# timoklein/alphazero-gym

Hardware: AMD Instinct MI355X
Metric: MCTS sims/sec (whole node), Pendulum-v1 4096 trees n_sims=200, 1/2/4/8 GPU (higher is better)
Workload: dtype f32; 1 GPU; config C: Pendulum-v1 A0C, 4096 trees/GPU x 200 sims, 2x256 ELU policy/value MLP, c_uct=0.05 c_pw=1 kappa=0.5; trees_per_gpu=4096, n_sims=200, parallelism=1 GPU

## Files before the change

alphazero_gym_amd/csrc/aux_kernels.cuh:

```cuda
#pragma once
#include "records.h"
#include "env.cuh"
#include "tree.cuh"
#include "results.cuh"


#define RS_TREES 16
__global__ __launch_bounds__(16 * RS_TREES) void results_kernel(KParams P) {
    const int sub = threadIdx.x & 15;
    const int tree = blockIdx.x * RS_TREES + (threadIdx.x >> 4);
    if (tree >= P.B) return;
    const size_t tb = (size_t)tree * P.R;
    TreeStore<TS_GLOBAL> ts;
    ts.hot = P.hot + tb;
    ts.child = P.child + tb * P.Kp;
    ts.prior = P.prior + tb;
    if (P.mode == AZG_MODE_CONTINUOUS) results_for_tree<true, TS_GLOBAL>(P, ts, P.cold + tb, P.action + tb, tb, tree, sub);
    else results_for_tree<false, TS_GLOBAL>(P, ts, P.cold + tb, P.action + tb, tb, tree, sub);
}


struct SelfPlay {
    int max_len, deterministic;
    int S_obs;
    int final_selection;
    double agent_eps;
    const double* ctab;
    unsigned step_idx;
    int* t; int* episode; int* fcnt;
    double* ret; double* fsum;
    float* rows;
    double* roots; int* carry;
};

__device__ __forceinline__ void selfplay_finish(const KParams& P, const SelfPlay& sp, int tree, float* row, float action, double v_target,
                                                int carry) {
    const int S = P.S;
    double root[4] = {0.0, 0.0, 0.0, 0.0};
    for (int k = 0; k < S; ++k) root[k] = sp.roots[(size_t)tree * S + k];
    float obs[8];
    double sn;
    game_obs(P.env_id, root, obs, &sn);
    for (int k = 0; k < 8; ++k) if (k < sp.S_obs) row[k] = obs[k];
    row[sp.S_obs + 3 * P.res_Kmax] = (float)v_target;
    double ns[4] = {0.0, 0.0, 0.0, 0.0}, r;
    int done;
    game_step(P.env_id, root, sn, action, ns, &r, &done);
    double ret = sp.ret[tree] + r;
    int t = sp.t[tree] + 1;
    if (done || t >= sp.max_len) {
        sp.fsum[tree] = sp.fsum[tree] + ret;
        sp.fcnt[tree] += 1;
        ret = 0.0;
        t = 0;
        const int ep = sp.episode[tree] + 1;
        sp.episode[tree] = ep;
        azg_reset_state(P.seed, (unsigned)(P.tree_base + tree), (unsigned)ep, azg_reset_kind(P.env_id), ns);
        carry = 0;
    }
    sp.carry[tree] = carry;
    sp.ret[tree] = ret;
    sp.t[tree] = t;
    for (int k = 0; k < S; ++k) sp.roots[(size_t)tree * S + k] = ns[k];
}

#define SP_TREES 16
__global__ __launch_bounds__(16 * SP_TREES) void selfplay_kernel16(KParams P, SelfPlay sp) {
    const int sub = threadIdx.x & 15;
    const int tree = blockIdx.x * SP_TREES + (threadIdx.x >> 4);
    if (tree >= P.B) return;
    const bool cont = P.mode == AZG_MODE_CONTINUOUS;
    const unsigned gtree = (unsigned)(P.tree_base + tree);
    const int K = P.res_Kmax, S_obs = sp.S_obs;
    float* row = sp.rows + (size_t)tree * (S_obs + 3 * K + 1);
    const int nc = P.res_nch[tree];
    const bool has = sub < nc;
    struct { int edge_n, node_n; double Q; } h;
    {
        const size_t o = (size_t)tree * K + (sub < K ? sub : 0);
        const int cn = P.res_child_n[o];
        h.edge_n = has ? P.res_counts[o] : 0;
        h.Q = has ? P.res_Q[o] : 0.0;
        h.node_n = (has && cn >= 0) ? cn : 0;
    }
    const float act = has ? (cont ? P.res_actions[(size_t)tree * K + sub] : (float)sub) : 0.0f;
    if (sub < K) {
        row[S_obs + sub] = act;
        row[S_obs + K + sub] = has ? (float)h.edge_n : 0.0f;
        row[S_obs + 2 * K + sub] = has ? (float)h.Q : 0.0f;
    }
    int tot = has ? h.edge_n : 0;
    double qmax = has ? h.Q : -__builtin_huge_val();
    int ckey = has ? ((h.edge_n << 4) | (15 - sub)) : -1;
    for (int m = 1; m < 16; m <<= 1) {
        tot += __shfl_xor(tot, m, 16);
        const double o = __shfl_xor(qmax, m, 16);
        qmax = o > qmax ? o : qmax;
        const int ok = __shfl_xor(ckey, m, 16);
        ckey = ok > ckey ? ok : ckey;
    }
    if (nc == 0) qmax = 0.0;
    const int cmax = ckey >> 4, amax = 15 - (ckey & 15);
    double x = 0.0;
    if (!cont && has) {
        if (sp.final_selection == AZG_FS_MAX_VALUE) x = h.Q / qmax;
        else x = sp.ctab ? sp.ctab[(size_t)cmax * (cmax + 1) / 2 + h.edge_n] : (double)h.edge_n / (double)cmax;
    }
    double onp = 0.0;
    if (P.res_v_target == AZG_VT_ON_POLICY) {
        if (!cont) {
            for (int a = 0; a < nc; ++a) onp += ((double)__shfl(h.edge_n, a, 16) / (double)tot) * __shfl(h.Q, a, 16);
        } else {
            for (int a = 0; a < nc; ++a) {
                const double qa = __shfl(h.Q, a, 16);
                for (int b2 = 0; b2 < nc; ++b2) onp += ((double)__shfl(h.edge_n, b2, 16) / (double)tot) * qa;
            }
        }
    }
    int pick = 0;
    if (cont) {
        pick = amax;
        if (sp.final_selection == AZG_FS_MAX_VALUE) {
            double qb = 0.0;
            for (int a = 0; a < nc; ++a) { const double q = __shfl(h.Q, a, 16); if (a == 0 || q > qb) { qb = q; pick = a; } }
        }
        if (sp.agent_eps != 0.0) {
            azg_u32x4 b = azg_draw(P.seed, gtree, sp.step_idx, 0u, AZG_STREAM_ACT);
            if ((double)azg_u01(b.v[0]) < sp.agent_eps) pick = (int)(b.v[1] % (unsigned)nc);
        }
    } else {
        double sum = 0.0;
        for (int a = 0; a < nc; ++a) sum = sum + __shfl(x, a, 16);
        const double pi = has ? __builtin_fabs(x / sum) : 0.0;
        double best = 0.0, cum = 0.0;
        for (int a = 0; a < nc; ++a) {
            const double pa = __shfl(pi, a, 16);
            if (a == 0 || pa > best) { best = pa; pick = a; }
            cum = cum + pa;
        }
        if (!sp.deterministic) {
            azg_u32x4 b = azg_draw(P.seed, gtree, sp.step_idx, 0u, AZG_STREAM_ACT);
            const double u = ((double)b.v[0] + 0.5) * (1.0 / 4294967296.0);
            const double last = cum;
            double c = 0.0;
            pick = nc - 1;
            bool found = false;
            for (int a = 0; a < nc; ++a) {
                const double pa = __shfl(pi, a, 16);
                if (!found) {
                    c = c + pa;
                    if (u < c / last) { pick = a; found = true; }
                }
            }
        }
    }
    const float pact = __shfl(act, pick, 16);
    const int pnode_n = __shfl(h.node_n, pick, 16);
    if (sub != 0) return;
    selfplay_finish(P, sp, tree, row, pact, P.res_v_target == AZG_VT_ON_POLICY ? onp : qmax, cont ? 0 : pnode_n);
}

#define SPW_THREADS 64
__global__ __launch_bounds__(SPW_THREADS) void selfplay_kernel(KParams P, SelfPlay sp) {
    const int tree = blockIdx.x * blockDim.x + threadIdx.x;
    if (tree >= P.B) return;
    const size_t tb = (size_t)tree * P.R;
    const unsigned gtree = (unsigned)(P.tree_base + tree);
    const int K = P.res_Kmax, S_obs = sp.S_obs;
    float* row = sp.rows + (size_t)tree * (S_obs + 3 * K + 1);
    const int nc = P.hot[tb].n_child;
    auto id = [&](int a) { return a < nc ? (int)P.child[tb * P.Kp + a] : 0; };
    auto rec = [&](int a) { return P.hot[tb + id(a)]; };
    auto act = [&](int a) { return P.action[tb + id(a)]; };
    double qmax = 0.0, onp = 0.0;
    long tot = 0;
    int cmax = 0, amax = 0;
    for (int a = 0; a < nc; ++a) tot += rec(a).edge_n;
    for (int a = 0; a < K; ++a) {
        const bool has = a < nc;
        const RecL h = rec(a);
        row[S_obs + a] = has ? act(a) : 0.0f;
        row[S_obs + K + a] = has ? (float)h.edge_n : 0.0f;
        row[S_obs + 2 * K + a] = has ? (float)h.Q : 0.0f;
        if (has) {
            if (a == 0 || h.Q > qmax) qmax = h.Q;
            if (a == 0 || h.edge_n > cmax) { cmax = h.edge_n; amax = a; }
        }
    }
    if (P.res_v_target == AZG_VT_ON_POLICY)
        for (int a = 0; a < nc; ++a)
            for (int b = 0; b < nc; ++b) onp += ((double)rec(b).edge_n / (double)tot) * rec(a).Q;
    int pick = amax;
    if (sp.final_selection == AZG_FS_MAX_VALUE) {
        double qb = 0.0;
        for (int a = 0; a < nc; ++a) { const double q = rec(a).Q; if (a == 0 || q > qb) { qb = q; pick = a; } }
    }
    if (sp.agent_eps != 0.0) {
        azg_u32x4 b = azg_draw(P.seed, gtree, sp.step_idx, 0u, AZG_STREAM_ACT);
        if ((double)azg_u01(b.v[0]) < sp.agent_eps) pick = (int)(b.v[1] % (unsigned)nc);
    }
    selfplay_finish(P, sp, tree, row, act(pick), P.res_v_target == AZG_VT_ON_POLICY ? onp : qmax, 0);
}
```

alphazero_gym_amd/csrc/azg_engine.hip:

```cpp
#include <cmath>
#include <cstdio>
#include <cstdlib>
#include <cstring>

#include "engine_host.h"
#include "../../include/azg_math.h"

static std::string g_create_err;

int fail(azg_engine* e, int code, const std::string& msg) {
    if (e) e->err = msg; else g_create_err = msg;
    return code;
}

static int ls_prepare(azg_engine* e) {
    if (e->ls_hp == e->HP) return AZG_OK;
    e->ls_mem.clear();
    const size_t B = e->cfg.n_trees, G = ((B + TREES_PER_WG - 1) / TREES_PER_WG + 3) / 4 * 4, HP = e->HP;
    float* obsT; float *a0, *a1, *parts; LsTree* tr; LsLane* ln;
    e->team_cnt_bytes = (((B + 31) / 32) * 8 * 32 + 32) * sizeof(unsigned);
    if (dalloc(e, e->ls_mem, &e->d_team_cnt, e->team_cnt_bytes / 4) ||
        dalloc(e, e->ls_mem, &obsT, G * 64) || dalloc(e, e->ls_mem, &a0, G * HP * 16) || dalloc(e, e->ls_mem, &a1, G * HP * 16) ||
        dalloc(e, e->ls_mem, &parts, G * (HP / 64) * 64 * 4) || dalloc(e, e->ls_mem, &tr, B) ||
        dalloc(e, e->ls_mem, &ln, B * 16))
        return AZG_E_DEVICE;
    e->ls.obsT = obsT; e->ls.act[0] = (f32x4*)a0; e->ls.act[1] = (f32x4*)a1; e->ls.parts = (f32x4*)parts;
    e->ls.tree = tr; e->ls.lane = ln;
    if (hipMemset(obsT, 0, G * 64 * sizeof(float)) != hipSuccess || hipMemset(a0, 0, G * HP * 16 * sizeof(float)) != hipSuccess || hipMemset(a1, 0, G * HP * 16 * sizeof(float)) != hipSuccess) return AZG_E_DEVICE;
    e->ls_hp = e->HP;
    return AZG_OK;
}

static bool use_lockstep(const azg_engine* e) {
    if (e->opt.force_persistent) return false;
    if (e->P.in8) return false;
    return e->HP >= 512 && e->n_hidden >= 2 && !e->P.layernorm;
}

template <int ENV>
static hipError_t search_path(azg_engine* e, bool lockstep) {
    if (lockstep) {
        if constexpr (ENV == AZG_ENV_ACROBOT) return hipErrorInvalidValue;
        else return azg_lockstep_search<ENV>(e);
    }
    return e->HP <= 128 ? azg_persistent_search<ENV, false>(e) : azg_persistent_search<ENV, true>(e);
}
static hipError_t search_launch(azg_engine* e, bool lockstep) {
    switch (azg_kernel_env(e->cfg)) {
        case AZG_ENV_CARTPOLE: return search_path<AZG_ENV_CARTPOLE>(e, lockstep);
        case AZG_ENV_MOUNTAINCAR_CONT: return search_path<AZG_ENV_MOUNTAINCAR_CONT>(e, lockstep);
        case AZG_ENV_ACROBOT: return search_path<AZG_ENV_ACROBOT>(e, lockstep);
        default: return search_path<AZG_ENV_PENDULUM_V1>(e, lockstep);
    }
}

static int team_check(azg_engine* e) {
    unsigned flag = 0;
    e->team_pending = 0;
    if (hipMemcpy(&flag, e->d_team_cnt + (e->team_cnt_bytes / 4 - 1), 4, hipMemcpyDeviceToHost) != hipSuccess)
        return fail(e, AZG_E_DEVICE, "reading the team kernel's status failed");
    if (flag) e->opt.ls_team = 0;
    if (flag == 0) return AZG_OK;
    e->team_fallbacks += 1;
    e->search_idx = e->team_search_idx;
    int rc = azg_search_resident(e);
    if (rc) return rc;
    if (hipStreamSynchronize(e->stream) != hipSuccess) return fail(e, AZG_E_DEVICE, "hipStreamSynchronize failed");
    return AZG_OK;
}
int settle_team(azg_engine* e) {
    if (!e->team_pending) return AZG_OK;
    HIPCHK(e, hipStreamSynchronize(e->stream));
    return team_check(e);
}

struct EnvFacts { int state_words, obs_width, discrete, n_actions; };
static constexpr EnvFacts kEnv[AZG_ENV_ACROBOT + 1] = {
    {4, 4, 1, 2},
    {2, 3, 0, 0},
    {2, 3, 0, 0},
    {2, 2, 1, 3},
    {2, 2, 0, 0},
    {4, 6, 1, 3},
};

static bool root_is_terminal(int env_id, const double* s) {
    switch (env_id) {
        case AZG_ENV_CARTPOLE: {
            const double theta_thr = 12.0 * 2.0 * 3.141592653589793 / 360.0, x_thr = 2.4;
            return (s[0] < -x_thr) || (s[0] > x_thr) || (s[2] < -theta_thr) || (s[2] > theta_thr);
        }
        case AZG_ENV_ACROBOT: return azg_acrobot_terminal(s);
        case AZG_ENV_MOUNTAINCAR: return s[0] >= 0.5 && s[1] >= 0.0;
        case AZG_ENV_MOUNTAINCAR_CONT: return s[0] >= 0.45 && s[1] >= 0.0;
        default: return false;
    }
}

EngineOptions EngineOptions::from_env() {
    const auto digit = [](const char* name, int dflt) {
        const char* v = getenv(name);
        return (v && v[0] >= '0' && v[0] <= '9') ? v[0] - '0' : dflt;
    };
    const auto num = [](const char* name) { const char* v = getenv(name); return v ? atoi(v) : 0; };
    EngineOptions o;
    o.force_persistent = digit("AZG_FORCE_PERSISTENT", 0) == 1;
    o.force_stream_weights = digit("AZG_FORCE_STREAM_WEIGHTS", 0) == 1;
    o.force_global_tree = digit("AZG_FORCE_GLOBAL_TREE", 0) == 1;
    o.no_spec = digit("AZG_NO_SPEC", 0) == 1;
    o.waves = digit("AZG_WAVES", o.waves);
    o.groups = digit("AZG_GROUPS", o.groups);
    { const int t = num("AZG_TRACE_CAP"); o.trace_cap = t > 0 ? t : 0; }
    { const int t = num("AZG_TILE_TREES"); o.tile_trees = (t == 16 || t == 8) ? t : 0; }
    o.ls_team = digit("AZG_LS_TEAM", o.ls_team);
    o.team_wide = digit("AZG_TEAM_WIDE", o.team_wide);
    o.team_tt = num("AZG_TEAM_TT");
    if (const char* v = getenv("AZG_TEAM_SPIN_LIMIT")) o.team_spin_limit = atol(v);
    o.no_lds_state = getenv("AZG_NO_LDS_STATE") != nullptr;
    o.publish_always = digit("AZG_PUBLISH_TREES", 0) == 1;
    return o;
}

extern "C" {

int azg_abi_version(void) { return AZG_ABI_VERSION; }

const char* azg_last_error(const azg_engine* e) { return e ? e->err.c_str() : g_create_err.c_str(); }

void azg_engine_destroy(azg_engine* e) {
    if (!e) return;
    DeviceScope scope(e->cfg.device_id);
    if (e->stream) (void)hipStreamSynchronize(e->stream);
    delete e;
}

static int mapped_hip_runtimes(std::string& paths) {
    static int cached_n = -1;
    static std::string cached_paths;
    if (cached_n >= 0) { paths = cached_paths; return cached_n; }
    std::vector<std::string> seen;
    FILE* f = fopen("/proc/self/maps", "r");
    if (!f) return 0;
    char line[1024];
    while (fgets(line, sizeof line, f)) {
        if (!strstr(line, "libamdhip64")) continue;
        const char* p = strchr(line, '/');
        if (!p) continue;
        std::string path(p);
        while (!path.empty() && (path.back() == '\n' || path.back() == ' ')) path.pop_back();
        bool dup = false;
        for (const auto& q : seen) dup = dup || q == path;
        if (!dup) seen.push_back(path);
    }
    fclose(f);
    paths.clear();
    for (const auto& q : seen) paths += (paths.empty() ? "" : ", ") + q;
    cached_paths = paths;
    cached_n = (int)seen.size();
    return cached_n;
}

static int engine_build(azg_engine* e) {
    const azg_config* cfg = &e->cfg;
    e->opt = EngineOptions::from_env();
    e->S_env = kEnv[cfg->env_id].state_words;
    e->S_obs = kEnv[cfg->env_id].obs_width;
    const int ns = cfg->n_sims;
    std::vector<int> pw(ns + 2, 0);
    if (cfg->mode == AZG_MODE_CONTINUOUS) {
        int kmax = 1;
        for (int n = 0; n < ns + 2; ++n) {
            double v = std::ceil(cfg->c_pw * std::pow((double)(n + 1), cfg->kappa));
            if (v > 1e6) v = 1e6;
            pw[n] = (int)v;
            if (n < ns && pw[n] > kmax) kmax = pw[n];
        }
        e->Kmax = kmax;
        e->R = ns + 2;
        e->nd = 2;
    } else {
        e->Kmax = cfg->num_actions;
        e->R = 1 + cfg->num_actions * (ns + 1);
        e->nd = cfg->num_actions;
    }
    if (e->R > 32767) return fail(e, AZG_E_UNSUPPORTED, "tree too large: records per tree must be < 32768");
    if (cfg->tie_break == AZG_TIE_RANDOM && e->Kmax > 16) return fail(e, AZG_E_UNSUPPORTED, "tie_break random supports at most 16 children per node");
    e->Kp = (e->Kmax + 15) / 16 * 16;
    e->tab_n = cfg->mode == AZG_MODE_CONTINUOUS ? ns + 2 : 4 * ns + 4;
    ON_DEVICE(e);
    (void)hipDeviceGetAttribute(&e->n_cus, hipDeviceAttributeMultiprocessorCount, cfg->device_id);
    HIPCHK(e, hipStreamCreateWithFlags(&e->stream, hipStreamNonBlocking));
    HIPCHK(e, hipEventCreate(&e->ev0));
    HIPCHK(e, hipEventCreate(&e->ev1));
    KParams& P = e->P;
    const size_t B = (size_t)cfg->n_trees, R = (size_t)e->R, K = (size_t)e->Kmax;
    RecL* hot; Cold* cold; double* edge_W; float* action; float* prior; unsigned short* child; int* n_rec;
    int* d_pw; double* d_sq; unsigned long long* stamps;
    e->res = ResultsLayout(B, K);
    e->stamp_n = stamp_rows(B);
    DeviceAllocs& mem = e->mem;
    if (dalloc(e, mem, &hot, B * R) || dalloc(e, mem, &cold, B * R) || dalloc(e, mem, &edge_W, B * R) || dalloc(e, mem, &action, B * R) ||
        dalloc(e, mem, &prior, B * R) || dalloc(e, mem, &child, B * R * e->Kp) || dalloc(e, mem, &n_rec, B) ||
        dalloc(e, mem, &d_pw, (size_t)ns + 2) || dalloc(e, mem, &d_sq, (size_t)e->tab_n) || dalloc(e, mem, &e->d_roots, B * e->S_env) ||
        dalloc(e, mem, &e->d_carry, B) || dalloc(e, mem, &e->d_res_block, e->res.bytes) || dalloc(e, mem, &e->d_child_n, B * K) ||
        dalloc(e, mem, &e->d_child_state, B * K * e->S_env) || dalloc(e, mem, &e->d_rootV, B) || dalloc(e, mem, &e->d_rootdist, B * e->nd) ||
        dalloc(e, e->stamp_mem, &stamps, e->stamp_n * 16))
        return AZG_E_DEVICE;
    HIPCHK(e, hipHostMalloc(&e->h_res.p, e->res.bytes, hipHostMallocDefault));
    char* const blk = e->d_res_block;
    e->d_Q = (double*)(blk + e->res.Q); e->d_vt = (double*)(blk + e->res.vt); e->d_actions = (float*)(blk + e->res.actions);
    e->d_counts = (int*)(blk + e->res.counts); e->d_nch = (int*)(blk + e->res.nch);
    std::vector<double> sq(e->tab_n);
    for (int n = 0; n < e->tab_n; ++n) sq[n] = std::sqrt((double)(n + 1));
    HIPCHK(e, hipMemcpy(d_pw, pw.data(), sizeof(int) * (ns + 2), hipMemcpyHostToDevice));
    HIPCHK(e, hipMemcpy(d_sq, sq.data(), sizeof(double) * e->tab_n, hipMemcpyHostToDevice));
    HIPCHK(e, hipMemset(hot, 0, B * R * sizeof(RecL)));
    HIPCHK(e, hipMemset(e->d_carry, 0, B * sizeof(int)));
    P.B = cfg->n_trees; P.n_sims = ns; P.R = e->R; P.Kp = e->Kp; P.A = cfg->num_actions; P.nd = e->nd;
    P.trace_cap = e->opt.trace_cap > 0 ? e->opt.trace_cap : 5;
    P.tie_random = cfg->tie_break == AZG_TIE_RANDOM; P.env_id = cfg->env_id; P.v1 = cfg->env_id == AZG_ENV_PENDULUM_V1; P.tree_base = cfg->tree_id_base; P.mode = cfg->mode;
    P.c_uct = cfg->c_uct; P.gamma = cfg->gamma; P.epsilon = cfg->epsilon; P.reward_scale = cfg->reward_scale;
    P.c_uct_f = (float)cfg->c_uct; P.gamma_f = (float)cfg->gamma; P.bound_f = (float)cfg->action_bound;
    P.seed = cfg->seed; P.S = e->S_env; P.tab_n = e->tab_n; P.pw0 = cfg->mode == AZG_MODE_CONTINUOUS ? pw[0] : 0;
    P.roots = e->d_roots; P.carry = e->d_carry;
    P.hot = hot; P.cold = cold; P.edge_W = edge_W; P.action = action; P.prior = prior; P.child = child;
    P.n_rec = n_rec; P.pw_need = d_pw; P.sqrt_tab = d_sq; P.stamps = stamps;
    P.res_actions = e->d_actions; P.res_counts = e->d_counts; P.res_Q = e->d_Q; P.res_vt = e->d_vt; P.res_nch = e->d_nch;
    P.res_child_n = e->d_child_n; P.res_child_state = e->d_child_state; P.res_root_V = e->d_rootV; P.res_root_dist = e->d_rootdist;
    P.res_Kmax = e->Kmax; P.res_v_target = cfg->v_target;
    P.net_T = cfg->n_trees; P.net_wgs = 1; P.net_wstride = 0;
    return AZG_OK;
}

int azg_engine_create(const azg_config* cfg, azg_engine** out) {
    if (!cfg || !out) return fail(nullptr, AZG_E_INVALID, "null argument");
    {
        std::string rts;
        const char* allow = getenv("AZG_ALLOW_MULTI_HIP");
        if (mapped_hip_runtimes(rts) > 1 && !(allow && allow[0] == '1'))
            return fail(nullptr, AZG_E_DEVICE, ("two HIP runtimes are mapped in this process (" + rts + "): load PyTorch (import torch) BEFORE "
                                               "libazgym_hip.so so that both use PyTorch's copy; if they are meant to coexist (differing "
                                               "SONAMEs, a deliberate second copy), set AZG_ALLOW_MULTI_HIP=1").c_str());
    }
    if (cfg->struct_size != (int32_t)sizeof(azg_config)) return fail(nullptr, AZG_E_INVALID, "azg_config size mismatch");
    if (cfg->n_trees < 1 || cfg->n_sims < 1) return fail(nullptr, AZG_E_INVALID, "n_trees and n_sims must be >= 1");
    if (cfg->env_id < 0 || cfg->env_id > AZG_ENV_ACROBOT) return fail(nullptr, AZG_E_INVALID, "unknown env_id");
    const bool discrete_env = kEnv[cfg->env_id].discrete;
    if (cfg->mode == AZG_MODE_DISCRETE && !discrete_env)
        return fail(nullptr, AZG_E_UNSUPPORTED, "discrete mode requires a discrete-action env (CartPole, MountainCar, Acrobot)");
    if (cfg->mode == AZG_MODE_CONTINUOUS && discrete_env)
        return fail(nullptr, AZG_E_UNSUPPORTED, "continuous mode requires a continuous-action env (Pendulum, MountainCarContinuous)");
    if (cfg->mode == AZG_MODE_DISCRETE && cfg->num_actions != kEnv[cfg->env_id].n_actions)
        return fail(nullptr, AZG_E_INVALID, "num_actions does not match the env (CartPole 2, MountainCar 3, Acrobot 3)");
    if (cfg->tie_break != AZG_TIE_FIRST && cfg->tie_break != AZG_TIE_RANDOM) return fail(nullptr, AZG_E_INVALID, "unknown tie_break");
    if (cfg->mode == AZG_MODE_CONTINUOUS && !(cfg->c_pw > 0.0 && cfg->c_pw < 1e6 && cfg->kappa >= 0.0 && cfg->kappa <= 8.0))
        return fail(nullptr, AZG_E_INVALID, "c_pw must be > 0 and kappa >= 0 (progressive widening: ceil(c_pw (n + 1)^kappa) children)");
    int ndev = 0;
    if (hipGetDeviceCount(&ndev) != hipSuccess || ndev < 1) return fail(nullptr, AZG_E_DEVICE, "no HIP device available");
    if (cfg->device_id < 0 || cfg->device_id >= ndev) return fail(nullptr, AZG_E_DEVICE, "device_id out of range");
    azg_engine* e = new azg_engine();
    e->cfg = *cfg;
    const int rc = engine_build(e);
    if (rc != AZG_OK) {
        const std::string msg = e->err;
        azg_engine_destroy(e);
        return fail(nullptr, rc, msg);
    }
    *out = e;
    return AZG_OK;
}

int azg_set_search_index(azg_engine* e, uint32_t idx) { if (!e) return AZG_E_INVALID; e->search_idx = idx; return AZG_OK; }

int azg_upload_roots(azg_engine* e, const double* roots, const int32_t* carry) {
    if (!e || !roots) return AZG_E_INVALID;
    const int B = e->cfg.n_trees, S = e->S_env;
    for (int i = 0; i < B; ++i)
        if (root_is_terminal(e->cfg.env_id, roots + (size_t)i * S)) return fail(e, AZG_E_TERMINAL_ROOT, "Can't do tree search from a terminal node");
    int cmax = 0;
    if (carry)
        for (int i = 0; i < B; ++i) {
            if (carry[i] < 0 || carry[i] > (1 << 30)) return fail(e, AZG_E_INVALID, "root_n_carry out of range");
            if (carry[i] != 0 && e->cfg.mode == AZG_MODE_CONTINUOUS)
                return fail(e, AZG_E_INVALID, "root_n_carry: continuous searches start from a fresh root (no carried count)");
            if (carry[i] > cmax) cmax = carry[i];
        }
    ON_DEVICE(e);
    { int trc = settle_team(e); if (trc) return trc; }
    e->carry_max = cmax;
    e->redo_ok = 0;
    HIPCHK(e, hipMemcpyAsync(e->d_roots, roots, sizeof(double) * (size_t)B * S, hipMemcpyHostToDevice, e->stream));
    if (carry) HIPCHK(e, hipMemcpyAsync(e->d_carry, carry, sizeof(int) * (size_t)B, hipMemcpyHostToDevice, e->stream));
    else HIPCHK(e, hipMemsetAsync(e->d_carry, 0, sizeof(int) * (size_t)B, e->stream));
    HIPCHK(e, hipStreamSynchronize(e->stream));
    return AZG_OK;
}

int azg_search_resident(azg_engine* e) {
    if (!e) return AZG_E_INVALID;
    if (!e->mlp_ready)
        return fail(e, AZG_E_STATE, e->n_nets > 1 ? "azg_set_net_weights has not been called for every net of the population"
                                                 : "azg_set_weights has not been called");
    if (e->n_nets > 1 && use_lockstep(e))
        return fail(e, AZG_E_UNSUPPORTED, "populations run on the one-launch search kernel only");
    ON_DEVICE(e);
    e->P.search_idx = e->search_idx;
    e->last_search_idx = e->search_idx;
    e->ms_kept_valid = 0;
    e->P.publish = (e->opt.publish_always || e->publish_once) ? 1 : 0;
    e->team_search_idx = e->search_idx;
    e->last = LaunchRecord();
    const bool lockstep = use_lockstep(e);
    if (lockstep) { int prc = ls_prepare(e); if (prc) return prc; }
    if (lockstep) HIPCHK(e, hipEventRecord(e->ev0, e->stream));
    const hipError_t rc = search_launch(e, lockstep);
    if (rc != hipSuccess) return fail(e, AZG_E_DEVICE, std::string("search kernel launch: ") + hipGetErrorString(rc));
    if (!e->last.timed) HIPCHK(e, hipEventRecord(e->ev1, e->stream));
    e->search_idx += 1;
    e->searched = 1;
    const bool persistent = e->last.form == AZG_FORM_PERSISTENT;
    e->results_valid = persistent ? 1 : 0;
    e->published = (!persistent || e->last.tree_lds == TS_GLOBAL || e->P.publish) ? 1 : 0;
    e->redo_ok = 1;
    if (persistent && e->last.tree_lds == TS_GLOBAL && e->last.lds_exit != AZG_LDS_EXIT_FORCED && !e->lds_warned) {
        e->lds_warned = 1;
        static const char* why[] = {"", "more than 511 records per tree (n_sims + 2)", "more than 16 children per node (c_pw / kappa)",
                                    "the workgroup's LDS plan exceeds the CU's 160 KB", "", "",
                                    "the root's visit count (carried + n_sims) overflows the LDS records' counters"};
        const int x = e->last.lds_exit;
        const char* reason = x == AZG_LDS_EXIT_RECORDS && e->R <= 511 ? "more than 255 records per tree (n_sims + 2) for this network's kernels"
                                                                      : (x >= 0 && x < (int)(sizeof(why) / sizeof(why[0])) ? why[x] : "");
        if (!getenv("AZG_QUIET"))
            fprintf(stderr, "azgym: the trees of this search do not fit LDS residency (%s): they are kept in global memory -- same results, "
                            "slower tree walk (azg_search_info; once per engine)\n", reason);
    }
    return AZG_OK;
}

int azg_sync(azg_engine* e) {
    if (!e) return AZG_E_INVALID;
    ON_DEVICE(e);
    HIPCHK(e, hipStreamSynchronize(e->stream));
    return settle_team(e);
}

int azg_search(azg_engine* e, const double* roots, const int32_t* carry) {
    int rc = azg_upload_roots(e, roots, carry);
    if (rc) return rc;
    rc = azg_search_resident(e);
    if (rc) return rc;
    return azg_sync(e);
}

int azg_last_search_ms(azg_engine* e, float* ms) {
    if (!e || !ms) return AZG_E_INVALID;
    if (!e->searched) return fail(e, AZG_E_STATE, "no search has run");
    ON_DEVICE(e);
    HIPCHK(e, hipEventSynchronize(e->ev1));
    { int trc = settle_team(e); if (trc) return trc; }
    if (e->ms_kept_valid) { *ms = e->ms_kept; return AZG_OK; }
    HIPCHK(e, hipEventElapsedTime(ms, e->ev0, e->ev1));
    return AZG_OK;
}

static int gather_results(azg_engine* e) {
    ON_DEVICE(e);
    int rc = launch_results(e);
    if (rc) return rc;
    HIPCHK(e, hipStreamSynchronize(e->stream));
    return AZG_OK;
}

int azg_results(azg_engine* e, float* actions, int32_t* counts, double* Q, double* v_target, int32_t* n_children) {
    if (!e) return AZG_E_INVALID;
    ON_DEVICE(e);
    int rc = launch_results(e);
    if (rc) return rc;
    const ResultsLayout& L = e->res;
    HIPCHK(e, hipMemcpyAsync(e->h_res.p, e->d_res_block, L.bytes, hipMemcpyDeviceToHost, e->stream));
    HIPCHK(e, hipStreamSynchronize(e->stream));
    const char* h = (const char*)e->h_res.p;
    if (Q) memcpy(Q, h + L.Q, L.vt - L.Q);
    if (v_target) memcpy(v_target, h + L.vt, L.actions - L.vt);
    if (actions) memcpy(actions, h + L.actions, L.counts - L.actions);
    if (counts) memcpy(counts, h + L.counts, L.nch - L.counts);
    if (n_children) memcpy(n_children, h + L.nch, L.bytes - L.nch);
    return AZG_OK;
}

int azg_results_resident(azg_engine* e, const float** actions, const int32_t** counts, const double** Q, const double** v_target,
                         const int32_t** n_children) {
    if (!e) return AZG_E_INVALID;
    ON_DEVICE(e);
    int rc = launch_results(e);
    if (rc) return rc;
    if (actions) *actions = e->d_actions;
    if (counts) *counts = e->d_counts;
    if (Q) *Q = e->d_Q;
    if (v_target) *v_target = e->d_vt;
    if (n_children) *n_children = e->d_nch;
    return AZG_OK;
}

int azg_root_children(azg_engine* e, int32_t* child_n, double* child_state) {
    if (!e) return AZG_E_INVALID;
    int rc = gather_results(e);
    if (rc) return rc;
    size_t B = e->cfg.n_trees, K = e->Kmax;
    D2H(child_n, e->d_child_n, B * K * 4);
    D2H(child_state, e->d_child_state, B * K * e->S_env * 8);
    return AZG_OK;
}

int azg_root_eval(azg_engine* e, float* value, float* dist) {
    if (!e) return AZG_E_INVALID;
    if (e->n_nets > 1) return fail(e, AZG_E_UNSUPPORTED, "azg_root_eval: not available for populations (azg_set_population > 1)");
    int rc = gather_results(e);
    if (rc) return rc;
    size_t B = e->cfg.n_trees;
    D2H(value, e->d_rootV, B * 4);
    D2H(dist, e->d_rootdist, B * e->nd * 4);
    return AZG_OK;
}

int azg_mlp_eval(azg_engine* e, const float* obs, size_t n, float* value, float* dist, float* raw) {
    if (!e || !obs) return AZG_E_INVALID;
    if (e->n_nets > 1) return fail(e, AZG_E_UNSUPPORTED, "azg_mlp_eval: not available for populations (azg_set_population > 1): evaluate each net's policy");
    if (!e->mlp_ready) return fail(e, AZG_E_STATE, "azg_set_weights has not been called");
    if (n == 0) return AZG_OK;
    if (n > (size_t)1 << 24) return fail(e, AZG_E_INVALID, "too many observations in one call");
    ON_DEVICE(e);
    const size_t So = e->S_obs, nd = e->nd;
    const size_t need = n * (So + 1 + nd + 1 + nd);
    if (need > e->eval_floats) {
        e->eval_mem.clear();
        e->eval_floats = 0;
        if (dalloc(e, e->eval_mem, &e->d_eval, need)) return AZG_E_DEVICE;
        e->eval_floats = need;
    }
    float* d_obs = e->d_eval;
    float* d_v = d_obs + n * So;
    float* d_d = d_v + n;
    float* d_r = d_d + n * nd;
    HIPCHK(e, hipMemcpyAsync(d_obs, obs, n * So * 4, hipMemcpyHostToDevice, e->stream));
    hipError_t rc = azg_dispatch_mlp_eval(e, d_obs, (int)n, d_v, d_d, d_r);
    if (rc != hipSuccess) return fail(e, AZG_E_DEVICE, std::string("mlp_eval kernel launch: ") + hipGetErrorString(rc));
    HIPCHK(e, hipStreamSynchronize(e->stream));
    D2H(value, d_v, n * 4);
    D2H(dist, d_d, n * nd * 4);
    D2H(raw, d_r, n * (nd + 1) * 4);
    return AZG_OK;
}

int azg_dump_tree(azg_engine* e, int32_t* n_records, int32_t* parent, int32_t* edge_n, double* edge_W, double* edge_Q,
                  float* edge_action, int32_t* node_n, double* node_r, float* node_V, uint8_t* node_flags) {
    if (!e) return AZG_E_INVALID;
    if (!e->searched) return fail(e, AZG_E_STATE, "no search has run");
    ON_DEVICE(e);
    HIPCHK(e, hipStreamSynchronize(e->stream));
    { int trc = settle_team(e); if (trc) return trc; }
    if (!e->published) {
        if (!e->redo_ok)
            return fail(e, AZG_E_STATE, "the last search's trees were not written out and its inputs have changed since (self-play step, new "
                                        "roots or weights): dump right after the search, or set AZG_PUBLISH_TREES=1");
        float ms_before = 0.0f;
        HIPCHK(e, hipEventElapsedTime(&ms_before, e->ev0, e->ev1));
        const uint32_t idx_now = e->search_idx;
        e->publish_once = 1;
        e->search_idx = e->last_search_idx;
        int rc = azg_search_resident(e);
        e->publish_once = 0;
        e->search_idx = idx_now;
        if (rc) return rc;
        HIPCHK(e, hipStreamSynchronize(e->stream));
        { int trc = settle_team(e); if (trc) return trc; }
        e->ms_kept = ms_before; e->ms_kept_valid = 1;
    }
    size_t B = e->cfg.n_trees, R = e->R;
    std::vector<RecL> hot(B * R);
    std::vector<Cold> cold(B * R);
    std::vector<int> nrec(B);
    std::vector<double> ew(B * R);
    std::vector<float> ac(B * R);
    HIPCHK(e, hipMemcpy(hot.data(), e->P.hot, B * R * sizeof(RecL), hipMemcpyDeviceToHost));
    HIPCHK(e, hipMemcpy(cold.data(), e->P.cold, B * R * sizeof(Cold), hipMemcpyDeviceToHost));
    HIPCHK(e, hipMemcpy(nrec.data(), e->P.n_rec, B * 4, hipMemcpyDeviceToHost));
    HIPCHK(e, hipMemcpy(ew.data(), e->P.edge_W, B * R * 8, hipMemcpyDeviceToHost));
    HIPCHK(e, hipMemcpy(ac.data(), e->P.action, B * R * 4, hipMemcpyDeviceToHost));
    const bool cont = e->cfg.mode == AZG_MODE_CONTINUOUS;
    const int A = e->cfg.num_actions;
    for (size_t i = 0; i < B; ++i) {
        if (n_records) n_records[i] = nrec[i];
        for (size_t j = 0; j < R; ++j) {
            size_t o = i * R + j;
            bool in = (int)j < nrec[i];
            const RecL& h = hot[o];
            bool ex = in && (h.flags & FLAG_EXPANDED);
            if (parent) parent[o] = in ? (j == 0 ? -1 : h.parent) : 0;
            if (edge_n) edge_n[o] = in ? h.edge_n : 0;
            if (edge_W) edge_W[o] = in ? ew[o] : 0.0;
            if (edge_Q) edge_Q[o] = in ? h.Q : 0.0;
            if (edge_action) edge_action[o] = in ? (cont ? ac[o] : (j == 0 ? 0.0f : (float)((j - 1) % A))) : 0.0f;
            if (node_n) node_n[o] = in ? h.node_n : 0;
            if (node_r) node_r[o] = ex ? cold[o].r : 0.0;
            if (node_V) node_V[o] = ex ? cold[o].V : 0.0f;
            if (node_flags) node_flags[o] = in ? h.flags : 0;
        }
    }
    return AZG_OK;
}

static int kernel_name(const azg_engine* e, char* buf, size_t n) {
    const int env = azg_kernel_env(e->cfg);
    const char* gmm = (env != AZG_ENV_CARTPOLE && e->P.ncomp >= 2) ? "true" : "false";
    const LaunchRecord& r = e->last;
    switch (r.form) {
        case AZG_FORM_PERSISTENT: return snprintf(buf, n, "search_kernel<%d, %d, %d, %d, %s, %d, %d, %d, %d>", env, e->HP, e->nreg, r.tree_lds, gmm, r.waves, r.groups, r.tile_trees, r.spec);
        case AZG_FORM_PER_LAYER: return snprintf(buf, n, "ls_tree_kernel<%d, ...> + ls_layer0_kernel + ls_hidden_tiled_kernel<%d, ...> per simulation step", env, e->HP);
        case AZG_FORM_TEAM: return snprintf(buf, n, "ls_team_kernel<%d, %d, %s, %d, %d, %d, %d, %d>", env, e->HP, gmm, r.tree_lds, r.team_kc, r.team_minb, r.spec, r.team_tt);
        default: return snprintf(buf, n, "(no search yet)");
    }
}

int azg_search_info(azg_engine* e, azg_search_report* info) {
    if (!e || !info) return AZG_E_INVALID;
    if (info->struct_size != (int32_t)sizeof(azg_search_report)) return fail(e, AZG_E_INVALID, "azg_search_info: struct_size mismatch");
    if (e->searched && e->team_pending) {
        ON_DEVICE(e);
        int trc = settle_team(e);
        if (trc) return trc;
    }
    memset(info, 0, sizeof(*info));
    info->struct_size = (int32_t)sizeof(azg_search_report);
    const LaunchRecord& r = e->last;
    info->kernel_form = e->searched ? r.form : AZG_FORM_NONE;
    info->max_records = e->R; info->max_children = e->Kmax;
    info->team_fallbacks = e->team_fallbacks;
    if (!e->searched) { kernel_name(e, info->kernel_name, sizeof(info->kernel_name)); info->lds_exit = AZG_LDS_RESIDENT; return AZG_OK; }
    info->tree_storage = r.form == AZG_FORM_PERSISTENT ? r.tree_lds : AZG_TREES_GLOBAL;
    info->lds_exit = r.lds_exit;
    info->spec = r.spec;
    info->waves = r.waves; info->groups = r.groups; info->tile_trees = r.tile_trees;
    if (r.form == AZG_FORM_TEAM) { info->team_trees = r.team_tt; info->team_per_cu = r.team_minb; info->team_parts = r.team_parts; }
    float ms = 0.0f;
    int rc = azg_last_search_ms(e, &ms);
    if (rc) return rc;
    info->last_ms = ms;
    kernel_name(e, info->kernel_name, sizeof(info->kernel_name));
    return AZG_OK;
}

int azg_max_children(const azg_engine* e) { return e ? e->Kmax : AZG_E_INVALID; }
int azg_max_records(const azg_engine* e) { return e ? e->R : AZG_E_INVALID; }
int azg_env_state_dim(const azg_engine* e) { return e ? e->S_env : AZG_E_INVALID; }
int azg_obs_dim(const azg_engine* e) { return e ? e->S_obs : AZG_E_INVALID; }

int azg_synthetic_roots(azg_engine* e, double* roots) {
    if (!e || !roots) return AZG_E_INVALID;
    for (int i = 0; i < e->cfg.n_trees; ++i)
        azg_reset_state(e->cfg.seed, (uint32_t)(e->cfg.tree_id_base + i), 0u, azg_reset_kind(e->cfg.env_id), roots + (size_t)i * e->S_env);
    return AZG_OK;
}

}
```

alphazero_gym_amd/csrc/engine_host.h:

```cpp
#pragma once
#include <hip/hip_runtime.h>

#include <atomic>
#include <string>
#include <vector>

#include "hip_host.h"
#include "records.h"
#include "../../include/azgym_population.h"

struct EngineOptions {
    int force_persistent = 0;
    int force_stream_weights = 0;
    int force_global_tree = 0;
    int waves = 0;
    int groups = 0;
    int trace_cap = 0;
    int no_spec = 0;
    int tile_trees = 0;
    int ls_team = 1;
    int team_wide = 1;
    int team_tt = 0;
    long team_spin_limit = 1L << 23;
    int no_lds_state = 0;
    int publish_always = 0;
    static EngineOptions from_env();
};
#define AZG_MAX_DEVICES 64

struct LaunchRecord {
    int form = AZG_FORM_NONE;
    int tree_lds = TS_GLOBAL, spec = 0;
    int lds_exit = AZG_LDS_NOT_APPLICABLE;
    int waves = 0, groups = 0, tile_trees = 0;
    int team_kc = 0, team_minb = 0, team_tt = 0, team_parts = 0;
    int timed = 0;
};

struct WeightMap {
    bool valid = false;
    azg_mlp_desc desc;
    int HP = 0;
    std::vector<unsigned> src;
    size_t oW0, oW0b, ob0, oW0u, ob0u, oWl[MAX_STREAM_LAYERS], obl[MAX_STREAM_LAYERS], oWh, obh, olg[MAX_STREAM_LAYERS], olb[MAX_STREAM_LAYERS];
};

struct ResultsLayout {
    size_t Q = 0, vt = 0, actions = 0, counts = 0, nch = 0, bytes = 0;
    ResultsLayout() = default;
    ResultsLayout(size_t B, size_t K) : vt(B * K * 8), actions(vt + B * 8), counts(actions + B * K * 4), nch(counts + B * K * 4), bytes(nch + B * 4) {}
};

struct EngineQueue {
    hipStream_t stream = nullptr;
    hipEvent_t ev0 = nullptr, ev1 = nullptr;
    ~EngineQueue() {
        if (ev0) (void)hipEventDestroy(ev0);
        if (ev1) (void)hipEventDestroy(ev1);
        if (stream) (void)hipStreamDestroy(stream);
    }
};

struct azg_engine : EngineQueue {
    azg_config cfg{};
    EngineOptions opt;
    int carry_max = 0;
    int S_env = 0, S_obs = 0, Kmax = 0, Kp = 0, R = 0, nd = 0, tab_n = 0;
    int mlp_ready = 0, HP = 0, n_hidden = 0, nreg = 0;
    int n_cus = 256;
    LaunchRecord last;
    KParams P{};
    DeviceAllocs mem;
    DeviceAllocs wblob_mem; float* d_wblob = nullptr;
    size_t w_floats = 0;
    std::vector<float> w_stage;
    WeightMap wmap;
    DeviceAllocs wmap_mem; unsigned* d_wmap = nullptr;
    DeviceAllocs dist_mem;
    int dist_nd = -1, dist_ncomp = -1;
    float* d_actions = nullptr; int* d_counts = nullptr; double* d_Q = nullptr; double* d_vt = nullptr; int* d_nch = nullptr;
    int* d_child_n = nullptr; double* d_child_state = nullptr; float* d_rootV = nullptr; float* d_rootdist = nullptr;
    ResultsLayout res;
    char* d_res_block = nullptr; PinnedBlock h_res;
    double* d_roots = nullptr; int* d_carry = nullptr;
    uint32_t search_idx = 0;
    int sp_on = 0, sp_max_len = 0, sp_det = 0, sp_cap = 0, sp_steps = 0, sp_row = 0;
    int sp_insert = 0, sp_fs = 0, sp_ring = 0;
    long long sp_total = 0;
    double sp_agent_eps = 0.0;
    double* d_sp_ctab = nullptr;
    uint32_t sp_step_idx = 0;
    int* d_sp_t = nullptr; int* d_sp_episode = nullptr; int* d_sp_fcnt = nullptr; double* d_sp_ret = nullptr; double* d_sp_fsum = nullptr;
    float* d_sp_rows = nullptr;
    DeviceAllocs sp_mem;
    unsigned* d_team_cnt = nullptr; size_t team_cnt_bytes = 0;
    int team_pending = 0;
    int team_fallbacks = 0;
    uint32_t team_search_idx = 0;
    int lds_warned = 0;
    LockStep ls{};
    DeviceAllocs ls_mem;
    int ls_hp = 0;
    DeviceAllocs eval_mem; float* d_eval = nullptr; size_t eval_floats = 0;
    DeviceAllocs rollout_mem; char* d_rollout = nullptr; size_t rollout_bytes = 0;
    std::vector<char> rollout_stage;
    int searched = 0, results_valid = 0;
    int publish_once = 0;
    int published = 0;
    int redo_ok = 0;
    int n_nets = 1;
    std::vector<char> net_have = std::vector<char>(1, 0);
    DeviceAllocs stamp_mem; size_t stamp_n = 0;
    uint32_t last_search_idx = 0;
    float ms_kept = 0.0f; int ms_kept_valid = 0;
    std::string err;
};


int fail(azg_engine* e, int code, const std::string& msg);

#define HIPCHK(e, call)                                                                                  \
    do {                                                                                                 \
        hipError_t _rc = (call);                                                                         \
        if (_rc != hipSuccess) return fail(e, AZG_E_DEVICE, std::string(#call) + ": " + hipGetErrorString(_rc)); \
    } while (0)
#define ON_DEVICE(e)                                     \
    DeviceScope _scope((e)->cfg.device_id);              \
    if (!_scope.ok) return fail(e, AZG_E_DEVICE, "hipSetDevice failed")
#define D2H(dst, src, bytes) do { if (dst) HIPCHK(e, hipMemcpy(dst, src, bytes, hipMemcpyDeviceToHost)); } while (0)

template <typename T>
static int dalloc(azg_engine* e, DeviceAllocs& mem, T** p, size_t n) {
    if ((*p = mem.alloc<T>(n))) return AZG_OK;
    return fail(e, AZG_E_DEVICE, std::string("hipMalloc: ") + hipGetErrorString(mem.last));
}

int settle_team(azg_engine* e);
int launch_results(azg_engine* e);

static inline size_t stamp_rows(size_t B) {
    size_t r = ((B + 3) / 4) * 4;
    const size_t r8 = ((B + 15) / 16) * 8, team = ((B + 31) / 32) * 16 * 3 / 2;
    if (r8 > r) r = r8;
    if (team > r) r = team;
    return r < 16 ? 16 : r;
}

static inline long azg_padded_trees(const azg_engine* e, int tpw) {
    const long T = e->cfg.n_trees / e->n_nets;
    return (long)e->n_nets * ((T + tpw - 1) / tpw * tpw);
}

static inline int azg_kernel_env(const azg_config& c) {
    if (c.mode == AZG_MODE_DISCRETE) return c.env_id == AZG_ENV_ACROBOT ? AZG_ENV_ACROBOT : AZG_ENV_CARTPOLE;
    return c.env_id == AZG_ENV_MOUNTAINCAR_CONT ? AZG_ENV_MOUNTAINCAR_CONT : AZG_ENV_PENDULUM_V1;
}

struct TreeStorage { int ts, lds_exit; };
static inline TreeStorage azg_tree_storage(const azg_engine* e, bool lds9) {
    const long nmax = (long)e->carry_max + e->cfg.n_sims + 2;
    if (e->opt.force_global_tree) return {TS_GLOBAL, AZG_LDS_EXIT_FORCED};
    if (e->Kp != 16) return {TS_GLOBAL, AZG_LDS_EXIT_CHILDREN};
    if (e->R <= 255) return nmax < 65536 ? TreeStorage{TS_LDS8, AZG_LDS_RESIDENT} : TreeStorage{TS_GLOBAL, AZG_LDS_EXIT_COUNTS};
    if (e->R > 511 || !lds9) return {TS_GLOBAL, AZG_LDS_EXIT_RECORDS};
    return nmax < 2048 ? TreeStorage{TS_LDS9, AZG_LDS_RESIDENT} : TreeStorage{TS_GLOBAL, AZG_LDS_EXIT_COUNTS};
}

struct KernelAttrs {
    std::atomic<int> static_lds{-1};
    std::atomic<size_t> dyn_lds[AZG_MAX_DEVICES] = {};
    std::atomic<int> per_cu[AZG_MAX_DEVICES] = {};

    hipError_t static_bytes(const void* kern, int* bytes) {
        if ((*bytes = static_lds.load(std::memory_order_relaxed)) >= 0) return hipSuccess;
        hipFuncAttributes fa;
        hipError_t rc = hipFuncGetAttributes(&fa, kern);
        if (rc == hipSuccess) static_lds.store(*bytes = (int)fa.sharedSizeBytes, std::memory_order_relaxed);
        return rc;
    }
    hipError_t set_dyn_lds(const azg_engine* e, const void* kern, size_t bytes) {
        std::atomic<size_t>& last = dyn_lds[e->cfg.device_id % AZG_MAX_DEVICES];
        if (last.load(std::memory_order_relaxed) == bytes) return hipSuccess;
        hipError_t rc = hipFuncSetAttribute(kern, hipFuncAttributeMaxDynamicSharedMemorySize, (int)bytes);
        if (rc == hipSuccess) last.store(bytes, std::memory_order_relaxed);
        return rc;
    }
    hipError_t occupancy(const azg_engine* e, const void* kern, int threads, size_t bytes, int* blocks) {
        std::atomic<int>& cached = per_cu[e->cfg.device_id % AZG_MAX_DEVICES];
        *blocks = cached.load(std::memory_order_relaxed);
        if (*blocks > 0 && dyn_lds[e->cfg.device_id % AZG_MAX_DEVICES].load(std::memory_order_relaxed) == bytes) return hipSuccess;
        hipError_t rc = set_dyn_lds(e, kern, bytes);
        if (rc == hipSuccess) rc = hipOccupancyMaxActiveBlocksPerMultiprocessor(blocks, kern, threads, bytes);
        if (rc == hipSuccess) cached.store(*blocks, std::memory_order_relaxed);
        return rc;
    }
};

template <int ENV, bool WIDE> hipError_t azg_persistent_search(azg_engine* e);
template <int ENV> hipError_t azg_lockstep_search(azg_engine* e);
template <int ENV> hipError_t azg_team_search(azg_engine* e);
hipError_t azg_team_wide_forms(azg_engine* e, int g_base, int G, bool dry, bool common, bool t32, bool t64);
hipError_t azg_dispatch_mlp_eval(azg_engine* e, const float* obs, int n, float* value, float* dist, float* raw);
```

alphazero_gym_amd/csrc/engine_selftest.hip:

```cpp
#include "engine_host.h"
#include "probe_kernels.cuh"

extern "C" {

int azg_debug_stamps(azg_engine* e, unsigned long long* out, size_t max_rows) {
    if (!e || !out) return AZG_E_INVALID;
    size_t rows = e->stamp_n;
    if (rows > max_rows) rows = max_rows;
    ON_DEVICE(e);
    HIPCHK(e, hipStreamSynchronize(e->stream));
    HIPCHK(e, hipMemcpy(out, e->P.stamps, rows * 16 * sizeof(unsigned long long), hipMemcpyDeviceToHost));
    return (int)rows;
}

int azg_math_selftest(int device_id, int fn_id, const double* in, double* out, size_t n) {
    if (!in || !out || n == 0) return AZG_E_INVALID;
    DeviceScope scope(device_id);
    if (!scope.ok) return AZG_E_DEVICE;
    DeviceAllocs mem;
    double* const di = mem.alloc<double>(n);
    double* const dout = mem.alloc<double>(n);
    if (!di || !dout) return AZG_E_DEVICE;
    int rc = AZG_OK;
    if (hipMemcpy(di, in, n * 8, hipMemcpyHostToDevice) != hipSuccess) rc = AZG_E_DEVICE;
    if (rc == AZG_OK) {
        if (fn_id == 100) {
            int K = (int)((n - 1) / 2);
            hipLaunchKernelGGL(mfma_probe_kernel, dim3(1), dim3(64), 0, 0, di, dout, K);
        } else if (fn_id == 102 && n >= 16) {
            std::vector<int> hc(1 << 16);
            for (size_t i = 0; i < hc.size(); ++i) hc[i] = (int)((i * 4099 + 77) & (hc.size() - 1));
            if (int* chase = mem.alloc<int>(hc.size())) {
                (void)hipMemcpy(chase, hc.data(), hc.size() * 4, hipMemcpyHostToDevice);
                hipLaunchKernelGGL(latency_probe_kernel, dim3(1), dim3(64), 0, 0, dout, chase, 4096);
                (void)hipDeviceSynchronize();
            }
        } else if (fn_id == 101 && n >= 8) {
            const int wgs = (int)in[0], iters = (int)in[1], reps = (int)in[2] > 0 ? (int)in[2] : 1;
            hipEvent_t e0, e1;
            (void)hipEventCreate(&e0); (void)hipEventCreate(&e1);
            hipLaunchKernelGGL(mfma_rate_kernel, dim3(wgs), dim3(256), 0, 0, dout, iters);
            (void)hipEventRecord(e0, 0);
            for (int r = 0; r < reps; ++r) hipLaunchKernelGGL(mfma_rate_kernel, dim3(wgs), dim3(256), 0, 0, dout, iters);
            (void)hipEventRecord(e1, 0);
            (void)hipEventSynchronize(e1);
            float ms = 0.0f;
            (void)hipEventElapsedTime(&ms, e0, e1);
            double res[2] = {ms / reps, (double)wgs * 4 * iters * 16 * 2048.0 / (ms / reps * 1e-3) / 1e12};
            (void)hipMemcpy(dout + 3, res, sizeof(res), hipMemcpyHostToDevice);
            (void)hipEventDestroy(e0); (void)hipEventDestroy(e1);
        } else {
            hipLaunchKernelGGL(math_selftest_kernel, dim3((unsigned)((n + 255) / 256)), dim3(256), 0, 0, fn_id, di, dout, n);
        }
        if (hipGetLastError() != hipSuccess || hipDeviceSynchronize() != hipSuccess) rc = AZG_E_DEVICE;
    }
    if (rc == AZG_OK && hipMemcpy(out, dout, n * 8, hipMemcpyDeviceToHost) != hipSuccess) rc = AZG_E_DEVICE;
    return rc;
}

}
```

alphazero_gym_amd/csrc/env.cuh:

```cuda
#pragma once
#include "records.h"


template <int ENV> struct EnvFamily {
    static constexpr bool CONT = ENV == AZG_ENV_PENDULUM_V1 || ENV == AZG_ENV_MOUNTAINCAR_CONT;
    static constexpr bool TERM = ENV != AZG_ENV_PENDULUM_V1;
    static constexpr int S = CONT ? 2 : 4;
    static constexpr bool IN8 = ENV == AZG_ENV_ACROBOT;
};

template <int ENV>
__device__ __forceinline__ void env_obs(const double* s, float* obs, double* sn_out) {
    if (ENV == AZG_ENV_CARTPOLE) {
        obs[0] = (float)s[0]; obs[1] = (float)s[1]; obs[2] = (float)s[2]; obs[3] = (float)s[3];
        *sn_out = 0.0;
    } else if (ENV == AZG_ENV_MOUNTAINCAR_CONT) {
        obs[0] = (float)s[0]; obs[1] = (float)s[1]; obs[2] = 0.0f; obs[3] = 0.0f;
        *sn_out = 0.0;
    } else {
        double sn, cs;
        azg_sincos(s[0], &sn, &cs);
        obs[0] = (float)cs; obs[1] = (float)sn; obs[2] = (float)s[1]; obs[3] = 0.0f;
        *sn_out = sn;
    }
}

__device__ __forceinline__ void cartpole_step(const double* s, int action, double* o, double* reward, int* done) {
    const double gravity = 9.8, masspole = 0.1, total_mass = 0.1 + 1.0, length = 0.5;
    const double polemass_length = 0.1 * 0.5, force_mag = 10.0, tau = 0.02;
    const double theta_thr = 12.0 * 2.0 * 3.141592653589793 / 360.0, x_thr = 2.4;
    double x = s[0], x_dot = s[1], theta = s[2], theta_dot = s[3];
    double force = action == 1 ? force_mag : -force_mag;
    double sintheta, costheta;
    azg_sincos(theta, &sintheta, &costheta);
    double temp = (force + (polemass_length * (theta_dot * theta_dot)) * sintheta) / total_mass;
    double thetaacc = (gravity * sintheta - costheta * temp) /
                      (length * (4.0 / 3.0 - (masspole * (costheta * costheta)) / total_mass));
    double xacc = temp - ((polemass_length * thetaacc) * costheta) / total_mass;
    x = x + tau * x_dot;
    x_dot = x_dot + tau * xacc;
    theta = theta + tau * theta_dot;
    theta_dot = theta_dot + tau * thetaacc;
    o[0] = x; o[1] = x_dot; o[2] = theta; o[3] = theta_dot;
    *done = (x < -x_thr) || (x > x_thr) || (theta < -theta_thr) || (theta > theta_thr);
    *reward = 1.0;
}

__device__ __forceinline__ void mountaincar_step(const double* s, int action, double* o, double* reward, int* done) {
    const double min_position = -1.2, max_position = 0.6, max_speed = 0.07, goal_position = 0.5, goal_velocity = 0.0;
    const double force = 0.001, gravity = 0.0025;
    double position = s[0], velocity = s[1];
    double sn, cs;
    azg_sincos(3.0 * position, &sn, &cs);
    velocity = velocity + ((double)(action - 1) * force + cs * (-gravity));
    velocity = velocity < -max_speed ? -max_speed : (velocity > max_speed ? max_speed : velocity);
    position = position + velocity;
    position = position < min_position ? min_position : (position > max_position ? max_position : position);
    if (position == min_position && velocity < 0.0) velocity = 0.0;
    o[0] = position; o[1] = velocity; o[2] = 0.0; o[3] = 0.0;
    *done = (position >= goal_position) && (velocity >= goal_velocity);
    *reward = -1.0;
}

__device__ __forceinline__ void mountaincar_cont_step(const double* s, float action, double* o, double* reward, int* done) {
    const double min_position = -1.2, max_position = 0.6, max_speed = 0.07, goal_position = 0.45, goal_velocity = 0.0, power = 0.0015;
    double position = s[0], velocity = s[1];
    const double a = (double)action;
    const double force = a < -1.0 ? -1.0 : (a > 1.0 ? 1.0 : a);
    double sn, cs;
    azg_sincos(3.0 * position, &sn, &cs);
    velocity = velocity + (force * power - 0.0025 * cs);
    velocity = velocity > max_speed ? max_speed : velocity;
    velocity = velocity < -max_speed ? -max_speed : velocity;
    position = position + velocity;
    position = position > max_position ? max_position : position;
    position = position < min_position ? min_position : position;
    if (position == min_position && velocity < 0.0) velocity = 0.0;
    const int d = (position >= goal_position) && (velocity >= goal_velocity);
    o[0] = position; o[1] = velocity;
    *done = d;
    *reward = (d ? 100.0 : 0.0) - (a * a) * 0.1;
}

__device__ __forceinline__ void discrete_env_step(int env_id, const double* s, int action, double* o, double* reward, int* done) {
    if (env_id == AZG_ENV_MOUNTAINCAR) mountaincar_step(s, action, o, reward, done);
    else cartpole_step(s, action, o, reward, done);
}
template <int ENV>
__device__ __forceinline__ void family_env_step(int env_id, const double* s, int action, double* o, double* reward, int* done) {
    if constexpr (ENV == AZG_ENV_ACROBOT) azg_acrobot_step(s, action, o, reward, done);
    else discrete_env_step(env_id, s, action, o, reward, done);
}

__device__ __forceinline__ void discrete_env_obs(int env_id, const double* s, float* obs8) {
    if (env_id == AZG_ENV_ACROBOT) { azg_acrobot_obs(s, obs8); obs8[6] = 0.0f; obs8[7] = 0.0f; }
    else { obs8[0] = (float)s[0]; obs8[1] = (float)s[1]; obs8[2] = (float)s[2]; obs8[3] = (float)s[3]; obs8[4] = obs8[5] = obs8[6] = obs8[7] = 0.0f; }
}

__device__ __forceinline__ double discrete_env_reward(int env_id) { return env_id == AZG_ENV_CARTPOLE ? 1.0 : -1.0; }
__device__ __forceinline__ double discrete_env_terminal_reward(int env_id) {
    return env_id == AZG_ENV_CARTPOLE ? 1.0 : (env_id == AZG_ENV_ACROBOT ? 0.0 : -1.0);
}

__device__ __forceinline__ double pendulum_torque(float action) {
    const float max_torque = 2.0f;
    const float uc = action < -max_torque ? -max_torque : (action > max_torque ? max_torque : action);
    return (double)uc;
}
__device__ __forceinline__ double pendulum_reward(const double* s, float action) {
    const double pi = 3.141592653589793;
    const double th = s[0], thdot = s[1], u = pendulum_torque(action);
    const double an = azg_pymod(th + pi, 2.0 * pi, 0.15915494309189535) - pi;
    const double costs = (an * an + 0.1 * (thdot * thdot)) + 0.001 * (u * u);
    return -costs;
}
__device__ __forceinline__ void pendulum_dynamics(int v1, const double* s, double sn_th, float action, double* o) {
    const double max_speed = 8.0, dt = 0.05, pi = 3.141592653589793;
    const double th = s[0], thdot = s[1], u = pendulum_torque(action);
    double newth, newthdot, sn, cs;
    if (v1) {
        newthdot = thdot + (15.0 * sn_th + 3.0 * u) * dt;
        newthdot = newthdot < -max_speed ? -max_speed : (newthdot > max_speed ? max_speed : newthdot);
        newth = th + newthdot * dt;
    } else {
        azg_sincos(th + pi, &sn, &cs);
        newthdot = thdot + (-15.0 * sn + 3.0 * u) * dt;
        newth = th + newthdot * dt;
        newthdot = newthdot < -max_speed ? -max_speed : (newthdot > max_speed ? max_speed : newthdot);
    }
    o[0] = newth; o[1] = newthdot;
}
__device__ __forceinline__ void pendulum_step(int v1, const double* s, double sn_th, float action, double* o, double* reward, int* done) {
    *reward = pendulum_reward(s, action);
    pendulum_dynamics(v1, s, sn_th, action, o);
    *done = 0;
}


__device__ __forceinline__ bool env_is_continuous(int env_id) {
    return env_id == AZG_ENV_PENDULUM_V0 || env_id == AZG_ENV_PENDULUM_V1 || env_id == AZG_ENV_MOUNTAINCAR_CONT;
}
__device__ __forceinline__ void game_obs(int env_id, const double* s, float* obs8, double* sn) {
    if (!env_is_continuous(env_id)) { discrete_env_obs(env_id, s, obs8); *sn = 0.0; return; }
    if (env_id == AZG_ENV_MOUNTAINCAR_CONT) env_obs<AZG_ENV_MOUNTAINCAR_CONT>(s, obs8, sn);
    else env_obs<AZG_ENV_PENDULUM_V1>(s, obs8, sn);
    obs8[4] = obs8[5] = obs8[6] = obs8[7] = 0.0f;
}
__device__ __forceinline__ void game_step(int env_id, const double* s, double sn, float action, double* ns, double* reward, int* done) {
    if (env_id == AZG_ENV_ACROBOT) azg_acrobot_step(s, (int)action, ns, reward, done);
    else if (!env_is_continuous(env_id)) discrete_env_step(env_id, s, (int)action, ns, reward, done);
    else if (env_id == AZG_ENV_MOUNTAINCAR_CONT) mountaincar_cont_step(s, action, ns, reward, done);
    else pendulum_step(env_id == AZG_ENV_PENDULUM_V1, s, sn, action, ns, reward, done);
}
```

alphazero_gym_amd/csrc/lockstep.cuh:

```cuda
#pragma once
#include <type_traits>

#include "records.h"
#include "env.cuh"
#include "mlp.cuh"
#include "tree.cuh"
#include "tree_phases.cuh"

template <int ENV, bool GMM, int NCH, int HP>
__global__ __launch_bounds__(256) void ls_tree_kernel(KParams P, LockStep L, int sim, int g_base) {
    constexpr bool CONT = EnvFamily<ENV>::CONT;
    extern __shared__ double s_dyn[];
    const int tid = threadIdx.x, wave = tid >> 6, lane = tid & 63, sub = lane & 15;
    const int tl = wave * 4 + (lane >> 4);
    const int tg = g_base + blockIdx.x;
    const int tree = tg * TREES_PER_WG + tl;
    const bool live = tree < P.B;
    const unsigned gtree = (unsigned)(P.tree_base + tree);
    double* s_sqrt = s_dyn;
    int* s_pw = (int*)(s_dyn + P.tab_n);
    for (int i = tid; i < P.tab_n; i += 256) s_sqrt[i] = P.sqrt_tab[i];
    if (CONT) for (int i = tid; i < P.n_sims + 2; i += 256) s_pw[i] = P.pw_need[i];
    __syncthreads();
    const size_t tb = (size_t)(live ? tree : 0) * P.R;
    Cold* cold = P.cold + tb;
    double* edge_W = P.edge_W + tb;
    float* action = P.action + tb;
    TreeStore<false> ts;
    ts.hot = P.hot + tb;
    ts.child = P.child + tb * P.Kp;
    ts.prior = P.prior + tb;
    float* obsT = L.obsT + (size_t)tg * 64;
    TreeState st;
    if (sim == -2) {
        tree_init_root<ENV, false>(P, st, ts, cold, edge_W, action, tree, live, sub, tl, gtree, obsT);
    } else {
        const LsTree t = L.tree[live ? tree : 0];
#ifdef AZG_STAMPS
        unsigned long long st_acc[16] = {0, 0, 0, 0, 0, 0, 0, 0, 0, 0, 0, 0, 0, 0, 0, 0};
#endif
        const LsLane ln = L.lane[(size_t)(live ? tree : 0) * 16 + sub];
        st.nrec = t.nrec; st.eps_draws = t.eps_draws; st.leaf = t.leaf; st.need_eval = live && t.need_eval; st.path_D = t.path_D;
        st.kbase = t.kbase; st.my_depth = ln.my_depth; st.pid = ln.pid; st.pr = ln.pr; st.pW = ln.pW; st.eps_c = ln.eps_c;
        if (live) tree_phase_a<ENV, false, GMM, NCH>(P, st, ts, cold, edge_W, action, tb, sim, sub, tl, gtree,
                                                     L.parts + (size_t)tg * NCH * 64, P.bhead, s_sqrt STAMP_ARG, s_pw);
        st.need_eval = false;
        if (sim < P.n_sims - 1) {
            __threadfence_block();
            if (live) tree_phase_b<ENV, false, GMM>(P, st, ts, cold, edge_W, action, tb, sub, tl, gtree, s_sqrt, s_pw, obsT STAMP_ARG);
            else if (sub < 4) obsT[sub * 16 + tl] = 0.0f;
        } else if (live && sub == 0) {
            P.n_rec[tree] = st.nrec;
        }
    }
    if (live) {
        if (sub == 0) {
            LsTree t;
            t.nrec = st.nrec; t.eps_draws = st.eps_draws; t.leaf = st.leaf; t.need_eval = st.need_eval ? 1 : 0; t.path_D = st.path_D;
            t.kbase = st.kbase;
            L.tree[tree] = t;
        }
        LsLane ln;
        ln.my_depth = st.my_depth; ln.pid = st.pid; ln.pr = st.pr; ln.pW = st.pW; ln.eps_c = st.eps_c; ln.pad = 0.0f;
        L.lane[(size_t)tree * 16 + sub] = ln;
    }
}

template <int HP>
__global__ __launch_bounds__(256) void ls_layer0_kernel(KParams P, LockStep L, int g_base) {
    constexpr int NS = HP / 256;
    const int tg = g_base + blockIdx.x / NS, sl = blockIdx.x % NS;
    const int wave = threadIdx.x >> 6, lane = threadIdx.x & 63;
    const float b = L.obsT[(size_t)tg * 64 + lane];
    f32x4* out = L.act[0] + (size_t)tg * (HP / 16) * 64;
#pragma unroll
    for (int i = 0; i < 4; ++i) {
        const int tile = sl * 16 + wave * 4 + i;
        f32x4 acc = __builtin_amdgcn_mfma_f32_16x16x4f32(P.W0[tile * 64 + lane], b, P.b0[tile * 64 + lane], 0, 0, 0);
        out[tile * 64 + lane] = act4<true>(P.act, acc);
    }
}

#ifndef LS_KC
#define LS_KC 4
#endif
#ifndef LS_PIPE
#define LS_PIPE 4
#endif
#ifndef LS_LAYER_WD
#define LS_LAYER_WD 0
#endif
#ifndef LS_LAYER_KC
#define LS_LAYER_KC 2
#endif
#ifndef LS_XCD_2D
#define LS_XCD_2D 1
#endif
template <bool SC1>
struct TileMem {
    __amdgpu_buffer_rsrc_t r;
    const f32x4* p;
    bool wt;
    __device__ __forceinline__ explicit TileMem(const void* base, bool write_through = true) : p((const f32x4*)base), wt(write_through) {
        if constexpr (SC1) r = __builtin_amdgcn_make_buffer_rsrc((void*)base, 0, 0x7fffffff, 0x00020000);
    }
    __device__ __forceinline__ f32x4 load4(size_t i) const {
        if constexpr (SC1) {
            typedef unsigned u32x4 __attribute__((ext_vector_type(4)));
            u32x4 v = __builtin_amdgcn_raw_buffer_load_b128(r, (int)(i * 16), 0, 16);
            return __builtin_bit_cast(f32x4, v);
        } else return p[i];
    }
    __device__ __forceinline__ float load1(size_t i) const {
        if constexpr (SC1) return __builtin_bit_cast(float, __builtin_amdgcn_raw_buffer_load_b32(r, (int)(i * 4), 0, 16));
        else return ((const float*)p)[i];
    }
    __device__ __forceinline__ void store1(size_t i, float v) const {
        if constexpr (SC1) {
            if (wt) __builtin_amdgcn_raw_buffer_store_b32(__builtin_bit_cast(unsigned, v), r, (int)(i * 4), 0, 16);
            else __builtin_amdgcn_raw_buffer_store_b32(__builtin_bit_cast(unsigned, v), r, (int)(i * 4), 0, 0);
        } else ((float*)p)[i] = v;
    }
    __device__ __forceinline__ void store4(size_t i, f32x4 v) const {
        if constexpr (SC1) {
            typedef unsigned u32x4 __attribute__((ext_vector_type(4)));
            if (wt) __builtin_amdgcn_raw_buffer_store_b128(__builtin_bit_cast(u32x4, v), r, (int)(i * 16), 0, 16);
            else __builtin_amdgcn_raw_buffer_store_b128(__builtin_bit_cast(u32x4, v), r, (int)(i * 16), 0, 0);
        } else ((f32x4*)p)[i] = v;
    }
};

template <int HP, bool LAST, int TG, int UT, bool SC1, int KC_ = LS_KC, int DBG = 0>
__device__ __forceinline__ void ls_tile(const KParams& P, const LockStep& L, int layer, int in_buf, int us, int g0, f32x4* s_ab, bool wt = true) {
    static_assert(!LAST || UT == 4, "a head chunk is 4 tiles");
    static_assert(TG == 4 || TG == 2, "4 waves: one or two per tree group");
    constexpr int WPG = 4 / TG;
    constexpr int WT = UT / WPG;
    constexpr int S4 = HP / 16, NU = HP / (16 * UT), KC = KC_, NCHUNK = S4 / KC;
    constexpr int PIPE = LS_PIPE == 4 && KC < 4 ? 3 : LS_PIPE;
    static_assert(S4 % KC == 0, "k-blocks per layer must be a multiple of the chunk");
    constexpr int ASZ = UT * KC * 64, BSZ = TG * KC * 64;
    constexpr int STAGE = ASZ + BSZ;
    constexpr int NLA = ASZ / 256, NLB = BSZ / 256;
    static_assert(ASZ % 256 == 0 && BSZ % 256 == 0, "chunk does not divide over the workgroup");
    const int tid = threadIdx.x, lane = tid & 63, wave = tid >> 6;
    const int t0 = us * UT;
    const int wg = wave % TG, wt0 = (wave / TG) * WT;
    const f32x4* W = P.Wl[layer - 1];
    const TileMem<SC1> in(L.act[in_buf]), out(L.act[in_buf ^ 1], wt), parts(L.parts, wt);
    f32x4 ra[NLA], rb[NLB];
    auto load_one = [&](int c, int j) {
        const int jj = j < NLA ? j : j - NLA;
        const int e = jj * 256 + tid, i = e / (KC * 64), r = e % (KC * 64);
        if (j < NLA) ra[jj] = W[((size_t)(t0 + i) * S4 + c * KC) * 64 + r];
        else rb[jj] = in.load4(((size_t)(g0 + i) * S4 + c * KC) * 64 + r);
    };
    f32x4 dbg_const = {1.0f, 2.0f, 3.0f, 4.0f};
    if (DBG & 8) asm volatile("" : "+v"(dbg_const));
    auto store_one = [&](int st, int j) {
        if (DBG & 8) { s_ab[st * STAGE + j * 256 + tid] = dbg_const; return; }
        if (j < NLA) s_ab[st * STAGE + j * 256 + tid] = ra[j];
        else s_ab[st * STAGE + ASZ + (j - NLA) * 256 + tid] = rb[j - NLA];
    };
    auto load_chunk = [&](int c) {
#pragma unroll
        for (int j = 0; j < NLA + NLB; ++j) load_one(c, j);
    };
    auto store_chunk = [&](int st) {
#pragma unroll
        for (int j = 0; j < NLA + NLB; ++j) store_one(st, j);
    };
    f32x4 acc[WT];
#pragma unroll
    for (int i = 0; i < WT; ++i) acc[i] = P.bl[layer - 1][(t0 + wt0 + i) * 64 + lane];
    load_chunk(0);
    store_chunk(0);
    if (PIPE >= 2 && NCHUNK > 1) load_chunk(1);
    __syncthreads();
#pragma unroll
    for (int i = 0; i < WT; ++i) asm volatile("" : "+v"(acc[i]));
    constexpr int NL = NLA + NLB, NGRP = 4 * KC;
    constexpr int SLOT0 = 1, SLOTD = (NGRP - 2) / NL > 0 ? (NGRP - 2) / NL : 1;
    auto chunk = [&](int c, auto has1_t, auto has2_t) {
        constexpr bool has1 = decltype(has1_t)::value, has2 = decltype(has2_t)::value;
        if (PIPE == 2) {
            if (has1) store_chunk((c + 1) & 1);
            if (has2) load_chunk(c + 2);
        } else if (PIPE == 1 && has1) load_chunk(c + 1);
        const f32x4* sB = s_ab + (c & 1) * STAGE + ASZ + wg * KC * 64;
        const f32x4* sA = s_ab + (c & 1) * STAGE + wt0 * KC * 64;
        f32x4 a[WT], b, an[WT], bn;
        b = sB[lane];
#pragma unroll
        for (int i = 0; i < WT; ++i) a[i] = sA[(i * KC) * 64 + lane];
#pragma unroll
        for (int s = 0; s < KC; ++s) {
            if (s + 1 < KC && !(DBG & 4)) {
                bn = sB[(s + 1) * 64 + lane];
#pragma unroll
                for (int i = 0; i < WT; ++i) an[i] = sA[(i * KC + s + 1) * 64 + lane];
            }
            __builtin_amdgcn_sched_barrier(0);
#pragma unroll
            for (int cmp = 0; cmp < 4; ++cmp) {
#pragma unroll
                for (int i = 0; i < WT; ++i) acc[i] = __builtin_amdgcn_mfma_f32_16x16x4f32(a[i][cmp], b[cmp], acc[i], 0, 0, 0);
                if (PIPE == 3) {
                    const int q = 4 * s + cmp;
                    if (q >= SLOT0 && (q - SLOT0) % SLOTD == 0 && (q - SLOT0) / SLOTD < NL) {
                        const int j = (q - SLOT0) / SLOTD;
                        __builtin_amdgcn_sched_barrier(0);
                        if (has1 && !(DBG & 2)) store_one((c + 1) & 1, j);
                        if (has2 && !(DBG & 1)) load_one(c + 2, j);
                        __builtin_amdgcn_sched_barrier(0);
                    }
                }
            }
            if (s + 1 < KC && !(DBG & 4)) {
                b = bn;
#pragma unroll
                for (int i = 0; i < WT; ++i) a[i] = an[i];
            }
        }
        if (PIPE == 1 && has1) store_chunk((c + 1) & 1);
        if (!(DBG & 2)) __syncthreads();
    };
    constexpr int NS4 = 4 * (KC - 1), SLOTD4 = NS4 / NL > 0 ? NS4 / NL : 1, SLOT04 = NS4 > NL * SLOTD4 ? 1 : 0;
    static_assert(PIPE != 4 || NS4 >= NL, "schedule 4 deals the staging pieces out over the first KC - 1 k-blocks");
    f32x4 ca[WT], cb;
    auto chunk4 = [&](int c, auto has1_t, auto has2_t) {
        constexpr bool has1 = decltype(has1_t)::value, has2 = decltype(has2_t)::value;
        const f32x4* sB = s_ab + (c & 1) * STAGE + ASZ + wg * KC * 64;
        const f32x4* sA = s_ab + (c & 1) * STAGE + wt0 * KC * 64;
        f32x4 an[WT], bn;
#pragma unroll
        for (int s = 0; s < KC; ++s) {
            if (s + 1 < KC) {
                if (!(DBG & 4)) {
                    bn = sB[(s + 1) * 64 + lane];
#pragma unroll
                    for (int i = 0; i < WT; ++i) an[i] = sA[(i * KC + s + 1) * 64 + lane];
                }
            } else {
                if (!(DBG & 2)) asm volatile("s_waitcnt lgkmcnt(0)\n\ts_barrier" ::: "memory");
                if (has1 && !(DBG & 4)) {
                    const f32x4* sBn = s_ab + ((c + 1) & 1) * STAGE + ASZ + wg * KC * 64;
                    const f32x4* sAn = s_ab + ((c + 1) & 1) * STAGE + wt0 * KC * 64;
                    bn = sBn[lane];
#pragma unroll
                    for (int i = 0; i < WT; ++i) an[i] = sAn[(i * KC) * 64 + lane];
                }
            }
            __builtin_amdgcn_sched_barrier(0);
#pragma unroll
            for (int cmp = 0; cmp < 4; ++cmp) {
#pragma unroll
                for (int i = 0; i < WT; ++i) acc[i] = __builtin_amdgcn_mfma_f32_16x16x4f32(ca[i][cmp], cb[cmp], acc[i], 0, 0, 0);
                const int q = 4 * s + cmp;
                if (s + 1 < KC && q >= SLOT04 && (q - SLOT04) % SLOTD4 == 0 && (q - SLOT04) / SLOTD4 < NL) {
                    const int j = (q - SLOT04) / SLOTD4;
                    __builtin_amdgcn_sched_barrier(0);
                    if (has1 && !(DBG & 2)) store_one((c + 1) & 1, j);
                    if (has2 && !(DBG & 1)) load_one(c + 2, j);
                    __builtin_amdgcn_sched_barrier(0);
                }
            }
            if ((s + 1 < KC || has1) && !(DBG & 4)) {
                cb = bn;
#pragma unroll
                for (int i = 0; i < WT; ++i) ca[i] = an[i];
            }
        }
    };
    static_assert(NCHUNK >= 2, "the staging pipeline is written for at least two chunks");
    (void)chunk; (void)chunk4;
    if constexpr (PIPE == 4) {
        cb = s_ab[ASZ + wg * KC * 64 + lane];
#pragma unroll
        for (int i = 0; i < WT; ++i) ca[i] = s_ab[(wt0 + i) * KC * 64 + lane];
#pragma unroll 1
        for (int c = 0; c < NCHUNK - 2; ++c) chunk4(c, std::true_type{}, std::true_type{});
        chunk4(NCHUNK - 2, std::true_type{}, std::false_type{});
        chunk4(NCHUNK - 1, std::false_type{}, std::false_type{});
    } else {
#pragma unroll 1
        for (int c = 0; c < NCHUNK - 2; ++c) chunk(c, std::true_type{}, std::true_type{});
        chunk(NCHUNK - 2, std::true_type{}, std::false_type{});
        chunk(NCHUNK - 1, std::false_type{}, std::false_type{});
    }
    if (DBG & 8) {
#pragma unroll
        for (int j = 0; j < NLA; ++j) asm volatile("" ::"v"(ra[j]));
#pragma unroll
        for (int j = 0; j < NLB; ++j) asm volatile("" ::"v"(rb[j]));
    }
    f32x4 h[WT];
#pragma unroll
    for (int i = 0; i < WT; ++i) h[i] = act4<true>(P.act, acc[i]);
    const int tg = g0 + wg;
    if constexpr (!LAST) {
#pragma unroll
        for (int i = 0; i < WT; ++i) out.store4(((size_t)tg * S4 + t0 + wt0 + i) * 64 + lane, h[i]);
    } else {
        f32x4 hs = {0.0f, 0.0f, 0.0f, 0.0f};
        if constexpr (WPG == 2) {
            if (wt0 == 0) {
#pragma unroll
                for (int i = 0; i < WT; ++i) hs = mfma4(P.Whead[(t0 + i) * 64 + lane], h[i], hs);
                s_ab[wg * 64 + lane] = hs;
            }
            __syncthreads();
            if (wt0 != 0) {
                hs = s_ab[wg * 64 + lane];
#pragma unroll
                for (int i = 0; i < WT; ++i) hs = mfma4(P.Whead[(t0 + wt0 + i) * 64 + lane], h[i], hs);
                parts.store4(((size_t)tg * NU + us) * 64 + lane, hs);
            }
        } else {
#pragma unroll
            for (int i = 0; i < 4; ++i) hs = mfma4(P.Whead[(t0 + i) * 64 + lane], h[i], hs);
            parts.store4(((size_t)tg * NU + us) * 64 + lane, hs);
        }
    }
}

template <int HP, bool LAST, int TG, bool SC1, int KC>
__device__ __forceinline__ void ls_tile_wd(const KParams& P, const LockStep& L, int layer, int in_buf, int us, int g0, f32x4* s_b, bool wt = true) {
    constexpr int S4 = HP / 16, NU = HP / 64, NCHUNK = S4 / KC;
    constexpr int BSZ = TG * KC * 64;
    constexpr int NLB = BSZ / 256;
    static_assert(S4 % KC == 0 && BSZ % 256 == 0 && NCHUNK >= 4 && NCHUNK % 2 == 0, "chunking");
    static_assert(KC >= 2 && 4 * (KC - 1) >= NLB, "the staging pieces are dealt out over the first KC - 1 k-blocks");
    const int tid = threadIdx.x, lane = tid & 63, wave = tid >> 6;
    const int tile = us * 4 + wave;
    const f32x4* W = P.Wl[layer - 1] + (size_t)tile * S4 * 64 + lane;
    const TileMem<SC1> in(L.act[in_buf]), out(L.act[in_buf ^ 1], wt), parts(L.parts, wt);
    f32x4 aw[2][KC];
    f32x4 rb[NLB];
    auto load_b = [&](int c, int j) {
        const int e = j * 256 + tid, i = e / (KC * 64), r = e % (KC * 64);
        rb[j] = in.load4(((size_t)(g0 + i) * S4 + c * KC) * 64 + r);
    };
    auto store_b = [&](int st, int j) { s_b[st * BSZ + j * 256 + tid] = rb[j]; };
    f32x4 acc[TG];
#pragma unroll
    for (int g = 0; g < TG; ++g) acc[g] = P.bl[layer - 1][tile * 64 + lane];
    f32x4 whead = {0.0f, 0.0f, 0.0f, 0.0f};
    if constexpr (LAST) whead = P.Whead[tile * 64 + lane];
#pragma unroll
    for (int s = 0; s < KC; ++s) aw[0][s] = W[s * 64];
#pragma unroll
    for (int j = 0; j < NLB; ++j) load_b(0, j);
// ... 109 lines not shown
```

alphazero_gym_amd/csrc/records.h:

```cpp
#pragma once
#include <hip/hip_runtime.h>
#include "../../include/azg_math.h"
#include "../../include/azgym.h"

#define FLAG_EXPANDED 1
#define FLAG_TERMINAL 2
#define TREES_PER_WG 16
#define MAX_STREAM_LAYERS 8

typedef float f32x4 __attribute__((ext_vector_type(4)));

struct __attribute__((aligned(16))) RecS {
    double Q;
    unsigned short edge_n;
    unsigned short node_n;
    unsigned char parent;
    unsigned char n_child : 5;
    unsigned char wnext : 1;
    unsigned char flags : 2;
    unsigned char first;
    unsigned char cbase;
};
#define POOL_UNITS(R) ((7 * ((R) - 1) + 8) / 9 + 1)
struct __attribute__((aligned(16))) RecM {
    double Q;
    unsigned long long edge_n : 11;
    unsigned long long node_n : 11;
    unsigned long long parent : 9;
    unsigned long long first : 9;
    unsigned long long cbase : 9;
    unsigned long long n_child : 5;
    unsigned long long flags : 2;
    unsigned long long wnext : 1;
};
static_assert(sizeof(RecM) == 16, "RecM must be 16 bytes");
#define TS_GLOBAL 0
#define TS_LDS8 1
#define TS_LDS9 2
struct __attribute__((aligned(8))) RecL {
    double Q;
    int edge_n;
    int node_n;
    short parent;
    unsigned short n_child;
    unsigned short first;
    unsigned char flags;
    unsigned char pad;
};
static_assert(sizeof(RecS) == 16, "RecS must be 16 bytes");
static_assert(sizeof(RecL) == 24, "RecL must be 24 bytes");

struct __attribute__((aligned(16))) Cold {
    double s[4];
    double r;
    float V;
    float mu;
    float sg;
    float pad;
};
static_assert(sizeof(Cold) == 64, "Cold must be 64 bytes");

struct KParams {
    int B, n_sims, R, Kp, A, nd, n_out, n_hidden, act, v1, tree_base, mode;
    double c_uct, gamma, epsilon, reward_scale;
    float c_uct_f, gamma_f, bound_f, ls_min, ls_max;
    unsigned long long seed;
    unsigned search_idx;
    int S;
    int tab_n;
    const double* roots;
    const int* carry;
    RecL* hot;
    Cold* cold;
    double* edge_W;
    float* action;
    float* prior;
    float* gmm;
    int ncomp;
    unsigned short* child;
    int* n_rec;
    const int* pw_need;
    const double* sqrt_tab;
    const f32x4* W0u;
    const f32x4* b0u;
    const float* W0;
    const float* W0b;
    int in8;
    const f32x4* b0;
    const f32x4* Wl[MAX_STREAM_LAYERS];
    const f32x4* bl[MAX_STREAM_LAYERS];
    const f32x4* Whead;
    const float* bhead;
    int layernorm;
    int Htrue[MAX_STREAM_LAYERS];
    const f32x4* lng[MAX_STREAM_LAYERS];
    const f32x4* lnb[MAX_STREAM_LAYERS];
    float* res_actions; int* res_counts; double* res_Q; double* res_vt; int* res_nch; int* res_child_n; double* res_child_state;
    float* res_root_V; float* res_root_dist;
    int res_Kmax, res_v_target;
    int tie_random;
    int env_id;
    int trace_cap;
    int lds_state;
    int pw0;
    int publish;
    unsigned long long* stamps;
    int net_T, net_wgs;
    size_t net_wstride;
};

struct LsLane { int my_depth, pid; double pr, pW; float eps_c; float pad; };
struct LsTree { int nrec; unsigned eps_draws; int leaf, need_eval, path_D, kbase; };

struct LockStep {
    float* obsT;
    f32x4* act[2];
    f32x4* parts;
    LsTree* tree;
    LsLane* lane;
};


#ifdef AZG_STAMPS
#ifdef AZG_STAMP_ONLY
#define STAMP_ON(s1, s2) ((s1) == (AZG_STAMP_ONLY) || (s2) == (AZG_STAMP_ONLY))
#else
#define STAMP_ON(s1, s2) 1
#endif
#define STAMP3(var, s1, s2, s3) [[maybe_unused]] unsigned long long var = 0; if constexpr (STAMP_ON(s1, s2) || STAMP_ON(s3, s3)) { var = __builtin_amdgcn_s_memtime(); __builtin_amdgcn_sched_barrier(0); }
#define STAMP2(var, s1, s2) STAMP3(var, s1, s2, -1)
#define STAMP(var) STAMP2(var, -2, -2)
#define STAMP_ADD(slot, t0, t1) do { if constexpr (STAMP_ON(slot, slot)) st_acc[slot] += (t1) - (t0); } while (0)
#define STAMP_PARAM , unsigned long long* st_acc
#define STAMP_ARG , st_acc
#ifdef AZG_STAMPS_A
#define STAMP_A(var, s1, s2) STAMP2(var, s1, s2)
#define STAMP_A_ADD(slot, t0, t1) do { if constexpr (STAMP_ON(slot, slot)) { if (st_acc) st_acc[slot] += (t1) - (t0); } } while (0)
#define STAMP_M(var, s1, s2) [[maybe_unused]] unsigned long long var = 0
#define STAMP_M_ADD(slot, t0, t1)
#else
#define STAMP_A(var, s1, s2)
#define STAMP_A_ADD(slot, t0, t1)
#define STAMP_M(var, s1, s2) STAMP2(var, s1, s2)
#define STAMP_M_ADD(slot, t0, t1) STAMP_ADD(slot, t0, t1)
#endif
#define STAMP_PARAM_OPT , unsigned long long* st_acc = nullptr
#else
#define STAMP_PARAM
#define STAMP_ARG
#define STAMP(var)
#define STAMP2(var, s1, s2)
#define STAMP3(var, s1, s2, s3)
#define STAMP_ADD(slot, t0, t1)
#define STAMP_A(var, s1, s2)
#define STAMP_A_ADD(slot, t0, t1)
#define STAMP_M(var, s1, s2)
#define STAMP_M_ADD(slot, t0, t1)
#define STAMP_PARAM_OPT
#endif
```

alphazero_gym_amd/csrc/results.cuh:

```cuda
#pragma once
#include "records.h"
#include "tree.cuh"

template <bool CONT, int TLDS>
__device__ __forceinline__ void results_for_tree(const KParams& P, const TreeStore<TLDS>& ts, const Cold* cold, const float* action, size_t tb,
                                                 int tree, int sub) {
    typedef typename TreeStore<TLDS>::Rec Rec;
    const int Kmax = P.res_Kmax;
    const Rec root = ts.hot[0];
    const int nc = root.n_child;
    int tot_l = 0;
    double qmax_l = -__builtin_huge_val();
    for (int a = sub; a < Kmax; a += 16) {
        const int k = a < nc ? (CONT ? ts.child_at(0, root, a, P.Kp) : (int)root.first + a) : -1;
        const Rec h = ts.hot[k >= 0 ? k : 0];
        const size_t o = (size_t)tree * Kmax + a;
        P.res_actions[o] = k >= 0 ? (CONT ? action[k] : (float)a) : 0.0f;
        P.res_counts[o] = k >= 0 ? (int)h.edge_n : 0;
        P.res_Q[o] = k >= 0 ? h.Q : 0.0;
        const bool ex = k >= 0 && (h.flags & FLAG_EXPANDED);
        P.res_child_n[o] = ex ? (int)h.node_n : -1;
        for (int s2 = 0; s2 < P.S; ++s2) P.res_child_state[o * P.S + s2] = ex ? cold[k].s[s2] : 0.0;
        if (k >= 0) { tot_l += (int)h.edge_n; qmax_l = h.Q > qmax_l ? h.Q : qmax_l; }
    }
    for (int m = 1; m < 16; m <<= 1) {
        tot_l += __shfl_xor(tot_l, m, 16);
        const double o = __shfl_xor(qmax_l, m, 16);
        qmax_l = o > qmax_l ? o : qmax_l;
    }
    if (sub == 0) {
        const double qmax = nc > 0 ? qmax_l : 0.0;
        double onp = 0.0;
        if (P.res_v_target == AZG_VT_ON_POLICY) {
            auto kid = [&](int a) { return ts.hot[CONT ? ts.child_at(0, root, a, P.Kp) : (int)root.first + a]; };
            const long tot = tot_l;
            if (!CONT) {
                for (int a = 0; a < nc; ++a) { const Rec h = kid(a); onp += ((double)(int)h.edge_n / (double)tot) * h.Q; }
            } else {
                for (int a = 0; a < nc; ++a) {
                    const double qa = kid(a).Q;
                    for (int b2 = 0; b2 < nc; ++b2) onp += ((double)(int)kid(b2).edge_n / (double)tot) * qa;
                }
            }
        }
        P.res_vt[tree] = P.res_v_target == AZG_VT_ON_POLICY ? onp : qmax;
        P.res_nch[tree] = nc;
        P.res_root_V[tree] = cold[0].V;
    }
    if (CONT && P.ncomp >= 2) {
        for (int i = sub; i < 3 * P.ncomp; i += 16) {
            const int part = i / P.ncomp, c = i % P.ncomp;
            P.res_root_dist[(size_t)tree * 3 * P.ncomp + i] = P.gmm[tb * 3 * GMM_MAXC + part * GMM_MAXC + c];
        }
    } else if (CONT) {
        if (sub == 0) { P.res_root_dist[(size_t)tree * 2] = cold[0].mu; P.res_root_dist[(size_t)tree * 2 + 1] = cold[0].sg; }
    } else {
        for (int d = sub; d < P.nd; d += 16) P.res_root_dist[(size_t)tree * P.nd + d] = ts.prior[(int)root.first + d];
    }
}
```

alphazero_gym_amd/csrc/search_kernel.cuh:

```cuda
#pragma once
#include "records.h"
#include "env.cuh"
#include "mlp.cuh"
#include "tree.cuh"
#include "tree_phases.cuh"
#include "results.cuh"
#ifndef AZG_DEFER
#define AZG_DEFER 1
#endif

struct LdsLayout {
    size_t act_off;
    size_t tree_off;
    size_t per_tree;
    size_t state_off;
    size_t total;
};
__host__ __device__ inline LdsLayout lds_layout(int tab_n, int n_sims, int HP, int NG, int nbuf, int R, bool cont, int tlds, int lds_state = 0, int NT = 16) {
    LdsLayout L;
    L.act_off = ((size_t)tab_n * 8 + (size_t)(n_sims + 2) * 2 + 15) / 16 * 16;
    L.tree_off = L.act_off + (size_t)nbuf * NG * HP * 64;
    L.per_tree = (size_t)R * 16 + (cont ? (size_t)POOL_UNITS(R) * (tlds == TS_LDS9 ? 8 : 4) : (size_t)R * 4);
    L.per_tree = (L.per_tree + 15) / 16 * 16;
    L.state_off = 0;
    if (lds_state && !cont && tlds != TS_GLOBAL) { L.state_off = L.per_tree; L.per_tree += (size_t)(n_sims + 1) * 32; }
    L.total = L.tree_off + (tlds != TS_GLOBAL ? L.per_tree * NT * NG : 0);
    return L;
}
__host__ __device__ constexpr int act_buffers(int NREG) { return NREG == 1 ? 1 : 2; }

template <int ENV, int HP, int NREG, int TLDS, bool GMM, int NW, int NG, int NT = 16, int SPEC = 0>
__global__ __launch_bounds__(64 * NW, NT < 16 ? 2 : 1) void search_kernel(KParams P) {
    constexpr bool CONT = EnvFamily<ENV>::CONT;
    static_assert(NT == 16 || (NG == 1 && NW == 4 && (NT == 8 || NT == 4)), "half-filled tiles: one group, four waves");
    constexpr int TPW = NT * NG;
    constexpr int NWALK = (NW == 8 && NG == 1) ? 4 : NW;
    constexpr int TPV = TPW / NWALK;
    typedef typename TreeStore<TLDS>::Rec Rec;
    constexpr int NCH = head_chunks<HP>();
    constexpr int PSTR = GMM ? 64 : 16;
    __shared__ f32x4 s_parts[NG * NCH * PSTR];
    constexpr bool IN8 = EnvFamily<ENV>::IN8;
    __shared__ float s_obsT[(IN8 ? 8 : 4) * TPW];
    __shared__ float s_bhead[16];
    __shared__ float s_ln[NREG == 0 ? 2 * 64 : 1];
    __shared__ int s_done;
    constexpr bool DEFER = AZG_DEFER && NW == 8 && NG == 1 && ENV == AZG_ENV_PENDULUM_V1 && TLDS != TS_GLOBAL && NREG > 0 && !GMM && HP <= 256;
    __shared__ int s_l0;
    extern __shared__ double s_dyn[];

    const int tid = threadIdx.x;
    const int wave = tid >> 6, lane = tid & 63;
    const int wnet = (int)blockIdx.x / P.net_wgs;
    const int wj0 = ((int)blockIdx.x - wnet * P.net_wgs) * TPW;
    const int tree0 = wnet * P.net_T + wj0;
    const int n_live = (P.net_T - wj0) < TPW ? (P.net_T - wj0) : TPW;
    const size_t wofs = (size_t)wnet * P.net_wstride;
    constexpr bool LEAN = (NW == 8);
    const LdsLayout L = lds_layout(P.tab_n, P.n_sims, HP, NG, act_buffers(NREG), P.R, CONT, TLDS, P.lds_state, NT);
    double* s_sqrt = s_dyn;
    unsigned short* s_pw = (unsigned short*)(s_dyn + P.tab_n);
    f32x4* s_actA = (f32x4*)((char*)s_dyn + L.act_off);
    f32x4* s_actB = act_buffers(NREG) == 2 ? s_actA + NG * (HP / 16 * 64) : s_actA;
    for (int i = tid; i < P.tab_n; i += 64 * NW) s_sqrt[i] = P.sqrt_tab[i];
    if (CONT) for (int i = tid; i < P.n_sims + 2; i += 64 * NW) s_pw[i] = (unsigned short)(P.pw_need[i] < 65535 ? P.pw_need[i] : 65535);
    if (tid < 16) s_bhead[tid] = P.bhead[wofs + tid];
    if (tid == 0) { s_done = 0; s_l0 = 0; }

    typedef WRegs<HP, NREG, NW, DEFER> WR;
    WR wr;
    constexpr int NTW = HP / (16 * NW);
    if constexpr (DEFER) {
        if (wave >= NW / 2) {
#pragma unroll
            for (int i = 0; i < 2 * NTW; ++i) {
                wr.w0[i] = P.W0[wofs + ((wave - NW / 2) * 2 * NTW + i) * 64 + lane];
                wr.b0[i] = net_ptr(P.b0, wofs)[((wave - NW / 2) * 2 * NTW + i) * 64 + lane];
            }
        }
    } else if constexpr (HP <= 256) {
#pragma unroll
        for (int i = 0; i < NTW; ++i) {
            wr.w0[i] = P.W0[wofs + (wave * NTW + i) * 64 + lane];
            if constexpr (IN8) { if (P.in8) wr.w0b[i] = P.W0b[wofs + (wave * NTW + i) * 64 + lane]; }
            wr.b0[i] = net_ptr(P.b0, wofs)[(wave * NTW + i) * 64 + lane];
        }
    }
    if (NREG > 0) {
        constexpr int S4 = HP / 16;
#pragma unroll
        for (int l = 0; l < NREG; ++l) {
#pragma unroll
            for (int i = 0; i < NTW; ++i) {
                wr.b[l][i] = net_ptr(P.bl[l], wofs)[(wave * NTW + i) * 64 + lane];
#pragma unroll
                for (int s4 = 0; s4 < S4; ++s4) wr.w[l][i][s4] = net_ptr(P.Wl[l], wofs)[((wave * NTW + i) * S4 + s4) * 64 + lane];
            }
        }
#pragma unroll
        for (int i = 0; i < NTW; ++i) wr.wh[i] = net_ptr(P.Whead, wofs)[(wave * NTW + i) * 64 + lane];
    }

    struct Ctx {
        int sub, tl, tree; bool has_tree, live; unsigned gtree; size_t tb;
        Cold* cold; double* edge_W; float* action; TreeStore<TLDS> ts; const f32x4* my_parts;
    };
    auto make_ctx = [&](int t) {
        Ctx c;
        const int w = t >> 6, ln = t & 63;
        c.sub = ln & 15;
        c.has_tree = w < NWALK && (ln >> 4) < TPV;
        c.tl = c.has_tree ? w * TPV + (ln >> 4) : 0;
        c.tree = tree0 + c.tl;
        c.live = c.has_tree && c.tl < n_live;
        c.gtree = (unsigned)(P.tree_base + c.tree);
        c.tb = (size_t)(c.live ? c.tree : 0) * P.R;
        c.cold = P.cold + c.tb;
        c.edge_W = P.edge_W + c.tb;
        c.action = P.action + c.tb;
        if constexpr (TLDS != TS_GLOBAL) {
            char* base = (char*)s_dyn + L.tree_off + L.per_tree * c.tl;
            c.ts.hot = (Rec*)base;
            c.ts.pool = (typename TreeStore<TLDS>::PoolId*)(base + (size_t)P.R * 16);
            c.ts.prior = (float*)(base + (size_t)P.R * 16);
            c.ts.state = L.state_off ? (double*)(base + L.state_off) : nullptr;
        } else {
            c.ts.hot = (Rec*)(P.hot + c.tb);
            c.ts.child = P.child + c.tb * P.Kp;
            c.ts.prior = P.prior + c.tb;
        }
        c.my_parts = s_parts + (c.tl / NT) * NCH * PSTR;
        return c;
    };
    Ctx cx = make_ctx(tid);

#ifdef AZG_STAMPS
    unsigned long long st_acc[16] = {0, 0, 0, 0, 0, 0, 0, 0, 0, 0, 0, 0, 0, 0, 0, 0};
#endif
    TreeState st = {};
    st.need_eval = false;
    BDeferred bdef = {};
    if (cx.has_tree) tree_init_root<ENV, TLDS, TPW, IN8>(P, st, cx.ts, cx.cold, cx.edge_W, cx.action, cx.tree, cx.live, cx.sub, cx.tl, cx.gtree, s_obsT);
    __syncthreads();

    constexpr bool MULTI = !CONT;
    static_assert(!(LEAN && MULTI), "discrete 8-wave shapes: extend the LEAN packing first");
    int my_sim = -1;
    for (int sim = -1; sim < P.n_sims; ++sim) {
        STAMP2(t_a, 0, -1);
        __syncthreads();
        if constexpr (MULTI) { if (*(volatile int*)&s_done >= n_live) break; }
        STAMP2(t_b, 0, 1);
        if constexpr (DEFER) {
            STAMP2(t_b2a, 12, -1);
            if (cx.live) tree_phase_b2<ENV, TLDS, SPEC>(P, st, cx.ts, cx.cold, cx.edge_W, cx.action, bdef, cx.sub, cx.gtree, s_pw);
            bdef.pending = false;
            STAMP2(t_b2b, 12, -1);
#ifdef AZG_STAMP_ONLY
            STAMP_ADD(12, t_b2a, t_b2b);
#endif
        }
        unsigned pk0 = 0, pk1 = 0, pk2 = 0, pk3 = 0;
        int tid_o = tid;
        if constexpr (LEAN) {
            pk0 = (unsigned)st.nrec | ((unsigned)st.leaf << 16);
            pk1 = (unsigned)st.path_D | ((unsigned)st.kbase << 16);
            pk2 = (unsigned)(st.my_depth + 1) | ((unsigned)st.pid << 16);
            pk3 = (unsigned)st.ptop | ((unsigned)st.need_eval << 16) | ((unsigned)st.resume << 20);
            asm volatile("" : "+v"(pk0), "+v"(pk1), "+v"(pk2), "+v"(pk3));
        }
#ifdef AZG_STAMPS
        mlp_forward<HP, NREG, NW, NG, PSTR, WR, NT, IN8, DEFER>(P, wr, s_obsT, s_actA, s_actB, s_parts, s_ln, wave, lane, st_acc, &s_l0, sim + 2, wofs);
#else
        mlp_forward<HP, NREG, NW, NG, PSTR, WR, NT, IN8, DEFER>(P, wr, s_obsT, s_actA, s_actB, s_parts, s_ln, wave, lane, &s_l0, sim + 2, wofs);
#endif
        STAMP2(t_c, 1, 2);
        if constexpr (LEAN) {
            asm volatile("" : "+v"(pk0), "+v"(pk1), "+v"(pk2), "+v"(pk3), "+v"(tid_o));
            st.nrec = (int)(pk0 & 0xffffu); st.leaf = (int)(pk0 >> 16);
            st.path_D = (int)(pk1 & 0xffffu); st.kbase = (int)(pk1 >> 16);
            st.my_depth = (int)(pk2 & 0xffffu) - 1; st.pid = (int)(pk2 >> 16);
            st.ptop = (int)(pk3 & 0xffffu); st.need_eval = ((pk3 >> 16) & 1u) != 0; st.resume = (int)(pk3 >> 20);
            cx = make_ctx(tid_o);
            st.pr = 0.0; st.pW = 0.0;
            if (cx.live && (MULTI ? my_sim : sim) >= 0 && st.my_depth >= 1) {
                st.pr = CONT ? cx.cold[st.pid].r : discrete_env_reward(Spec<SPEC, ENV>::env(P));
                st.pW = cx.edge_W[st.pid];
            }
        }
        if constexpr (!MULTI) {
            if (cx.live) tree_phase_a<ENV, TLDS, GMM, NCH, PSTR, !CONT, SPEC>(P, st, cx.ts, cx.cold, cx.edge_W, cx.action, cx.tb, sim, cx.sub, cx.tl % NT, cx.gtree, cx.my_parts, s_bhead, s_sqrt STAMP_ARG, s_pw);
            if (sim == P.n_sims - 1) break;
            if constexpr (DEFER) { if (sim < 0 && cx.live) eps_prepare(P, st, cx.gtree, cx.sub); }
            tree_fence();
            STAMP2(t_d, 2, 3);
            st.need_eval = false;
            if (cx.live) tree_phase_b<ENV, TLDS, GMM, TPW, unsigned short, !LEAN, !CONT, SPEC, IN8, DEFER>(P, st, cx.ts, cx.cold, cx.edge_W, cx.action, cx.tb, cx.sub, cx.tl, cx.gtree, s_sqrt, s_pw, s_obsT STAMP_ARG, &bdef);
            tree_fence();
            STAMP2(t_e, 3, -1);
            STAMP_ADD(2, t_c, t_d);
            STAMP_ADD(3, t_d, t_e);
        } else {
            bool run = cx.live && my_sim < P.n_sims;
            int k = 0;
            while (run) {
                STAMP2(t_c2, 2, -1);
                tree_phase_a<ENV, TLDS, GMM, NCH, PSTR, !CONT, SPEC>(P, st, cx.ts, cx.cold, cx.edge_W, cx.action, cx.tb, my_sim, cx.sub, cx.tl % NT, cx.gtree, cx.my_parts, s_bhead, s_sqrt STAMP_ARG, s_pw);
                tree_fence();
                STAMP2(t_d, 2, 3);
                st.need_eval = false;
                if (my_sim == P.n_sims - 1) {
                    my_sim = P.n_sims;
                    if (cx.sub == 0) atomicAdd(&s_done, 1);
                    run = false;
                } else {
                    my_sim += 1;
                    tree_phase_b<ENV, TLDS, GMM, TPW, unsigned short, !LEAN, !CONT, SPEC, IN8>(P, st, cx.ts, cx.cold, cx.edge_W, cx.action, cx.tb, cx.sub, cx.tl, cx.gtree, s_sqrt, s_pw, s_obsT STAMP_ARG);
                    tree_fence();
                    k += 1;
                    if (st.need_eval || k >= P.trace_cap) run = false;
                }
                STAMP2(t_e, 3, -1);
                STAMP_ADD(2, t_c2, t_d);
                STAMP_ADD(3, t_d, t_e);
            }
        }
        STAMP_ADD(0, t_a, t_b);
        STAMP_ADD(1, t_b, t_c);
    }
    const int nrec = st.nrec;
    const int sub = cx.sub, tree = cx.tree;
    const bool live = cx.live;
    const size_t tb = cx.tb;
    const TreeStore<TLDS>& ts = cx.ts;
#ifdef AZG_STAMPS
    if (lane == 0) for (int i = 0; i < 16; ++i) P.stamps[((size_t)blockIdx.x * NW + wave) * 16 + i] = st_acc[i];
#endif
    if (live) results_for_tree<CONT, TLDS>(P, ts, cx.cold, cx.action, tb, tree, sub);
    if (live) {
        if (sub == 0) P.n_rec[tree] = nrec;
        if constexpr (TLDS != TS_GLOBAL) {
            if (P.publish) {
                RecL* gh = P.hot + tb;
                for (int j = sub; j < nrec; j += 16) {
                    Rec h = ts.hot[j];
                    RecL o;
                    o.Q = h.Q; o.edge_n = h.edge_n; o.node_n = h.node_n; o.parent = (short)h.parent; o.n_child = h.n_child;
                    o.first = CONT ? 0 : h.first; o.flags = h.flags; o.pad = 0;
                    gh[j] = o;
                    if (CONT) {
                        for (int i = 0; i < (int)h.n_child; ++i) P.child[(tb + j) * P.Kp + i] = (unsigned short)ts.child_at(j, h, i, P.Kp);
                    } else {
                        P.prior[tb + j] = ts.prior[j];
                    }
                }
            }
        }
    }
}
```

alphazero_gym_amd/csrc/team.cuh:

```cuda
#pragma once
#include "lockstep.cuh"

#define TEAM_CNT_STRIDE 32
#define TEAM_MAX_CNT 8
#define TEAM_CNT_XA (TEAM_MAX_CNT - 1)
#define TEAM_CNT_XB (TEAM_MAX_CNT - 2)
#ifndef TEAM_SPREAD
#define TEAM_SPREAD 1
#endif
#ifndef TEAM_SAME_XCD
#define TEAM_SAME_XCD 1
#endif
#ifndef TEAM_DEFER
#define TEAM_DEFER 1
#endif
#ifndef TEAM_LDS_COLD
#define TEAM_LDS_COLD 1
#endif
__host__ __device__ inline size_t team_cold_bytes(int R) { return ((size_t)R * (64 + 8 + 4) + 15) / 16 * 16; }
#ifndef TEAM_TILE_DBG
#define TEAM_TILE_DBG 0
#endif
#ifndef TEAM_WD
#define TEAM_WD 1
#endif
#if TEAM_WD
#define LS_TILE_STAGE_F4(KC, TG) (2 * (TG) * (KC) * 64)
#else
#define LS_TILE_STAGE_F4(KC, TG) (2 * (4 + (TG)) * (KC) * 64)
#endif

struct TeamCtl {
    unsigned* cnt;
    unsigned* abort;
    unsigned spin_limit;
};

__host__ __device__ inline size_t team_tree_bytes(int R, bool cont, int tlds) {
    if (tlds == TS_GLOBAL) return 0;
    size_t per = (size_t)R * 16 + (cont ? (size_t)POOL_UNITS(R) * (tlds == TS_LDS9 ? 8 : 4) : (size_t)R * 4);
    return (per + 15) / 16 * 16;
}
__host__ __device__ inline size_t team_table_off(int kc, int tg = 2) { size_t f4 = LS_TILE_STAGE_F4(kc, tg); return (f4 < 1024 ? 1024 : f4) * 16; }
__host__ __device__ inline size_t team_tree_off(int tab_n, int n_sims, int kc, int tg = 2) {
    return (team_table_off(kc, tg) + (size_t)tab_n * 8 + (size_t)(n_sims + 2) * 4 + 15) / 16 * 16;
}

__device__ __forceinline__ void team_arrive(unsigned* c) {
    asm volatile("s_waitcnt vmcnt(0)" ::: "memory");
    __syncthreads();
    if (threadIdx.x == 0) __hip_atomic_fetch_add(c, 1u, __ATOMIC_RELAXED, __HIP_MEMORY_SCOPE_AGENT);
}

__device__ __forceinline__ bool team_wait(const unsigned* c, unsigned target, const TeamCtl& T, volatile int* s_ok) {
    unsigned* abort = T.abort;
    if (threadIdx.x == 0) {
        int ok = 1;
        unsigned spins = 0;
        if (T.spin_limit == 0u) {
            __hip_atomic_store(abort, 1u, __ATOMIC_RELAXED, __HIP_MEMORY_SCOPE_AGENT);
            ok = 0;
        } else {
            while (__hip_atomic_load(c, __ATOMIC_RELAXED, __HIP_MEMORY_SCOPE_AGENT) < target) {
                __builtin_amdgcn_s_sleep(2);
                if ((++spins & 15u) == 0u) {
                    if (spins > T.spin_limit) __hip_atomic_store(abort, 1u, __ATOMIC_RELAXED, __HIP_MEMORY_SCOPE_AGENT);
                    if (__hip_atomic_load(abort, __ATOMIC_RELAXED, __HIP_MEMORY_SCOPE_AGENT) != 0u) { ok = 0; break; }
                }
            }
        }
        *s_ok = ok;
    }
    __syncthreads();
    const bool ok = *s_ok != 0;
    __syncthreads();
    return ok;
}

#ifdef AZG_STAMPS
#define TSTAMP(v) const unsigned long long v = __builtin_amdgcn_s_memtime()
#define TADD(slot, a, b) tacc[slot] += (b) - (a)
#else
#define TSTAMP(v)
#define TADD(slot, a, b)
#endif

template <int ENV, int HP, bool GMM, int TLDS, int KC = LS_KC, int MINB = 2, int SPEC = 0, int TT = 32>
__global__ __launch_bounds__(256, MINB) void ls_team_kernel(KParams P, LockStep L, TeamCtl T, int TQ, int g_base) {
    constexpr bool CONT = EnvFamily<ENV>::CONT;
    constexpr int NU = HP / 64, NCH = HP / 64, TGN = TT / 16;
    constexpr int TPW = TT / NU;
    static_assert(TT == 32 || TT == 64, "a team is two or four 16-tree groups");
    static_assert(TPW >= 1 && TPW <= 4, "a team is TT trees over HP/64 workgroups");
    typedef typename TreeStore<TLDS>::Rec Rec;
    extern __shared__ f32x4 s_ab[];
    __shared__ float s_obs[32];
    __shared__ int s_ok;
    double* s_sqrt = (double*)((char*)s_ab + team_table_off(KC, TGN));
    int* s_pw = (int*)(s_sqrt + P.tab_n);
    const int tid = threadIdx.x, wave = tid >> 6, lane = tid & 63, sub = lane & 15;
    int tq, us;
#if TEAM_SPREAD
    if (NU % 8 == 0) { const int x = blockIdx.x % 8, j = blockIdx.x / 8, sp = NU / 8; tq = j / sp; us = x * sp + j % sp; }
    else
#endif
    if (TQ % 8 == 0) { const int x = blockIdx.x % 8, j = blockIdx.x / 8; tq = x * (TQ / 8) + j / NU; us = j % NU; }
    else { tq = blockIdx.x / NU; us = blockIdx.x % NU; }
    const int g0 = g_base + TGN * tq;
    unsigned* cnt = T.cnt + (size_t)(g0 / 2) * TEAM_MAX_CNT * TEAM_CNT_STRIDE;
    const int n_layers = P.n_hidden - 1;

    const int tj = lane >> 4;
    const bool has_tree = wave == 0 && tj < TPW;
    const int tt = us * TPW + (has_tree ? tj : 0);
    const int tree = g0 * 16 + tt;
    const bool live = has_tree && tree < P.B;
    const unsigned gtree = (unsigned)(P.tree_base + tree);
    const size_t tb = (size_t)(live ? tree : 0) * P.R;
    Cold* cold = P.cold + tb;
    double* edge_W = P.edge_W + tb;
    float* action = P.action + tb;
    TreeStore<TLDS> ts;
    if constexpr (TLDS != TS_GLOBAL) {
        char* base = (char*)s_ab + team_tree_off(P.tab_n, P.n_sims, KC, TGN) + team_tree_bytes(P.R, CONT, TLDS) * (has_tree ? tj : 0);
        ts.hot = (Rec*)base;
        ts.pool = (typename TreeStore<TLDS>::PoolId*)(base + (size_t)P.R * 16);
        ts.prior = (float*)(base + (size_t)P.R * 16);
        ts.state = nullptr;
    } else {
        ts.hot = (Rec*)(P.hot + tb);
        ts.child = P.child + tb * P.Kp;
        ts.prior = P.prior + tb;
    }
    constexpr bool LDS_COLD = TEAM_LDS_COLD && HP == 1024 && TT == 32 && MINB == 2 && TLDS == TS_LDS8;
    if constexpr (LDS_COLD) {
        char* cb = (char*)s_ab + team_tree_off(P.tab_n, P.n_sims, KC, TGN) + team_tree_bytes(P.R, CONT, TLDS) * TPW + team_cold_bytes(P.R) * (has_tree ? tj : 0);
        cold = (Cold*)cb;
        edge_W = (double*)(cb + (size_t)P.R * 64);
        action = (float*)(cb + (size_t)P.R * 72);
    }
    TreeState st = {};
    constexpr bool BDEF = TEAM_DEFER && ENV == AZG_ENV_PENDULUM_V1 && !GMM && TT == 32;
    BDeferred bdef = {};
    bool wt = true;
    if (tid == 0) {
        const unsigned xcc = __builtin_amdgcn_s_getreg((4 - 1) << 11 | 0 << 6 | 20) & 7u;
        __hip_atomic_fetch_max(cnt + TEAM_CNT_XA * TEAM_CNT_STRIDE, xcc, __ATOMIC_RELAXED, __HIP_MEMORY_SCOPE_AGENT);
        __hip_atomic_fetch_max(cnt + TEAM_CNT_XB * TEAM_CNT_STRIDE, 7u - xcc, __ATOMIC_RELAXED, __HIP_MEMORY_SCOPE_AGENT);
    }
    const TileMem<true> parts_mem(L.parts);
    for (int i = tid; i < P.tab_n; i += 256) s_sqrt[i] = P.sqrt_tab[i];
    if (CONT) for (int i = tid; i < P.n_sims + 2; i += 256) s_pw[i] = P.pw_need[i];
    if (tid < 32) s_obs[tid] = 0.0f;
    __syncthreads();
    const TileMem<true> act0(L.act[0], true);
    auto first_layer = [&](bool wt_now) {
        constexpr int TPT = 256 / TPW;
        constexpr int UPT = HP / TPT;
        const int j = tid / TPT, u0 = (tid % TPT) * UPT;
        static_assert(UPT % 4 == 0, "whole float4s of units per thread");
        const int c = us * TPW + j;
        const float x0 = s_obs[0 * TPW + j], x1 = s_obs[1 * TPW + j], x2 = s_obs[2 * TPW + j], x3 = s_obs[3 * TPW + j];
        TileMem<true> out = act0;
        out.wt = wt_now;
#pragma unroll
        for (int h = 0; h < UPT / 4; ++h) {
            const int u = u0 + 4 * h;
            f32x4 acc = P.b0u[u / 4];
            const f32x4 wa = P.W0u[u], wb = P.W0u[u + 1], wc = P.W0u[u + 2], wd = P.W0u[u + 3];
            acc.x = __builtin_fmaf(wa.x, x0, acc.x); acc.x = __builtin_fmaf(wa.y, x1, acc.x); acc.x = __builtin_fmaf(wa.z, x2, acc.x); acc.x = __builtin_fmaf(wa.w, x3, acc.x);
            acc.y = __builtin_fmaf(wb.x, x0, acc.y); acc.y = __builtin_fmaf(wb.y, x1, acc.y); acc.y = __builtin_fmaf(wb.z, x2, acc.y); acc.y = __builtin_fmaf(wb.w, x3, acc.y);
            acc.z = __builtin_fmaf(wc.x, x0, acc.z); acc.z = __builtin_fmaf(wc.y, x1, acc.z); acc.z = __builtin_fmaf(wc.z, x2, acc.z); acc.z = __builtin_fmaf(wc.w, x3, acc.z);
            acc.w = __builtin_fmaf(wd.x, x0, acc.w); acc.w = __builtin_fmaf(wd.y, x1, acc.w); acc.w = __builtin_fmaf(wd.z, x2, acc.w); acc.w = __builtin_fmaf(wd.w, x3, acc.w);
            out.store4(((size_t)(g0 + c / 16) * (HP / 16) + u / 16) * 64 + ((u % 16) / 4) * 16 + c % 16, act4<true>(P.act, acc));
        }
    };
#ifdef TEAM_STAGGER
    if ((blockIdx.x >= gridDim.x / 2) && tid == 0) {
        const unsigned long long t0 = __builtin_amdgcn_s_memtime();
        while (__builtin_amdgcn_s_memtime() - t0 < (unsigned long long)(TEAM_STAGGER)) __builtin_amdgcn_s_sleep(8);
    }
    __syncthreads();
#endif
    if (has_tree) tree_init_root<ENV, TLDS, TPW>(P, st, ts, cold, edge_W, action, tree, live, sub, tj, gtree, s_obs);
    __syncthreads();
    first_layer(true);
    team_arrive(cnt);
#ifdef AZG_STAMPS
    unsigned long long tacc[8] = {0, 0, 0, 0, 0, 0, 0, 0};
    unsigned long long st_acc[16] = {0, 0, 0, 0, 0, 0, 0, 0, 0, 0, 0, 0, 0, 0, 0, 0};
#endif
    TSTAMP(t_begin);
    for (int k = 0; k <= P.n_sims; ++k) {
        const int sim = k - 1;
        TSTAMP(t0);
        if (!team_wait(cnt, (unsigned)(NU * (k + 1)), T, &s_ok)) return;
        TSTAMP(t1);
        TADD(0, t0, t1);
        if (TEAM_SAME_XCD && k == 0) {
            if (tid == 0)
                s_ok = __hip_atomic_load(cnt + TEAM_CNT_XA * TEAM_CNT_STRIDE, __ATOMIC_RELAXED, __HIP_MEMORY_SCOPE_AGENT) +
                       __hip_atomic_load(cnt + TEAM_CNT_XB * TEAM_CNT_STRIDE, __ATOMIC_RELAXED, __HIP_MEMORY_SCOPE_AGENT) == 7u;
            __syncthreads();
            wt = s_ok == 0;
            __syncthreads();
        }
        for (int l = 1; l <= n_layers; ++l) {
            const int in_buf = (l - 1) & 1;
            TSTAMP(ta);
#if TEAM_WD
            if (l == n_layers) ls_tile_wd<HP, true, TGN, true, KC>(P, L, l, in_buf, us, g0, s_ab, wt);
            else ls_tile_wd<HP, false, TGN, true, KC>(P, L, l, in_buf, us, g0, s_ab, wt);
#else
            if (l == n_layers) ls_tile<HP, true, TGN, 4, true, KC, TEAM_TILE_DBG>(P, L, l, in_buf, us, g0, s_ab, wt);
            else ls_tile<HP, false, TGN, 4, true, KC, TEAM_TILE_DBG>(P, L, l, in_buf, us, g0, s_ab, wt);
#endif
            TSTAMP(tb_);
            team_arrive(cnt + l * TEAM_CNT_STRIDE);
            if (!team_wait(cnt + l * TEAM_CNT_STRIDE, (unsigned)(NU * (k + 1)), T, &s_ok)) return;
            TSTAMP(tc);
            TADD(l < 3 ? l : 3, ta, tb_);
            TADD(l < n_layers ? 4 : 5, tb_, tc);
        }
        TSTAMP(te);
        for (int i = tid; i < NCH * 4 * TPW; i += 256) {
            const int w = i / (4 * TPW), q = (i / TPW) % 4, j = i % TPW, c = us * TPW + j;
            s_ab[w * 64 + q * 16 + j] = parts_mem.load4(((size_t)(g0 + c / 16) * NCH + w) * 64 + q * 16 + c % 16);
        }
        __syncthreads();
        TSTAMP(tp0);
        __builtin_amdgcn_s_setprio(3);
        if (live) tree_phase_a<ENV, TLDS, GMM, NCH, 64, false, SPEC>(P, st, ts, cold, edge_W, action, tb, sim, sub, tj, gtree, s_ab, P.bhead, s_sqrt STAMP_ARG, s_pw);
        st.need_eval = false;
        TSTAMP(tp1);
        if constexpr (BDEF) { if (k == 0 && live) eps_prepare(P, st, gtree, sub); }
        if (k < P.n_sims) {
            tree_fence();
            if (live) tree_phase_b<ENV, TLDS, GMM, TPW, int, true, false, SPEC, false, BDEF>(P, st, ts, cold, edge_W, action, tb, sub, tj, gtree, s_sqrt, s_pw, s_obs STAMP_ARG, &bdef);
        }
        __builtin_amdgcn_s_setprio(0);
        TSTAMP(tp2);
#ifdef AZG_STAMPS
        st_acc[0] += tp0 - te; st_acc[1] += tp1 - tp0; st_acc[2] += tp2 - tp1;
#endif
        if (k < P.n_sims) {
            __syncthreads();
            first_layer(wt);
            team_arrive(cnt);
            if constexpr (BDEF) {
                if (live) tree_phase_b2<ENV, TLDS, SPEC, true>(P, st, ts, cold, edge_W, action, bdef, sub, gtree, s_pw);
                bdef.pending = false;
            }
        }
        TSTAMP(tf);
        TADD(6, te, tf);
#ifdef AZG_STAMPS
        st_acc[3] += tf - tp2;
#endif
    }
    if (live) {
        if (sub == 0) P.n_rec[tree] = st.nrec;
        if constexpr (TLDS != TS_GLOBAL) {
            RecL* gh = P.hot + tb;
            for (int j = sub; j < st.nrec; j += 16) {
                Rec h = ts.hot[j];
                RecL o;
                o.Q = h.Q; o.edge_n = h.edge_n; o.node_n = h.node_n; o.parent = (short)h.parent; o.n_child = h.n_child;
                o.first = CONT ? 0 : h.first; o.flags = h.flags; o.pad = 0;
                gh[j] = o;
                if (CONT) {
                    for (int i = 0; i < (int)h.n_child; ++i) P.child[(tb + j) * P.Kp + i] = (unsigned short)ts.child_at(j, h, i, P.Kp);
                } else {
                    P.prior[tb + j] = ts.prior[j];
                }
            }
        }
        if constexpr (LDS_COLD) {
            for (int j = sub; j < st.nrec; j += 16) { P.cold[tb + j] = cold[j]; P.edge_W[tb + j] = edge_W[j]; P.action[tb + j] = action[j]; }
        }
    }
#ifdef AZG_STAMPS
    TSTAMP(t_end);
    TADD(7, t_begin, t_end);
#ifdef TEAM_CENSUS
    tacc[0] = (unsigned long long)__builtin_amdgcn_s_getreg((32 - 1) << 11 | 0 << 6 | 4) | ((unsigned long long)__builtin_amdgcn_s_getreg((4 - 1) << 11 | 0 << 6 | 20) << 32) |
              ((unsigned long long)blockIdx.x << 40);
#endif
    if (tid == 0) {
        for (int i = 0; i < 8; ++i) P.stamps[((size_t)tq * NU + us) * 8 + i] = tacc[i];
        for (int i = 0; i < 16; ++i) P.stamps[(size_t)gridDim.x * 8 + ((size_t)tq * NU + us) * 16 + i] = st_acc[i];
    }
#endif
}
```

alphazero_gym_amd/csrc/tree.cuh:

```cuda
#pragma once
#include "records.h"

__device__ __forceinline__ void tree_fence() { __builtin_amdgcn_fence(__ATOMIC_ACQ_REL, "wavefront"); }

__device__ __forceinline__ double tree_div(double n, double d) {
    double r = __builtin_amdgcn_rcp(d);
    double e = __builtin_fma(-d, r, 1.0);
    r = __builtin_fma(r, e, r);
    e = __builtin_fma(-d, r, 1.0);
    r = __builtin_fma(r, e, r);
    double q = n * r;
    double rem = __builtin_fma(-d, q, n);
    return __builtin_fma(rem, r, q);
}


template <int CTRL>
__device__ __forceinline__ int dpp_i32(int v) { return __builtin_amdgcn_update_dpp(0, v, CTRL, 0xf, 0xf, false); }
template <int CTRL>
__device__ __forceinline__ double dpp_f64(double v) {
    unsigned long long u = azg_d2u(v);
    unsigned lo = (unsigned)dpp_i32<CTRL>((int)(unsigned)u), hi = (unsigned)dpp_i32<CTRL>((int)(unsigned)(u >> 32));
    return azg_u2d(((unsigned long long)hi << 32) | lo);
}
template <int CTRL>
__device__ __forceinline__ float dpp_f32(float v) { return __builtin_bit_cast(float, dpp_i32<CTRL>(__builtin_bit_cast(int, v))); }
#define DPP_QUAD_BCAST1 0x55
#define DPP_QUAD_XOR1 0xB1
#define DPP_QUAD_XOR2 0x4E
#define DPP_ROW_ROR4 0x124
#define DPP_ROW_ROR8 0x128
#define DPP_ROW_ROR15 0x12F

__device__ __forceinline__ double rowmax16(double u, bool valid) {
    double m = valid ? u : -__builtin_huge_val();
    double o;
    o = dpp_f64<DPP_QUAD_XOR1>(m); m = o > m ? o : m;
    o = dpp_f64<DPP_QUAD_XOR2>(m); m = o > m ? o : m;
    o = dpp_f64<DPP_ROW_ROR4>(m); m = o > m ? o : m;
    o = dpp_f64<DPP_ROW_ROR8>(m); m = o > m ? o : m;
    return m;
}
__device__ __forceinline__ int rowmin16(int c) {
    int t;
    t = dpp_i32<DPP_QUAD_XOR1>(c); c = t < c ? t : c;
    t = dpp_i32<DPP_QUAD_XOR2>(c); c = t < c ? t : c;
    t = dpp_i32<DPP_ROW_ROR4>(c); c = t < c ? t : c;
    t = dpp_i32<DPP_ROW_ROR8>(c); c = t < c ? t : c;
    return c;
}
__device__ __forceinline__ int argmax16(double u, bool valid, int sub) {
    double m = rowmax16(u, valid);
    return rowmin16((valid && u == m) ? sub : 99);
}
__device__ __forceinline__ int rowmax16_i32(int v) {
    int o;
    o = dpp_i32<DPP_QUAD_XOR1>(v); v = o > v ? o : v;
    o = dpp_i32<DPP_QUAD_XOR2>(v); v = o > v ? o : v;
    o = dpp_i32<DPP_ROW_ROR4>(v); v = o > v ? o : v;
    o = dpp_i32<DPP_ROW_ROR8>(v); v = o > v ? o : v;
    return v;
}
__device__ __forceinline__ unsigned rowmax16_u32(unsigned v) {
    unsigned o;
    o = (unsigned)dpp_i32<DPP_QUAD_XOR1>((int)v); v = o > v ? o : v;
    o = (unsigned)dpp_i32<DPP_QUAD_XOR2>((int)v); v = o > v ? o : v;
    o = (unsigned)dpp_i32<DPP_ROW_ROR4>((int)v); v = o > v ? o : v;
    o = (unsigned)dpp_i32<DPP_ROW_ROR8>((int)v); v = o > v ? o : v;
    return v;
}
__device__ __forceinline__ int argmax16_payload(double u, bool valid, int sub, int payload) {
    const long long bits = (long long)azg_d2u(u);
    const long long key = bits ^ ((bits >> 63) & 0x7fffffffffffffffLL);
    const int hi = valid ? (int)(key >> 32) : (int)0x80000000;
    const unsigned lo = (unsigned)key;
    const int mh = rowmax16_i32(hi);
    const bool top = valid && hi == mh;
    const unsigned ml = rowmax16_u32(top ? lo : 0u);
    return rowmin16((top && lo == ml) ? ((sub << 16) | payload) : 0x7fffffff) & 0xffff;
}

#define DPP_QUAD_BCAST0 0x00
__device__ __forceinline__ int argmax2_payload(double u, int sub, int payload) {
    const double o = dpp_f64<DPP_QUAD_XOR1>(u);
    const int po = dpp_i32<DPP_QUAD_XOR1>(payload);
    int w = (sub == 0) ? (u >= o ? payload : po) : 0;
    w = dpp_i32<DPP_QUAD_BCAST0>(w);
    int t = dpp_i32<DPP_ROW_ROR4>(w); w = t > w ? t : w;
    t = dpp_i32<DPP_ROW_ROR8>(w); w = t > w ? t : w;
    return w;
}

template <int TLDS> struct TreeStore;
template <typename RecT, typename IdT> struct TreeStoreLds {
    typedef RecT Rec;
    typedef IdT PoolId;
    Rec* hot; IdT* pool; float* prior;
    double* state;
    __device__ __forceinline__ int child_at(int, const Rec& hp, int i, int) const {
        return hp.n_child == 1 ? (int)hp.first : (int)pool[4 * (int)hp.cbase + i];
    }
    __device__ __forceinline__ void child_append(int p, const Rec& hp, int K, int id, int& ptop, bool writer, int, bool wnext = false) const {
        const int cb = hp.cbase;
        if (K == 0) {
            if (writer) hot[p].first = (decltype(hp.first))id;
        } else if (K == 1 || K == 4 || K == 8) {
            const int nb = ptop;
            ptop += K == 1 ? 1 : K / 2;
            if (writer) {
                if (K == 1) pool[4 * nb] = (IdT)hp.first;
                else for (int w = 0; w < K; ++w) pool[4 * nb + w] = pool[4 * cb + w];
                pool[4 * nb + K] = (IdT)id;
                hot[p].cbase = (decltype(hp.cbase))nb;
            }
        } else {
            if (writer) pool[4 * cb + K] = (IdT)id;
        }
        if (writer) { hot[p].n_child = (decltype(hp.n_child))(K + 1); hot[p].wnext = wnext ? 1 : 0; }
    }
};
template <> struct TreeStore<TS_LDS8> : TreeStoreLds<RecS, unsigned char> {};
template <> struct TreeStore<TS_LDS9> : TreeStoreLds<RecM, unsigned short> {};
template <> struct TreeStore<TS_GLOBAL> {
    typedef RecL Rec;
    Rec* hot; unsigned short* child; float* prior;
    static constexpr double* state = nullptr;
    __device__ __forceinline__ int child_at(int p, const Rec&, int i, int Kp) const { return (int)child[p * Kp + i]; }
    __device__ __forceinline__ void child_append(int p, const Rec&, int K, int id, int&, bool writer, int Kp, bool wnext = false) const {
        if (writer) {
            child[p * Kp + K] = (unsigned short)id;
            hot[p].n_child = (unsigned short)(K + 1);
            hot[p].pad = wnext ? 1 : 0;
        }
    }
};

__device__ __forceinline__ bool get_wnext(const RecS& h) { return h.wnext != 0; }
__device__ __forceinline__ bool get_wnext(const RecM& h) { return h.wnext != 0; }
__device__ __forceinline__ bool get_wnext(const RecL& h) { return (h.pad & 1) != 0; }
__device__ __forceinline__ void set_wnext(RecS& h, bool w) { h.wnext = w ? 1 : 0; }
__device__ __forceinline__ void set_wnext(RecM& h, bool w) { h.wnext = w ? 1 : 0; }
__device__ __forceinline__ void set_wnext(RecL& h, bool w) { h.pad = w ? 1 : 0; }
template <typename PW>
__device__ __forceinline__ int pw_at(const PW* s_pw, int n, int cap) { return (int)s_pw[n < cap ? n : cap]; }

template <typename Rec>
__device__ __forceinline__ Rec make_edge(double Q, int parent) {
    Rec h;
    h.Q = Q; h.edge_n = 0; h.node_n = 0; h.parent = (decltype(h.parent))parent; h.n_child = 0; h.flags = 0; h.first = 0;
    set_wnext(h, false);
    return h;
}
__device__ __forceinline__ void clear_pad(RecS& h) { h.cbase = 0; }
__device__ __forceinline__ void clear_pad(RecM& h) { h.cbase = 0; }
__device__ __forceinline__ void clear_pad(RecL& h) { h.pad = 0; }

template <bool CONT, int TLDS, typename F, typename PW = int>
__device__ __forceinline__ void backup_from(const TreeStore<TLDS>& ts, const Cold* cold, double* edge_W, int j, float V, int sub,
                                            float gamma_f, double gamma, bool firstlvl, bool at_leaf, double Rv, F&& on_node,
                                            const PW* s_pw = nullptr, int pw_cap = 0) {
    typedef typename TreeStore<TLDS>::Rec Rec;
    while (true) {
        int mine = 0, cnt = 0, jj = j;
        bool hit_root = false;
#pragma unroll 1
        for (int d = 0; d < 16; ++d) {
            if (sub == d) mine = jj;
            cnt = d + 1;
            if (jj == 0) { hit_root = true; break; }
            jj = ts.hot[jj].parent;
        }
        Rec mrec = ts.hot[mine];
        const bool is_edge = (sub < cnt) && (mine != 0);
        double r = 0.0, W = 0.0;
        if (is_edge) { r = cold[mine].r; W = edge_W[mine]; }
        double myR = 0.0;
        const int nedge = hit_root ? cnt - 1 : cnt;
#pragma unroll 1
        for (int d = 0; d < nedge; ++d) {
            double rd = __shfl(r, d, 16);
            double gR;
            if (firstlvl) {
                gR = CONT ? (double)(gamma_f * V) : gamma * (double)V;
                firstlvl = false;
            } else {
                gR = gamma * Rv;
            }
            Rv = rd + gR;
            if (sub == d) myR = Rv;
        }
        if (sub < cnt) {
            if (is_edge) {
                int en = (int)mrec.edge_n + 1;
                double Wn = W + myR;
                mrec.Q = tree_div(Wn, (double)en);
                mrec.edge_n = (decltype(mrec.edge_n))en;
                edge_W[mine] = Wn;
            }
            if (!(at_leaf && sub == 0)) {
                mrec.node_n = (decltype(mrec.node_n))(mrec.node_n + 1);
                if constexpr (CONT) set_wnext(mrec, pw_at(s_pw, (int)mrec.node_n, pw_cap) - (int)mrec.n_child > 0);
            }
            ts.hot[mine] = mrec;
        }
        if (!TLDS) tree_fence();
        for (int d = 0; d < cnt; ++d) {
            const int pn = __shfl(mine, d, 16);
            if (!(at_leaf && d == 0)) on_node(pn);
        }
        if (hit_root) break;
        j = jj;
        at_leaf = false;
    }
}

template <bool CONT, int TLDS, typename F, typename PW = int>
__device__ __forceinline__ void backup_path(const TreeStore<TLDS>& ts, const Cold* cold, double* edge_W, float V, int sub, float gamma_f,
                                            double gamma, int D, int my_depth, int pid, double pr, double& pW, F&& on_node,
                                            typename TreeStore<TLDS>::Rec& rec, double& chainR, bool same_chain = false,
                                            double r_uniform = 0.0, double r_first = 0.0, const PW* s_pw = nullptr, int pw_cap = 0) {
    typedef typename TreeStore<TLDS>::Rec Rec;
    const int n0 = D < 16 ? D : 16;
    double Rv = 0.0, myR = 0.0;
    if (same_chain) {
        myR = chainR;
    } else if constexpr (!CONT) {
        double R = 0.0;
        if (gamma == 1.0) {
            const float av = __builtin_fabsf(V);
            if (av == 0.0f || (av >= 0x1p-25f && av < 0x1p30f)) {
                const int dl = (D - sub) & 15;
                if (dl < n0) myR = (r_first + (double)dl * r_uniform) + (double)V;
                R = n0 > 0 ? (r_first + (double)(n0 - 1) * r_uniform) + (double)V : (double)V;
            } else {
                R = (double)V;
#pragma unroll 2
                for (int d = 0; d < n0; ++d) {
                    R = (d == 0 ? r_first : r_uniform) + R;
                    if (sub == ((D - d) & 15)) myR = R;
                }
            }
        } else {
#pragma unroll 2
            for (int d = 0; d < n0; ++d) {
                const double gR = d == 0 ? gamma * (double)V : gamma * R;
                R = (d == 0 ? r_first : r_uniform) + gR;
                if (sub == ((D - d) & 15)) myR = R;
            }
        }
        Rv = R;
        chainR = myR;
    } else {
#pragma unroll 1
        for (int d = 0; d < n0; ++d) {
            const int src = (D - d) & 15;
            const double nb = dpp_f64<DPP_ROW_ROR15>(myR);
            const double gR = d == 0 ? (CONT ? (double)(gamma_f * V) : gamma * (double)V) : gamma * nb;
            if (sub == src) myR = pr + gR;
        }
        chainR = myR;
    }
    if (CONT && D >= 16) Rv = __shfl(myR, (D - 15) & 15, 16);
    const bool valid = my_depth >= 0 && my_depth > D - 16;
    int par = 0;
    rec = make_edge<Rec>(0.0, 0);
    clear_pad(rec);
    if (valid) {
        rec = ts.hot[pid];
        int need = 0;
        if constexpr (CONT) { if (my_depth < D) need = pw_at(s_pw, (int)rec.node_n + 1, pw_cap); }
        par = rec.parent;
        if (my_depth >= 1) {
            int en = (int)rec.edge_n + 1;
            double Wn = pW + myR;
            rec.Q = tree_div(Wn, (double)en);
            rec.edge_n = (decltype(rec.edge_n))en;
            edge_W[pid] = Wn;
            pW = Wn;
        }
        if (my_depth < D) {
            rec.node_n = (decltype(rec.node_n))(rec.node_n + 1);
            if constexpr (CONT) set_wnext(rec, need - (int)rec.n_child > 0);
        }
        ts.hot[pid] = rec;
    }
    if (D >= 16) {
        int j = __shfl(par, (D - 15) & 15, 16);
        backup_from<CONT, TLDS>(ts, cold, edge_W, j, V, sub, gamma_f, gamma, false, false, Rv, on_node, s_pw, pw_cap);
    }
}
```

alphazero_gym_amd/csrc/tree_phases.cuh:

```cuda
#pragma once
#ifndef EARLY_COLD
#define EARLY_COLD 1
#endif
#include "records.h"
#include "env.cuh"
#include "mlp.cuh"
#include "tree.cuh"

struct TreeState {
    int nrec;
    unsigned eps_draws;
    int leaf;
    bool need_eval;
    int path_D;
    int my_depth, pid;
    double pr, pW;
    int kbase;
    float eps_c;
    float eps_next;
    int ptop;
    int resume;
    double chainR;
    bool repeat;
};

template <int SPEC, int ENV = AZG_ENV_CARTPOLE> struct Spec {
    static __device__ __forceinline__ bool eps0(const KParams& P) { return SPEC ? true : P.epsilon == 0.0; }
    static __device__ __forceinline__ bool tie_random(const KParams& P) { return SPEC ? false : P.tie_random != 0; }
    static __device__ __forceinline__ bool plain(const KParams& P) { return SPEC ? true : (P.epsilon == 0.0 && !P.tie_random); }
    static __device__ __forceinline__ int A(const KParams& P) { return ENV == AZG_ENV_ACROBOT ? 3 : (SPEC ? 2 : P.A); }
    static __device__ __forceinline__ int env(const KParams& P) {
        return ENV == AZG_ENV_ACROBOT ? (int)AZG_ENV_ACROBOT : (SPEC ? (int)AZG_ENV_CARTPOLE : P.env_id);
    }
    static __device__ __forceinline__ int v1(const KParams& P) { return SPEC ? 1 : P.v1; }
    static __device__ __forceinline__ bool in_table(const KParams& P, int n) { return SPEC ? true : n < P.tab_n; }
};

template <bool CONT> __device__ __forceinline__ int rec_best(const RecS& h) { return CONT ? (int)h.first : (int)h.first + (int)h.cbase; }
template <bool CONT> __device__ __forceinline__ int rec_best(const RecM& h) { return CONT ? (int)h.first : (int)h.first + (int)h.cbase; }
template <bool CONT> __device__ __forceinline__ int rec_best(const RecL& h) { return CONT ? (int)h.first : (int)h.first + (int)h.pad; }
template <bool CONT> __device__ __forceinline__ void set_best(RecS* r, const RecS& h, int c) {
    if (CONT) r->first = (unsigned char)c; else r->cbase = (unsigned char)(c - (int)h.first);
}
template <bool CONT> __device__ __forceinline__ void set_best(RecM* r, const RecM& h, int c) {
    if (CONT) r->first = (unsigned)c; else r->cbase = (unsigned)(c - (int)h.first);
}
template <bool CONT> __device__ __forceinline__ void set_best(RecL* r, const RecL& h, int c) {
    if (CONT) r->first = (unsigned short)c; else r->pad = (unsigned char)(c - (int)h.first);
}

template <int ENV, int TLDS, typename Rec, int SPEC = 0>
__device__ __forceinline__ int select_child(const KParams& P, const TreeStore<TLDS>& ts, int p, const Rec& hp, int sub, const double* s_sqrt,
                                            int pick, unsigned gtree = 0u) {
    constexpr bool CONT = EnvFamily<ENV>::CONT;
    const int K = hp.n_child;
    double sq;
    if (CONT || Spec<SPEC, ENV>::in_table(P, (int)hp.node_n)) sq = s_sqrt[hp.node_n];
    else sq = __builtin_sqrt((double)((int)hp.node_n + 1));
    int win_c = 0;
    if (TLDS || K <= 16) {
        const bool valid = sub < K;
        const int si = valid ? sub : 0;
        int c = CONT ? ts.child_at(p, hp, si, P.Kp) : (int)hp.first + si;
        if (!valid) c = 0;
        Rec h = ts.hot[c];
        double ratio = tree_div(sq, (double)((int)h.edge_n + 1));
        double U;
        if (CONT) {
            U = h.Q + P.c_uct * ratio;
        } else {
            float pc = ts.prior[c] * P.c_uct_f;
            U = h.Q + (double)pc * ratio;
        }
        if (!SPEC && pick >= 0) win_c = __shfl(c, pick, 16);
        else if (!CONT && K == 2) win_c = argmax2_payload(U, sub, c);
        else win_c = argmax16_payload(U, valid, sub, c);
        if (Spec<SPEC, ENV>::tie_random(P) && pick < 0) {
            const double m = rowmax16(U, valid);
            const unsigned row = (unsigned)(__ballot(valid && U == m) >> (threadIdx.x & 48)) & 0xffffu;
            const int cnt = __popc(row);
            if (cnt > 1) {
                const azg_u32x4 b = azg_draw(P.seed, gtree, P.search_idx, ((unsigned)hp.node_n << 16) ^ (unsigned)p, AZG_STREAM_TIE);
                int kth = (int)(b.v[0] % (unsigned)cnt);
                unsigned r2 = row;
                while (kth-- > 0) r2 &= r2 - 1;
                win_c = __shfl(c, __builtin_ctz(r2), 16);
            }
        }
    } else {
        double win_u = 0.0;
        bool have = false;
        for (int base = 0; base < K; base += 16) {
            const int i = base + sub;
            const bool valid = i < K;
            int c = 0;
            double U = 0.0;
            if (valid) {
                c = CONT ? ts.child_at(p, hp, i, P.Kp) : (int)hp.first + i;
                Rec h = ts.hot[c];
                double ratio = tree_div(sq, (double)((int)h.edge_n + 1));
                if (CONT) {
                    U = h.Q + P.c_uct * ratio;
                } else {
                    float pc = ts.prior[c] * P.c_uct_f;
                    U = h.Q + (double)pc * ratio;
                }
            }
            int w;
            if (pick >= 0) w = (pick >= base && pick < base + 16) ? pick - base : -1;
            else w = argmax16(U, valid, sub);
            if (w >= 0) {
                int wc = __shfl(c, w, 16);
                double wu = __shfl(U, w, 16);
                if (pick >= 0 || !have || wu > win_u) { win_c = wc; win_u = wu; have = true; }
            }
        }
    }
    return win_c;
}

template <int ENV, int TLDS, int SPEC = 0>
__device__ __forceinline__ void refresh_best(const KParams& P, const TreeStore<TLDS>& ts, int p, int sub, const double* s_sqrt) {
    constexpr bool CONT = EnvFamily<ENV>::CONT;
    typedef typename TreeStore<TLDS>::Rec Rec;
    const Rec hp = ts.hot[p];
    const int b = select_child<ENV, TLDS, Rec, SPEC>(P, ts, p, hp, sub, s_sqrt, -1);
    if (sub == 0) set_best<CONT>(&ts.hot[p], hp, b);
}

template <int ENV, int TLDS, int SPEC = 0>
__device__ __forceinline__ int refresh_best_own_slot(const KParams& P, const TreeStore<TLDS>& ts, int pid, bool mine, const double* s_sqrt,
                                                     const typename TreeStore<TLDS>::Rec& hp) {
    typedef typename TreeStore<TLDS>::Rec Rec;
    const int p = mine ? pid : 0;
    double sq;
    if (Spec<SPEC, ENV>::in_table(P, (int)hp.node_n)) sq = s_sqrt[hp.node_n];
    else sq = __builtin_sqrt((double)((int)hp.node_n + 1));
    const int c0 = (int)hp.first;
    const Rec h0 = ts.hot[c0], h1 = ts.hot[c0 + 1];
    const float pc0 = ts.prior[c0] * P.c_uct_f, pc1 = ts.prior[c0 + 1] * P.c_uct_f;
    const double U0 = h0.Q + (double)pc0 * tree_div(sq, (double)((int)h0.edge_n + 1));
    const double U1 = h1.Q + (double)pc1 * tree_div(sq, (double)((int)h1.edge_n + 1));
    const int win = c0 + (U0 >= U1 ? 0 : 1);
    if (mine) set_best<false>(&ts.hot[p], hp, win);
    return win;
}

template <int ENV, int TLDS, int TPW = 16, bool OBS8 = false>
__device__ __forceinline__ void tree_init_root(const KParams& P, TreeState& st, const TreeStore<TLDS>& ts, Cold* cold, double* edge_W,
                                               float* action, int tree, bool live, int sub, int tl, unsigned gtree, float* obsT) {
    constexpr bool CONT = EnvFamily<ENV>::CONT;
    constexpr int S = CONT ? 2 : 4;
    typedef typename TreeStore<TLDS>::Rec Rec;
    st.nrec = 1; st.eps_draws = 0; st.leaf = 0; st.need_eval = live;
    st.path_D = 0; st.my_depth = -1; st.pid = 0; st.pr = 0.0; st.pW = 0.0;
    st.kbase = 1; st.eps_c = 0.0f; st.eps_next = 0.0f; st.ptop = 0; st.resume = 0; st.chainR = 0.0; st.repeat = false;
    if (CONT && live) st.eps_c = azg_normal(P.seed, gtree, P.search_idx, (unsigned)(st.kbase + sub));
        double rs[S], sn;
#pragma unroll
        for (int k = 0; k < S; ++k) rs[k] = (live && k < P.S) ? P.roots[(size_t)tree * P.S + k] : 0.0;
        float obs[OBS8 ? 8 : 4];
        if constexpr (OBS8) { sn = 0.0; azg_acrobot_obs(rs, obs); obs[6] = 0.0f; obs[7] = 0.0f; }
        else env_obs<ENV == AZG_ENV_ACROBOT ? AZG_ENV_CARTPOLE : ENV>(rs, obs, &sn);
        if (live && sub == 0) {
            Rec h = make_edge<Rec>(0.0, 0);
            h.node_n = (decltype(h.node_n))P.carry[tree];
            h.flags = FLAG_EXPANDED;
            clear_pad(h);
            if (CONT) set_wnext(h, pw_at(P.pw_need, (int)P.carry[tree], P.n_sims + 1) > 0);
            ts.hot[0] = h;
            Cold c;
#pragma unroll
            for (int k = 0; k < 4; ++k) c.s[k] = k < S ? rs[k] : 0.0;
            if (CONT) c.s[2] = sn;
            c.r = 0.0; c.V = 0.0f; c.mu = 0.0f; c.sg = 0.0f; c.pad = 0.0f;
            cold[0] = c;
            edge_W[0] = 0.0;
            if (CONT) action[0] = 0.0f;
            if constexpr (!CONT && TLDS != TS_GLOBAL) {
                if (ts.state) {
#pragma unroll
                    for (int k = 0; k < 4; ++k) ts.state[k] = rs[k];
                }
            }
        }
        if constexpr (!OBS8) {
            if (sub < 4) obsT[sub * TPW + tl] = live ? obs[sub] : 0.0f;
        } else if (sub < 8) {
            float v = sub == 0 ? obs[0] : (sub == 1 ? obs[1] : (sub == 2 ? obs[2] : obs[3]));
            if (sub >= 4) v = sub == 4 ? obs[4] : (sub == 5 ? obs[5] : (sub == 6 ? obs[6] : obs[7]));
            obsT[sub * TPW + tl] = live ? v : 0.0f;
        }
}

template <int ENV, int TLDS, bool GMM, int NCH, int PSTR = 64, bool RESUME = false, int SPEC = 0, typename PW = int>
__device__ __forceinline__ void tree_phase_a(const KParams& P, TreeState& st, const TreeStore<TLDS>& ts, Cold* cold, double* edge_W,
                                             float* action, size_t tb, int sim, int sub, int tl, unsigned gtree, const f32x4* parts,
                                             const float* bhead, const double* s_sqrt STAMP_PARAM_OPT, const PW* s_pw = nullptr) {
    constexpr bool CONT = EnvFamily<ENV>::CONT;
    typedef typename TreeStore<TLDS>::Rec Rec;
    float V = 0.0f;
    STAMP_A(ta0, 4, -1);
    if (st.need_eval) {
        f32x4 out4 = {0.0f, 0.0f, 0.0f, 0.0f};
        if constexpr (!CONT) { out4 = head_output4<NCH, PSTR>(parts, bhead, tl); V = out4.x; }
        else V = head_output<NCH, PSTR>(parts, bhead, tl, 0);
        if (CONT) {
            float mu, sg;
            float gd[15];
            if constexpr (GMM) {
                gmm_params<NCH, PSTR>(parts, bhead, tl, P.ncomp, P.ls_min, P.ls_max, gd);
                mu = gd[0]; sg = gd[GMM_MAXC];
                float* g = P.gmm + (tb + st.leaf) * 3 * GMM_MAXC;
                if (sub == 0) {
#pragma unroll
                    for (int i = 0; i < 3 * GMM_MAXC; ++i) g[i] = gd[i];
                }
            } else {
                mu = head_output<NCH, PSTR>(parts, bhead, tl, 1);
                float ls = head_output<NCH, PSTR>(parts, bhead, tl, 2);
                ls = ls < P.ls_min ? P.ls_min : (ls > P.ls_max ? P.ls_max : ls);
                sg = azg_expf(ls);
            }
            if (sub == 0) { cold[st.leaf].V = V; cold[st.leaf].mu = mu; cold[st.leaf].sg = sg; }
            if (sim < 0) {
                int k = st.nrec++;
                if constexpr (GMM) gmm_pick(gd, P.ncomp, P.seed, gtree, P.search_idx, (unsigned)k, &mu, &sg);
                float eps = __shfl(st.eps_c, k - st.kbase, 16);
                float a = P.bound_f * azg_tanhf(mu + sg * eps);
                if (sub == 0) {
                    Rec h = make_edge<Rec>((double)V, 0);
                    clear_pad(h);
                    ts.hot[k] = h;
                    edge_W[k] = 0.0;
                    action[k] = a;
                }
                ts.child_append(0, make_edge<Rec>(0.0, 0), 0, k, st.ptop, sub == 0, P.Kp,
                                pw_at(P.pw_need, (int)ts.hot[0].node_n, P.n_sims + 1) - 1 > 0);
            }
        } else {
            const int A = Spec<SPEC, ENV>::A(P);
            float my_logit = sub == 0 ? out4.y : (sub == 1 ? out4.z : out4.w);
            if (A > 3 && sub >= 3 && sub < A) my_logit = head_output<NCH, PSTR>(parts, bhead, tl, 1 + sub);
            float mx = out4.y;
            if (A == 2) {
                mx = out4.z > mx ? out4.z : mx;
            } else {
                for (int a = 1; a < A; ++a) { const float v = __shfl(my_logit, a, 16); mx = v > mx ? v : mx; }
            }
            const float e_mine = azg_expf(my_logit - mx);
            float sum;
            if (A == 2) {
                sum = dpp_f32<DPP_QUAD_BCAST0>(e_mine) + dpp_f32<DPP_QUAD_BCAST1>(e_mine);
            } else {
                sum = 0.0f;
                for (int a = 0; a < A; ++a) sum = sum + __shfl(e_mine, a, 16);
            }
            int k0 = st.nrec;
            st.nrec += A;
            if (sub < A) {
                float prior_a = e_mine / sum;
                Rec h = make_edge<Rec>((double)V, st.leaf);
                clear_pad(h);
                ts.hot[k0 + sub] = h;
                ts.prior[k0 + sub] = prior_a;
                edge_W[k0 + sub] = 0.0;
            }
            if (sub == 0) {
                cold[st.leaf].V = V;
                ts.hot[st.leaf].n_child = (decltype(ts.hot[st.leaf].n_child))A;
                ts.hot[st.leaf].first = (decltype(ts.hot[st.leaf].first))k0;
            }
            if (Spec<SPEC, ENV>::plain(P)) {
                if (A == 2) {
                    const int nn = (int)ts.hot[st.leaf].node_n;
                    double sq;
                    if (Spec<SPEC, ENV>::in_table(P, nn)) sq = s_sqrt[nn];
                    else sq = __builtin_sqrt((double)(nn + 1));
                    float prior_s = 0.0f;
                    if (sub < A) prior_s = e_mine / sum;
                    const float pc = prior_s * P.c_uct_f;
                    const double U = (double)V + (double)pc * sq;
                    const double o = dpp_f64<DPP_QUAD_XOR1>(U);
                    if (sub == 0) set_best<false>(&ts.hot[st.leaf], make_edge<Rec>(0.0, 0), U >= o ? 0 : 1);
                } else {
                    if (!TLDS) tree_fence();
                    refresh_best<ENV, TLDS, SPEC>(P, ts, st.leaf, sub, s_sqrt);
                }
            }
        }
    }
    STAMP_A(ta1, 4, 5);
    STAMP_A_ADD(4, ta0, ta1);
    if (sim >= 0) {
        if (!TLDS) tree_fence();
        const bool keep = !CONT && Spec<SPEC, ENV>::plain(P);
        Rec myrec;
        backup_path<CONT, TLDS>(ts, cold, edge_W, V, sub, P.gamma_f, P.gamma, st.path_D, st.my_depth, st.pid, st.pr, st.pW,
                                [&](int pn) { if (keep) refresh_best<ENV, TLDS, SPEC>(P, ts, pn, sub, s_sqrt); }, myrec, st.chainR,
                                RESUME && !CONT && st.repeat,
                                CONT ? 0.0 : discrete_env_reward(Spec<SPEC, ENV>::env(P)),
                                CONT ? 0.0 : (st.need_eval ? discrete_env_reward(Spec<SPEC, ENV>::env(P)) : discrete_env_terminal_reward(Spec<SPEC, ENV>::env(P))),
                                s_pw, P.n_sims + 1);
        STAMP_A(ta2, 5, 6);
        STAMP_A_ADD(5, ta1, ta2);
        if constexpr (!CONT) {
            if (keep) {
                const int D = st.path_D, lo = D > 15 ? D - 15 : 0;
                if (!TLDS) tree_fence();
                if (Spec<SPEC, ENV>::A(P) == 2) {
                    const bool mine = st.my_depth >= lo && st.my_depth < D;
                    const int win = refresh_best_own_slot<ENV, TLDS, SPEC>(P, ts, st.pid, mine, s_sqrt, myrec);
                    if constexpr (RESUME) {
                        const int next_pid = dpp_i32<DPP_ROW_ROR15>(st.pid);
                        const unsigned long long votes = __ballot(mine && win != next_pid);
                        const unsigned row = (unsigned)(votes >> (threadIdx.x & 48)) & 0xffffu;
                        st.resume = D < 16 ? (row ? __builtin_ctz(row) : D) : 0;
                    }
                } else {
                    for (int d = D - 1; d >= lo; --d) refresh_best<ENV, TLDS, SPEC>(P, ts, __shfl(st.pid, d & 15, 16), sub, s_sqrt);
                }
            }
        }
        STAMP_A(ta3, 6, -1);
        STAMP_A_ADD(6, ta2, ta3);
    }
}

__device__ __forceinline__ void eps_prepare(const KParams& P, TreeState& st, unsigned gtree, int sub) {
    if (st.nrec >= st.kbase + 16) {
        st.kbase = st.nrec;
        st.eps_c = azg_normal(P.seed, gtree, P.search_idx, (unsigned)(st.kbase + sub));
    }
    st.eps_next = __shfl(st.eps_c, st.nrec - st.kbase, 16);
}

struct BDeferred {
    bool pending, widen;
    int p, chosen;
    float cact;
};

template <int ENV, int TLDS, int SPEC, bool FETCH = false, typename PW = int>
__device__ __forceinline__ void tree_phase_b2(const KParams& P, TreeState& st, const TreeStore<TLDS>& ts, Cold* cold, double* edge_W, float* action,
                                              const BDeferred& d, int sub, unsigned gtree, const PW* s_pw) {
    typedef typename TreeStore<TLDS>::Rec Rec;
    static_assert(ENV == AZG_ENV_PENDULUM_V1, "deferred expansion: the Pendulum family");
    if (!d.pending) return;
    const double ps0 = cold[d.p].s[0], ps1 = cold[d.p].s[1];
    if (d.widen) {
        const float V = cold[d.p].V;
        const Rec hp = ts.hot[d.p];
        if (sub == 0) {
            Rec h = make_edge<Rec>((double)V, d.p);
            h.flags = FLAG_EXPANDED;
            clear_pad(h);
            set_wnext(h, P.pw0 > 0);
            ts.hot[d.chosen] = h;
            edge_W[d.chosen] = 0.0;
            action[d.chosen] = d.cact;
        }
        ts.child_append(d.p, hp, (int)hp.n_child, d.chosen, st.ptop, sub == 0, P.Kp,
                        pw_at(s_pw, (int)hp.node_n, P.n_sims + 1) - ((int)hp.n_child + 1) > 0);
    } else if (sub == 0) {
        Rec h = ts.hot[d.chosen];
        h.flags = FLAG_EXPANDED;
        set_wnext(h, P.pw0 > 0);
        ts.hot[d.chosen] = h;
    }
    const double sp[2] = {ps0, ps1};
    const double r = pendulum_reward(sp, d.cact) / P.reward_scale;
    if constexpr (FETCH) { if (sub == (st.path_D & 15)) st.pr = r; }
    if (sub == 0) {
        float zero = 0.0f;
        asm volatile("" : "+v"(zero));
        Cold* c = cold + d.chosen;
        c->s[3] = 0.0; c->r = r; c->V = zero; c->mu = zero; c->sg = zero; c->pad = zero;
    }
    eps_prepare(P, st, gtree, sub);
}

template <int ENV, int TLDS, bool GMM, int TPW = 16, typename PW = int, bool FETCH = true, bool RESUME = false, int SPEC = 0, bool OBS8 = false, bool DEFER = false>
__device__ __forceinline__ void tree_phase_b(const KParams& P, TreeState& st, const TreeStore<TLDS>& ts, Cold* cold, double* edge_W,
                                             float* action, size_t tb, int sub, int tl, unsigned gtree, const double* s_sqrt,
                                             const PW* s_pw, float* obsT STAMP_PARAM, BDeferred* def = nullptr) {
    static_assert(!DEFER || (ENV == AZG_ENV_PENDULUM_V1 && !GMM), "deferred expansion: Pendulum family, squashed-Normal head");
    constexpr bool CONT = EnvFamily<ENV>::CONT;
    constexpr int S = CONT ? 2 : 4;
    typedef typename TreeStore<TLDS>::Rec Rec;
    st.need_eval = false;
    if (CONT && !DEFER && st.nrec >= st.kbase + 16) {
        st.kbase = st.nrec;
        st.eps_c = azg_normal(P.seed, gtree, P.search_idx, (unsigned)(st.kbase + sub));
    }
    int p = 0;
    bool resumed = false;
    st.repeat = false;
    if constexpr (RESUME && !CONT) {
        if (Spec<SPEC, ENV>::plain(P) && Spec<SPEC, ENV>::A(P) == 2 && st.resume > 0) {
            resumed = true;
            p = __shfl(st.pid, st.resume, 16);
            if (st.my_depth > st.resume) st.my_depth = -1;
            st.path_D = st.resume;
        }
    }
    const double r_step = CONT ? 0.0 : discrete_env_reward(Spec<SPEC, ENV>::env(P));
    const bool keep_slot = !CONT && FETCH && resumed && st.my_depth >= 1;
    Rec hp = ts.hot[p];
    Cold cp;
    bool from_cold = true;
    if constexpr (!CONT && TLDS != TS_GLOBAL) from_cold = (ts.state == nullptr);
    if (from_cold) cp = cold[p];
    else { cp.s[0] = cp.s[1] = cp.s[2] = cp.s[3] = 0.0; }
    if (!resumed) { st.path_D = 0; st.my_depth = sub == 0 ? 0 : -1; st.pid = 0; }
    if (!keep_slot) { st.pr = 0.0; st.pW = 0.0; }
    int chosen = 0;
    bool widen = false, hit_terminal = false;
    if constexpr (RESUME && !CONT) {
        hit_terminal = resumed && (hp.flags & FLAG_TERMINAL);
        st.repeat = FETCH && hit_terminal;
    }
    STAMP2(tb0, 13, -1);
    while (!hit_terminal) {
        STAMP3(tl0, 7, 8, 11);
        const int K = hp.n_child;
        if (CONT) {
            widen = get_wnext(hp);
            if (widen) break;
        }
        if (CONT || !Spec<SPEC, ENV>::plain(P)) {
            int pick = -1;
            if (!Spec<SPEC, ENV>::eps0(P)) {
                azg_u32x4 b = azg_draw(P.seed, gtree, P.search_idx, st.eps_draws++, AZG_STREAM_EPS);
                if ((double)azg_u01(b.v[0]) < P.epsilon) pick = (int)(b.v[1] % (unsigned)K);
            }
            chosen = select_child<ENV, TLDS, Rec, SPEC>(P, ts, p, hp, sub, s_sqrt, pick, gtree);
        } else {
            chosen = rec_best<CONT>(hp);
        }
        STAMP2(tl1, 7, -1);
        STAMP_ADD(7, tl0, tl1);
        STAMP2(tl2, 8, 9);
        Cold cn;
        if constexpr (CONT && EARLY_COLD) cn = cold[chosen];
        Rec hc = ts.hot[chosen];
        if (!(hc.flags & FLAG_EXPANDED)) break;
        STAMP2(tl3, 9, 10);
        st.path_D += 1;
        p = chosen;
        hp = hc;
        if (sub == (st.path_D & 15)) {
            st.my_depth = st.path_D; st.pid = chosen;
            if (CONT && FETCH) { st.pr = EARLY_COLD ? cn.r : cold[chosen].r; st.pW = edge_W[chosen]; }
            if (!CONT && FETCH) { st.pr = r_step; st.pW = edge_W[chosen]; }
        }
        if constexpr (EnvFamily<ENV>::TERM) {
            if (hc.flags & FLAG_TERMINAL) { hit_terminal = true; break; }
        }
        if (CONT) { if constexpr (EARLY_COLD) cp = cn; else cp = cold[p]; }
        else if (from_cold) { cp.s[0] = cold[p].s[0]; cp.s[1] = cold[p].s[1]; cp.s[2] = cold[p].s[2]; cp.s[3] = cold[p].s[3]; }
        STAMP2(tl4, 10, 11);
        STAMP_ADD(8, tl0, tl2);
        STAMP_ADD(9, tl2, tl3);
        STAMP_ADD(10, tl3, tl4);
        STAMP_ADD(11, tl0, tl4);
#if defined(AZG_STAMPS) && !defined(AZG_STAMP_ONLY)
        st_acc[12] += 1;
#endif
    }
    STAMP2(tb1, 13, 14);
    STAMP_ADD(13, tb0, tb1);
    if (hit_terminal) {
        st.leaf = p;
    } else {
        float cact = 0.0f;
        if (widen) {
            const int K = hp.n_child;
            chosen = st.nrec++;
            float eps = DEFER ? st.eps_next : __shfl(st.eps_c, chosen - st.kbase, 16);
            float wmu = cp.mu, wsg = cp.sg;
            if constexpr (GMM) {
                float gd[15];
                const float* g = P.gmm + (tb + p) * 3 * GMM_MAXC;
#pragma unroll
                for (int i = 0; i < 3 * GMM_MAXC; ++i) gd[i] = g[i];
                gmm_pick(gd, P.ncomp, P.seed, gtree, P.search_idx, (unsigned)chosen, &wmu, &wsg);
            }
            cact = P.bound_f * azg_tanhf(wmu + wsg * eps);
            if constexpr (!DEFER) {
                if (sub == 0) {
                    Rec h = make_edge<Rec>((double)cp.V, p);
                    clear_pad(h);
                    ts.hot[chosen] = h;
                    edge_W[chosen] = 0.0;
                    action[chosen] = cact;
                }
                ts.child_append(p, hp, K, chosen, st.ptop, sub == 0, P.Kp, pw_at(s_pw, (int)hp.node_n, P.n_sims + 1) - (K + 1) > 0);
            }
        }
        STAMP2(tw1, 14, 15);
        STAMP_ADD(14, tb1, tw1);
        st.path_D += 1;
        double ns[S], r, sn;
        int done;
        if (CONT) {
            if (!widen) cact = action[chosen];
            if constexpr (DEFER) {
                pendulum_dynamics(Spec<SPEC, ENV>::v1(P), cp.s, cp.s[2], cact, ns);
                r = 0.0; done = 0;
            } else {
                if constexpr (ENV == AZG_ENV_MOUNTAINCAR_CONT) mountaincar_cont_step(cp.s, cact, ns, &r, &done);
                else pendulum_step(Spec<SPEC, ENV>::v1(P), cp.s, cp.s[2], cact, ns, &r, &done);
                r = r / P.reward_scale;
            }
        } else {
            if constexpr (TLDS != TS_GLOBAL) {
                if (ts.state) {
                    const int slot = Spec<SPEC, ENV>::A(P) == 2 ? ((int)hp.first - 1) >> 1 : ((int)hp.first - 1) / P.A;
                    const double* sp = ts.state + 4 * slot;
                    cp.s[0] = sp[0]; cp.s[1] = sp[1]; cp.s[2] = sp[2]; cp.s[3] = sp[3];
                }
            }
            family_env_step<ENV>(Spec<SPEC, ENV>::env(P), cp.s, chosen - (int)hp.first, ns, &r, &done);
        }
        float obs[OBS8 ? 8 : 4];
        if constexpr (OBS8) { sn = 0.0; azg_acrobot_obs(ns, obs); obs[6] = 0.0f; obs[7] = 0.0f; }
        else env_obs<ENV == AZG_ENV_ACROBOT ? AZG_ENV_CARTPOLE : ENV>(ns, obs, &sn);
        STAMP2(tw2, 15, -1);
        STAMP_ADD(15, tw1, tw2);
        if constexpr (DEFER) {
            def->pending = true; def->widen = widen; def->p = p; def->chosen = chosen; def->cact = cact;
            if (sub == 0) { cold[chosen].s[0] = ns[0]; cold[chosen].s[1] = ns[1]; cold[chosen].s[2] = sn; }
        } else if (sub == 0) {
            Cold c;
#pragma unroll
            for (int k = 0; k < 4; ++k) c.s[k] = k < S ? ns[k] : 0.0;
            if (CONT) c.s[2] = sn;
            float zero = 0.0f;
            asm volatile("" : "+v"(zero));
            c.r = r; c.V = zero; c.mu = zero; c.sg = zero; c.pad = zero;
            cold[chosen] = c;
            if constexpr (CONT) {
                Rec hn = ts.hot[chosen];
                hn.flags = (unsigned char)(FLAG_EXPANDED | (done ? FLAG_TERMINAL : 0));
                set_wnext(hn, P.pw0 > 0);
                ts.hot[chosen] = hn;
            } else {
                ts.hot[chosen].flags = (unsigned char)(FLAG_EXPANDED | (done ? FLAG_TERMINAL : 0));
            }
            if constexpr (!CONT && TLDS != TS_GLOBAL) {
                if (ts.state && !done) {
                    double* sp = ts.state + 4 * (Spec<SPEC, ENV>::A(P) == 2 ? (st.nrec - 1) >> 1 : (st.nrec - 1) / P.A);
#pragma unroll
                    for (int k = 0; k < 4; ++k) sp[k] = ns[k];
                }
            }
        }
        if (sub == (st.path_D & 15)) { st.my_depth = st.path_D; st.pid = chosen; st.pr = r; st.pW = 0.0; }
        st.leaf = chosen;
        st.need_eval = !done;
        if constexpr (!OBS8) {
            if (sub < 4) obsT[sub * TPW + tl] = done ? 0.0f : obs[sub];
        } else if (sub < 8) {
            float v = sub == 0 ? obs[0] : (sub == 1 ? obs[1] : (sub == 2 ? obs[2] : obs[3]));
            if (sub >= 4) v = sub == 4 ? obs[4] : (sub == 5 ? obs[5] : (sub == 6 ? obs[6] : obs[7]));
            obsT[sub * TPW + tl] = done ? 0.0f : v;
        }
    }
}
```

Before: 548.9 million sims/s.

## Split per-node Cold record into Widen, EdgeG, V and s3 arrays

Measured after the change: 533.2 million sims/s. -2.9%, worse.

```diff
diff --git a/alphazero_gym_amd/csrc/aux_kernels.cuh b/alphazero_gym_amd/csrc/aux_kernels.cuh
--- a/alphazero_gym_amd/csrc/aux_kernels.cuh
+++ b/alphazero_gym_amd/csrc/aux_kernels.cuh
@@ -15,8 +15,8 @@
     ts.hot = P.hot + tb;
     ts.child = P.child + tb * P.Kp;
     ts.prior = P.prior + tb;
-    if (P.mode == AZG_MODE_CONTINUOUS) results_for_tree<true, TS_GLOBAL>(P, ts, P.cold + tb, P.action + tb, tb, tree, sub);
-    else results_for_tree<false, TS_GLOBAL>(P, ts, P.cold + tb, P.action + tb, tb, tree, sub);
+    if (P.mode == AZG_MODE_CONTINUOUS) results_for_tree<true, TS_GLOBAL>(P, ts, cold_global(P, tb), P.action + tb, tb, tree, sub);
+    else results_for_tree<false, TS_GLOBAL>(P, ts, cold_global(P, tb), P.action + tb, tb, tree, sub);
 }
 
 
diff --git a/alphazero_gym_amd/csrc/azg_engine.hip b/alphazero_gym_amd/csrc/azg_engine.hip
--- a/alphazero_gym_amd/csrc/azg_engine.hip
+++ b/alphazero_gym_amd/csrc/azg_engine.hip
@@ -194,12 +194,13 @@
     HIPCHK(e, hipEventCreate(&e->ev1));
     KParams& P = e->P;
     const size_t B = (size_t)cfg->n_trees, R = (size_t)e->R, K = (size_t)e->Kmax;
-    RecL* hot; Cold* cold; double* edge_W; float* action; float* prior; unsigned short* child; int* n_rec;
+    RecL* hot; Widen* widen; EdgeG* edge; float* nodeV; double* s3; float* action; float* prior; unsigned short* child; int* n_rec;
     int* d_pw; double* d_sq; unsigned long long* stamps;
     e->res = ResultsLayout(B, K);
     e->stamp_n = stamp_rows(B);
     DeviceAllocs& mem = e->mem;
-    if (dalloc(e, mem, &hot, B * R) || dalloc(e, mem, &cold, B * R) || dalloc(e, mem, &edge_W, B * R) || dalloc(e, mem, &action, B * R) ||
+    if (dalloc(e, mem, &hot, B * R) || dalloc(e, mem, &widen, B * R) || dalloc(e, mem, &edge, B * R) || dalloc(e, mem, &nodeV, B * R) ||
+        dalloc(e, mem, &s3, cfg->mode == AZG_MODE_CONTINUOUS ? 1 : B * R) || dalloc(e, mem, &action, B * R) ||
         dalloc(e, mem, &prior, B * R) || dalloc(e, mem, &child, B * R * e->Kp) || dalloc(e, mem, &n_rec, B) ||
         dalloc(e, mem, &d_pw, (size_t)ns + 2) || dalloc(e, mem, &d_sq, (size_t)e->tab_n) || dalloc(e, mem, &e->d_roots, B * e->S_env) ||
         dalloc(e, mem, &e->d_carry, B) || dalloc(e, mem, &e->d_res_block, e->res.bytes) || dalloc(e, mem, &e->d_child_n, B * K) ||
@@ -223,7 +224,7 @@
     P.c_uct_f = (float)cfg->c_uct; P.gamma_f = (float)cfg->gamma; P.bound_f = (float)cfg->action_bound;
     P.seed = cfg->seed; P.S = e->S_env; P.tab_n = e->tab_n; P.pw0 = cfg->mode == AZG_MODE_CONTINUOUS ? pw[0] : 0;
     P.roots = e->d_roots; P.carry = e->d_carry;
-    P.hot = hot; P.cold = cold; P.edge_W = edge_W; P.action = action; P.prior = prior; P.child = child;
+    P.hot = hot; P.widen = widen; P.edge = edge; P.V = nodeV; P.s3 = s3; P.action = action; P.prior = prior; P.child = child;
     P.n_rec = n_rec; P.pw_need = d_pw; P.sqrt_tab = d_sq; P.stamps = stamps;
     P.res_actions = e->d_actions; P.res_counts = e->d_counts; P.res_Q = e->d_Q; P.res_vt = e->d_vt; P.res_nch = e->d_nch;
     P.res_child_n = e->d_child_n; P.res_child_state = e->d_child_state; P.res_root_V = e->d_rootV; P.res_root_dist = e->d_rootdist;
@@ -478,35 +479,17 @@
     }
     size_t B = e->cfg.n_trees, R = e->R;
     std::vector<RecL> hot(B * R);
-    std::vector<Cold> cold(B * R);
+    std::vector<EdgeG> edge(B * R);
+    std::vector<float> nV(B * R);
     std::vector<int> nrec(B);
-    std::vector<double> ew(B * R);
     std::vector<float> ac(B * R);
     HIPCHK(e, hipMemcpy(hot.data(), e->P.hot, B * R * sizeof(RecL), hipMemcpyDeviceToHost));
-    HIPCHK(e, hipMemcpy(cold.data(), e->P.cold, B * R * sizeof(Cold), hipMemcpyDeviceToHost));
+    HIPCHK(e, hipMemcpy(edge.data(), e->P.edge, B * R * sizeof(EdgeG), hipMemcpyDeviceToHost));
+    HIPCHK(e, hipMemcpy(nV.data(), e->P.V, B * R * 4, hipMemcpyDeviceToHost));
     HIPCHK(e, hipMemcpy(nrec.data(), e->P.n_rec, B * 4, hipMemcpyDeviceToHost));
-    HIPCHK(e, hipMemcpy(ew.data(), e->P.edge_W, B * R * 8, hipMemcpyDeviceToHost));
     HIPCHK(e, hipMemcpy(ac.data(), e->P.action, B * R * 4, hipMemcpyDeviceToHost));
-    const bool cont = e->cfg.mode == AZG_MODE_CONTINUOUS;
-    const int A = e->cfg.num_actions;
-    for (size_t i = 0; i < B; ++i) {
-        if (n_records) n_records[i] = nrec[i];
-        for (size_t j = 0; j < R; ++j) {
-            size_t o = i * R + j;
-            bool in = (int)j < nrec[i];
-            const RecL& h = hot[o];
-            bool ex = in && (h.flags & FLAG_EXPANDED);
-            if (parent) parent[o] = in ? (j == 0 ? -1 : h.parent) : 0;
-            if (edge_n) edge_n[o] = in ? h.edge_n : 0;
-            if (edge_W) edge_W[o] = in ? ew[o] : 0.0;
-            if (edge_Q) edge_Q[o] = in ? h.Q : 0.0;
-            if (edge_action) edge_action[o] = in ? (cont ? ac[o] : (j == 0 ? 0.0f : (float)((j - 1) % A))) : 0.0f;
-            if (node_n) node_n[o] = in ? h.node_n : 0;
-            if (node_r) node_r[o] = ex ? cold[o].r : 0.0;
-            if (node_V) node_V[o] = ex ? cold[o].V : 0.0f;
-            if (node_flags) node_flags[o] = in ? h.flags : 0;
-        }
-    }
+    dump_fill(B, R, e->cfg.mode == AZG_MODE_CONTINUOUS, e->cfg.num_actions, nrec.data(), hot.data(), edge.data(), nV.data(), ac.data(),
+              n_records, parent, edge_n, edge_W, edge_Q, edge_action, node_n, node_r, node_V, node_flags);
     return AZG_OK;
 }
 
diff --git a/alphazero_gym_amd/csrc/engine_host.h b/alphazero_gym_amd/csrc/engine_host.h
--- a/alphazero_gym_amd/csrc/engine_host.h
+++ b/alphazero_gym_amd/csrc/engine_host.h
@@ -135,6 +135,29 @@
     return fail(e, AZG_E_DEVICE, std::string("hipMalloc: ") + hipGetErrorString(mem.last));
 }
 
+static inline void dump_fill(size_t B, size_t R, bool cont, int A, const int* nrec, const RecL* hot, const EdgeG* edge, const float* V, const float* action,
+                             int32_t* n_records, int32_t* parent, int32_t* edge_n, double* edge_W, double* edge_Q, float* edge_action,
+                             int32_t* node_n, double* node_r, float* node_V, uint8_t* node_flags) {
+    for (size_t i = 0; i < B; ++i) {
+        if (n_records) n_records[i] = nrec[i];
+        for (size_t j = 0; j < R; ++j) {
+            size_t o = i * R + j;
+            bool in = (int)j < nrec[i];
+            const RecL& h = hot[o];
+            bool ex = in && (h.flags & FLAG_EXPANDED);
+            if (parent) parent[o] = in ? (j == 0 ? -1 : h.parent) : 0;
+            if (edge_n) edge_n[o] = in ? h.edge_n : 0;
+            if (edge_W) edge_W[o] = in ? edge[o].W : 0.0;
+            if (edge_Q) edge_Q[o] = in ? h.Q : 0.0;
+            if (edge_action) edge_action[o] = in ? (cont ? action[o] : (j == 0 ? 0.0f : (float)((j - 1) % A))) : 0.0f;
+            if (node_n) node_n[o] = in ? h.node_n : 0;
+            if (node_r) node_r[o] = ex ? edge[o].r : 0.0;
+            if (node_V) node_V[o] = ex ? V[o] : 0.0f;
+            if (node_flags) node_flags[o] = in ? h.flags : 0;
+        }
+    }
+}
+
 int settle_team(azg_engine* e);
 int launch_results(azg_engine* e);
 
diff --git a/alphazero_gym_amd/csrc/engine_selftest.hip b/alphazero_gym_amd/csrc/engine_selftest.hip
--- a/alphazero_gym_amd/csrc/engine_selftest.hip
+++ b/alphazero_gym_amd/csrc/engine_selftest.hip
@@ -1,3 +1,4 @@
+#include <cstddef>
 #include "engine_host.h"
 #include "probe_kernels.cuh"
 
@@ -58,4 +59,19 @@
     return rc;
 }
 
+int azg_selftest_cold_layout(int* out) {
+    if (!out) return AZG_E_INVALID;
+    out[0] = (int)sizeof(Widen); out[1] = (int)alignof(Widen); out[2] = (int)offsetof(Widen, s2); out[3] = (int)offsetof(Widen, mu);
+    out[4] = (int)offsetof(Widen, sg); out[5] = (int)sizeof(EdgeG); out[6] = (int)offsetof(EdgeG, W); out[7] = (int)offsetof(EdgeG, r);
+    return AZG_OK;
 }
+int azg_selftest_dump_fill(size_t B, size_t R, int cont, int A, const int* nrec, const void* hot, const void* edge, const float* V, const float* action,
+                           int32_t* n_records, int32_t* parent, int32_t* edge_n, double* edge_W, double* edge_Q, float* edge_action,
+                           int32_t* node_n, double* node_r, float* node_V, uint8_t* node_flags) {
+    if (!nrec || !hot || !edge || !V || !action) return AZG_E_INVALID;
+    dump_fill(B, R, cont != 0, A, nrec, (const RecL*)hot, (const EdgeG*)edge, V, action,
+              n_records, parent, edge_n, edge_W, edge_Q, edge_action, node_n, node_r, node_V, node_flags);
+    return AZG_OK;
+}
+
+}
diff --git a/alphazero_gym_amd/csrc/env.cuh b/alphazero_gym_amd/csrc/env.cuh
--- a/alphazero_gym_amd/csrc/env.cuh
+++ b/alphazero_gym_amd/csrc/env.cuh
@@ -6,6 +6,7 @@
     static constexpr bool CONT = ENV == AZG_ENV_PENDULUM_V1 || ENV == AZG_ENV_MOUNTAINCAR_CONT;
     static constexpr bool TERM = ENV != AZG_ENV_PENDULUM_V1;
     static constexpr int S = CONT ? 2 : 4;
+    static constexpr bool S4 = !CONT;
     static constexpr bool IN8 = ENV == AZG_ENV_ACROBOT;
 };
 
diff --git a/alphazero_gym_amd/csrc/lockstep.cuh b/alphazero_gym_amd/csrc/lockstep.cuh
--- a/alphazero_gym_amd/csrc/lockstep.cuh
+++ b/alphazero_gym_amd/csrc/lockstep.cuh
@@ -23,8 +23,7 @@
     if (CONT) for (int i = tid; i < P.n_sims + 2; i += 256) s_pw[i] = P.pw_need[i];
     __syncthreads();
     const size_t tb = (size_t)(live ? tree : 0) * P.R;
-    Cold* cold = P.cold + tb;
-    double* edge_W = P.edge_W + tb;
+    const ColdG cs = cold_global(P, tb);
     float* action = P.action + tb;
     TreeStore<false> ts;
     ts.hot = P.hot + tb;
@@ -33,7 +32,7 @@
     float* obsT = L.obsT + (size_t)tg * 64;
     TreeState st;
     if (sim == -2) {
-        tree_init_root<ENV, false>(P, st, ts, cold, edge_W, action, tree, live, sub, tl, gtree, obsT);
+        tree_init_root<ENV, false>(P, st, ts, cs, action, tree, live, sub, tl, gtree, obsT);
     } else {
         const LsTree t = L.tree[live ? tree : 0];
 #ifdef AZG_STAMPS
@@ -42,12 +41,12 @@
         const LsLane ln = L.lane[(size_t)(live ? tree : 0) * 16 + sub];
         st.nrec = t.nrec; st.eps_draws = t.eps_draws; st.leaf = t.leaf; st.need_eval = live && t.need_eval; st.path_D = t.path_D;
         st.kbase = t.kbase; st.my_depth = ln.my_depth; st.pid = ln.pid; st.pr = ln.pr; st.pW = ln.pW; st.eps_c = ln.eps_c;
-        if (live) tree_phase_a<ENV, false, GMM, NCH>(P, st, ts, cold, edge_W, action, tb, sim, sub, tl, gtree,
+        if (live) tree_phase_a<ENV, false, GMM, NCH>(P, st, ts, cs, action, tb, sim, sub, tl, gtree,
                                                      L.parts + (size_t)tg * NCH * 64, P.bhead, s_sqrt STAMP_ARG, s_pw);
         st.need_eval = false;
         if (sim < P.n_sims - 1) {
             __threadfence_block();
-            if (live) tree_phase_b<ENV, false, GMM>(P, st, ts, cold, edge_W, action, tb, sub, tl, gtree, s_sqrt, s_pw, obsT STAMP_ARG);
+            if (live) tree_phase_b<ENV, false, GMM>(P, st, ts, cs, action, tb, sub, tl, gtree, s_sqrt, s_pw, obsT STAMP_ARG);
             else if (sub < 4) obsT[sub * 16 + tl] = 0.0f;
         } else if (live && sub == 0) {
             P.n_rec[tree] = st.nrec;
diff --git a/alphazero_gym_amd/csrc/records.h b/alphazero_gym_amd/csrc/records.h
--- a/alphazero_gym_amd/csrc/records.h
+++ b/alphazero_gym_amd/csrc/records.h
@@ -50,6 +50,17 @@
 static_assert(sizeof(RecS) == 16, "RecS must be 16 bytes");
 static_assert(sizeof(RecL) == 24, "RecL must be 24 bytes");
 
+struct __attribute__((aligned(32))) Widen {
+    double s0, s1, s2;
+    float mu;
+    float sg;
+};
+static_assert(sizeof(Widen) == 32, "Widen must be 32 bytes");
+struct __attribute__((aligned(16))) EdgeG {
+    double W;
+    double r;
+};
+static_assert(sizeof(EdgeG) == 16, "EdgeG must be 16 bytes");
 struct __attribute__((aligned(16))) Cold {
     double s[4];
     double r;
@@ -71,8 +82,10 @@
     const double* roots;
     const int* carry;
     RecL* hot;
-    Cold* cold;
-    double* edge_W;
+    Widen* widen;
+    EdgeG* edge;
+    float* V;
+    double* s3;
     float* action;
     float* prior;
     float* gmm;
@@ -145,7 +158,17 @@
 #define STAMP_M_ADD(slot, t0, t1) STAMP_ADD(slot, t0, t1)
 #endif
 #define STAMP_PARAM_OPT , unsigned long long* st_acc = nullptr
+#ifdef AZG_STAMP_ONLY
+#define STAMP_VMWAIT(slot) do { if constexpr ((slot) == (AZG_STAMP_ONLY)) { if (st_acc) { \
+        __builtin_amdgcn_sched_barrier(0); const unsigned long long vw0 = __builtin_amdgcn_s_memtime(); __builtin_amdgcn_sched_barrier(0); \
+        asm volatile("s_waitcnt vmcnt(0)" ::: "memory"); \
+        const unsigned long long vw1 = __builtin_amdgcn_s_memtime(); __builtin_amdgcn_sched_barrier(0); \
+        st_acc[(slot) - 16] += vw1 - vw0; } } } while (0)
 #else
+#define STAMP_VMWAIT(slot)
+#endif
+#else
+#define STAMP_VMWAIT(slot)
 #define STAMP_PARAM
 #define STAMP_ARG
 #define STAMP(var)
diff --git a/alphazero_gym_amd/csrc/results.cuh b/alphazero_gym_amd/csrc/results.cuh
--- a/alphazero_gym_amd/csrc/results.cuh
+++ b/alphazero_gym_amd/csrc/results.cuh
@@ -3,7 +3,7 @@
 #include "tree.cuh"
 
 template <bool CONT, int TLDS>
-__device__ __forceinline__ void results_for_tree(const KParams& P, const TreeStore<TLDS>& ts, const Cold* cold, const float* action, size_t tb,
+__device__ __forceinline__ void results_for_tree(const KParams& P, const TreeStore<TLDS>& ts, const ColdG& cs, const float* action, size_t tb,
                                                  int tree, int sub) {
     typedef typename TreeStore<TLDS>::Rec Rec;
     const int Kmax = P.res_Kmax;
@@ -20,7 +20,7 @@
         P.res_Q[o] = k >= 0 ? h.Q : 0.0;
         const bool ex = k >= 0 && (h.flags & FLAG_EXPANDED);
         P.res_child_n[o] = ex ? (int)h.node_n : -1;
-        for (int s2 = 0; s2 < P.S; ++s2) P.res_child_state[o * P.S + s2] = ex ? cold[k].s[s2] : 0.0;
+        for (int s2 = 0; s2 < P.S; ++s2) P.res_child_state[o * P.S + s2] = ex ? cs.state(k, s2) : 0.0;
         if (k >= 0) { tot_l += (int)h.edge_n; qmax_l = h.Q > qmax_l ? h.Q : qmax_l; }
     }
     for (int m = 1; m < 16; m <<= 1) {
@@ -45,7 +45,7 @@
         }
         P.res_vt[tree] = P.res_v_target == AZG_VT_ON_POLICY ? onp : qmax;
         P.res_nch[tree] = nc;
-        P.res_root_V[tree] = cold[0].V;
+        P.res_root_V[tree] = cs.V(0);
     }
     if (CONT && P.ncomp >= 2) {
         for (int i = sub; i < 3 * P.ncomp; i += 16) {
@@ -53,7 +53,7 @@
             P.res_root_dist[(size_t)tree * 3 * P.ncomp + i] = P.gmm[tb * 3 * GMM_MAXC + part * GMM_MAXC + c];
         }
     } else if (CONT) {
-        if (sub == 0) { P.res_root_dist[(size_t)tree * 2] = cold[0].mu; P.res_root_dist[(size_t)tree * 2 + 1] = cold[0].sg; }
+        if (sub == 0) { P.res_root_dist[(size_t)tree * 2] = cs.mu(0); P.res_root_dist[(size_t)tree * 2 + 1] = cs.sg(0); }
     } else {
         for (int d = sub; d < P.nd; d += 16) P.res_root_dist[(size_t)tree * P.nd + d] = ts.prior[(int)root.first + d];
     }
diff --git a/alphazero_gym_amd/csrc/search_kernel.cuh b/alphazero_gym_amd/csrc/search_kernel.cuh
--- a/alphazero_gym_amd/csrc/search_kernel.cuh
+++ b/alphazero_gym_amd/csrc/search_kernel.cuh
@@ -103,7 +103,7 @@
 
     struct Ctx {
         int sub, tl, tree; bool has_tree, live; unsigned gtree; size_t tb;
-        Cold* cold; double* edge_W; float* action; TreeStore<TLDS> ts; const f32x4* my_parts;
+        ColdG cs; float* action; TreeStore<TLDS> ts; const f32x4* my_parts;
     };
     auto make_ctx = [&](int t) {
         Ctx c;
@@ -115,8 +115,7 @@
         c.live = c.has_tree && c.tl < n_live;
         c.gtree = (unsigned)(P.tree_base + c.tree);
         c.tb = (size_t)(c.live ? c.tree : 0) * P.R;
-        c.cold = P.cold + c.tb;
-        c.edge_W = P.edge_W + c.tb;
+        c.cs = cold_global(P, c.tb);
         c.action = P.action + c.tb;
         if constexpr (TLDS != TS_GLOBAL) {
             char* base = (char*)s_dyn + L.tree_off + L.per_tree * c.tl;
@@ -140,7 +139,7 @@
     TreeState st = {};
     st.need_eval = false;
     BDeferred bdef = {};
-    if (cx.has_tree) tree_init_root<ENV, TLDS, TPW, IN8>(P, st, cx.ts, cx.cold, cx.edge_W, cx.action, cx.tree, cx.live, cx.sub, cx.tl, cx.gtree, s_obsT);
+    if (cx.has_tree) tree_init_root<ENV, TLDS, TPW, IN8>(P, st, cx.ts, cx.cs, cx.action, cx.tree, cx.live, cx.sub, cx.tl, cx.gtree, s_obsT);
     __syncthreads();
 
     constexpr bool MULTI = !CONT;
@@ -153,7 +152,7 @@
         STAMP2(t_b, 0, 1);
         if constexpr (DEFER) {
             STAMP2(t_b2a, 12, -1);
-            if (cx.live) tree_phase_b2<ENV, TLDS, SPEC>(P, st, cx.ts, cx.cold, cx.edge_W, cx.action, bdef, cx.sub, cx.gtree, s_pw);
+            if (cx.live) tree_phase_b2<ENV, TLDS, SPEC>(P, st, cx.ts, cx.cs, cx.action, bdef, cx.sub, cx.gtree, s_pw);
             bdef.pending = false;
             STAMP2(t_b2b, 12, -1);
 #ifdef AZG_STAMP_ONLY
@@ -184,18 +183,18 @@
             cx = make_ctx(tid_o);
             st.pr = 0.0; st.pW = 0.0;
             if (cx.live && (MULTI ? my_sim : sim) >= 0 && st.my_depth >= 1) {
-                st.pr = CONT ? cx.cold[st.pid].r : discrete_env_reward(Spec<SPEC, ENV>::env(P));
-                st.pW = cx.edge_W[st.pid];
+                if constexpr (CONT) cx.cs.load_rW(st.pid, st.pr, st.pW);
+                else { st.pr = discrete_env_reward(Spec<SPEC, ENV>::env(P)); st.pW = cx.cs.W(st.pid); }
             }
         }
         if constexpr (!MULTI) {
-            if (cx.live) tree_phase_a<ENV, TLDS, GMM, NCH, PSTR, !CONT, SPEC>(P, st, cx.ts, cx.cold, cx.edge_W, cx.action, cx.tb, sim, cx.sub, cx.tl % NT, cx.gtree, cx.my_parts, s_bhead, s_sqrt STAMP_ARG, s_pw);
+            if (cx.live) tree_phase_a<ENV, TLDS, GMM, NCH, PSTR, !CONT, SPEC>(P, st, cx.ts, cx.cs, cx.action, cx.tb, sim, cx.sub, cx.tl % NT, cx.gtree, cx.my_parts, s_bhead, s_sqrt STAMP_ARG, s_pw);
             if (sim == P.n_sims - 1) break;
             if constexpr (DEFER) { if (sim < 0 && cx.live) eps_prepare(P, st, cx.gtree, cx.sub); }
             tree_fence();
             STAMP2(t_d, 2, 3);
             st.need_eval = false;
-            if (cx.live) tree_phase_b<ENV, TLDS, GMM, TPW, unsigned short, !LEAN, !CONT, SPEC, IN8, DEFER>(P, st, cx.ts, cx.cold, cx.edge_W, cx.action, cx.tb, cx.sub, cx.tl, cx.gtree, s_sqrt, s_pw, s_obsT STAMP_ARG, &bdef);
+            if (cx.live) tree_phase_b<ENV, TLDS, GMM, TPW, unsigned short, !LEAN, !CONT, SPEC, IN8, DEFER>(P, st, cx.ts, cx.cs, cx.action, cx.tb, cx.sub, cx.tl, cx.gtree, s_sqrt, s_pw, s_obsT STAMP_ARG, &bdef);
             tree_fence();
             STAMP2(t_e, 3, -1);
             STAMP_ADD(2, t_c, t_d);
@@ -205,7 +204,7 @@
             int k = 0;
             while (run) {
                 STAMP2(t_c2, 2, -1);
-                tree_phase_a<ENV, TLDS, GMM, NCH, PSTR, !CONT, SPEC>(P, st, cx.ts, cx.cold, cx.edge_W, cx.action, cx.tb, my_sim, cx.sub, cx.tl % NT, cx.gtree, cx.my_parts, s_bhead, s_sqrt STAMP_ARG, s_pw);
+                tree_phase_a<ENV, TLDS, GMM, NCH, PSTR, !CONT, SPEC>(P, st, cx.ts, cx.cs, cx.action, cx.tb, my_sim, cx.sub, cx.tl % NT, cx.gtree, cx.my_parts, s_bhead, s_sqrt STAMP_ARG, s_pw);
                 tree_fence();
                 STAMP2(t_d, 2, 3);
                 st.need_eval = false;
@@ -215,7 +214,7 @@
                     run = false;
                 } else {
                     my_sim += 1;
-                    tree_phase_b<ENV, TLDS, GMM, TPW, unsigned short, !LEAN, !CONT, SPEC, IN8>(P, st, cx.ts, cx.cold, cx.edge_W, cx.action, cx.tb, cx.sub, cx.tl, cx.gtree, s_sqrt, s_pw, s_obsT STAMP_ARG);
+                    tree_phase_b<ENV, TLDS, GMM, TPW, unsigned short, !LEAN, !CONT, SPEC, IN8>(P, st, cx.ts, cx.cs, cx.action, cx.tb, cx.sub, cx.tl, cx.gtree, s_sqrt, s_pw, s_obsT STAMP_ARG);
                     tree_fence();
                     k += 1;
                     if (st.need_eval || k >= P.trace_cap) run = false;
@@ -236,7 +235,7 @@
 #ifdef AZG_STAMPS
     if (lane == 0) for (int i = 0; i < 16; ++i) P.stamps[((size_t)blockIdx.x * NW + wave) * 16 + i] = st_acc[i];
 #endif
-    if (live) results_for_tree<CONT, TLDS>(P, ts, cx.cold, cx.action, tb, tree, sub);
+    if (live) results_for_tree<CONT, TLDS>(P, ts, cx.cs, cx.action, tb, tree, sub);
     if (live) {
         if (sub == 0) P.n_rec[tree] = nrec;
         if constexpr (TLDS != TS_GLOBAL) {
diff --git a/alphazero_gym_amd/csrc/team.cuh b/alphazero_gym_amd/csrc/team.cuh
--- a/alphazero_gym_amd/csrc/team.cuh
+++ b/alphazero_gym_amd/csrc/team.cuh
@@ -117,8 +117,6 @@
     const bool live = has_tree && tree < P.B;
     const unsigned gtree = (unsigned)(P.tree_base + tree);
     const size_t tb = (size_t)(live ? tree : 0) * P.R;
-    Cold* cold = P.cold + tb;
-    double* edge_W = P.edge_W + tb;
     float* action = P.action + tb;
     TreeStore<TLDS> ts;
     if constexpr (TLDS != TS_GLOBAL) {
@@ -133,11 +131,15 @@
         ts.prior = P.prior + tb;
     }
     constexpr bool LDS_COLD = TEAM_LDS_COLD && HP == 1024 && TT == 32 && MINB == 2 && TLDS == TS_LDS8;
+    typedef typename std::conditional<LDS_COLD, ColdL, ColdG>::type CS;
+    CS cs;
     if constexpr (LDS_COLD) {
         char* cb = (char*)s_ab + team_tree_off(P.tab_n, P.n_sims, KC, TGN) + team_tree_bytes(P.R, CONT, TLDS) * TPW + team_cold_bytes(P.R) * (has_tree ? tj : 0);
-        cold = (Cold*)cb;
-        edge_W = (double*)(cb + (size_t)P.R * 64);
+        cs.c = (Cold*)cb;
+        cs.eW = (double*)(cb + (size_t)P.R * 64);
         action = (float*)(cb + (size_t)P.R * 72);
+    } else {
+        cs = cold_global(P, tb);
     }
     TreeState st = {};
     constexpr bool BDEF = TEAM_DEFER && ENV == AZG_ENV_PENDULUM_V1 && !GMM && TT == 32;
@@ -182,7 +184,7 @@
     }
     __syncthreads();
 #endif
-    if (has_tree) tree_init_root<ENV, TLDS, TPW>(P, st, ts, cold, edge_W, action, tree, live, sub, tj, gtree, s_obs);
+    if (has_tree) tree_init_root<ENV, TLDS, TPW>(P, st, ts, cs, action, tree, live, sub, tj, gtree, s_obs);
     __syncthreads();
     first_layer(true);
     team_arrive(cnt);
@@ -230,13 +232,13 @@
         __syncthreads();
         TSTAMP(tp0);
         __builtin_amdgcn_s_setprio(3);
-        if (live) tree_phase_a<ENV, TLDS, GMM, NCH, 64, false, SPEC>(P, st, ts, cold, edge_W, action, tb, sim, sub, tj, gtree, s_ab, P.bhead, s_sqrt STAMP_ARG, s_pw);
+        if (live) tree_phase_a<ENV, TLDS, GMM, NCH, 64, false, SPEC>(P, st, ts, cs, action, tb, sim, sub, tj, gtree, s_ab, P.bhead, s_sqrt STAMP_ARG, s_pw);
         st.need_eval = false;
         TSTAMP(tp1);
         if constexpr (BDEF) { if (k == 0 && live) eps_prepare(P, st, gtree, sub); }
         if (k < P.n_sims) {
             tree_fence();
-            if (live) tree_phase_b<ENV, TLDS, GMM, TPW, int, true, false, SPEC, false, BDEF>(P, st, ts, cold, edge_W, action, tb, sub, tj, gtree, s_sqrt, s_pw, s_obs STAMP_ARG, &bdef);
+            if (live) tree_phase_b<ENV, TLDS, GMM, TPW, int, true, false, SPEC, false, BDEF>(P, st, ts, cs, action, tb, sub, tj, gtree, s_sqrt, s_pw, s_obs STAMP_ARG, &bdef);
         }
         __builtin_amdgcn_s_setprio(0);
         TSTAMP(tp2);
@@ -248,7 +250,7 @@
             first_layer(wt);
             team_arrive(cnt);
             if constexpr (BDEF) {
-                if (live) tree_phase_b2<ENV, TLDS, SPEC, true>(P, st, ts, cold, edge_W, action, bdef, sub, gtree, s_pw);
+                if (live) tree_phase_b2<ENV, TLDS, SPEC, true>(P, st, ts, cs, action, bdef, sub, gtree, s_pw);
                 bdef.pending = false;
             }
         }
@@ -276,7 +278,8 @@
             }
         }
         if constexpr (LDS_COLD) {
-            for (int j = sub; j < st.nrec; j += 16) { P.cold[tb + j] = cold[j]; P.edge_W[tb + j] = edge_W[j]; P.action[tb + j] = action[j]; }
+            const ColdG g = cold_global(P, tb);
+            for (int j = sub; j < st.nrec; j += 16) { g.template put<EnvFamily<ENV>::S4>(j, cs.c[j], cs.eW[j]); P.action[tb + j] = action[j]; }
         }
     }
 #ifdef AZG_STAMPS
diff --git a/alphazero_gym_amd/csrc/tree.cuh b/alphazero_gym_amd/csrc/tree.cuh
--- a/alphazero_gym_amd/csrc/tree.cuh
+++ b/alphazero_gym_amd/csrc/tree.cuh
@@ -1,4 +1,5 @@
 #pragma once
+#include <type_traits>
 #include "records.h"
 
 __device__ __forceinline__ void tree_fence() { __builtin_amdgcn_fence(__ATOMIC_ACQ_REL, "wavefront"); }
@@ -155,8 +156,84 @@
 __device__ __forceinline__ void clear_pad(RecM& h) { h.cbase = 0; }
 __device__ __forceinline__ void clear_pad(RecL& h) { h.pad = 0; }
 
-template <bool CONT, int TLDS, typename F, typename PW = int>
-__device__ __forceinline__ void backup_from(const TreeStore<TLDS>& ts, const Cold* cold, double* edge_W, int j, float V, int sub,
+struct ColdRegs { double s[4]; float mu, sg, V; };
+struct ColdG {
+    Widen* w; EdgeG* e; float* v; double* s3;
+    template <bool S4, bool WV> __device__ __forceinline__ ColdRegs load(int j) const {
+        ColdRegs c;
+        const Widen x = w[j];
+        c.s[0] = x.s0; c.s[1] = x.s1; c.s[2] = x.s2; c.s[3] = 0.0; c.mu = x.mu; c.sg = x.sg; c.V = 0.0f;
+        if constexpr (S4) c.s[3] = s3[j];
+        if constexpr (WV) c.V = v[j];
+        return c;
+    }
+    template <bool S4> __device__ __forceinline__ void load_state(int j, double* s) const {
+        s[0] = w[j].s0; s[1] = w[j].s1; s[2] = w[j].s2;
+        if constexpr (S4) s[3] = s3[j];
+    }
+    __device__ __forceinline__ double state(int j, int k) const { return k == 0 ? w[j].s0 : (k == 1 ? w[j].s1 : (k == 2 ? w[j].s2 : s3[j])); }
+    __device__ __forceinline__ float mu(int j) const { return w[j].mu; }
+    __device__ __forceinline__ float sg(int j) const { return w[j].sg; }
+    __device__ __forceinline__ float V(int j) const { return v[j]; }
+    __device__ __forceinline__ double r(int j) const { return e[j].r; }
+    __device__ __forceinline__ double W(int j) const { return e[j].W; }
+    __device__ __forceinline__ void load_rW(int j, double& r, double& W) const { const EdgeG x = e[j]; r = x.r; W = x.W; }
+    __device__ __forceinline__ void set_V(int j, float V) const { v[j] = V; }
+    __device__ __forceinline__ void set_policy(int j, float mu, float sg) const { w[j].mu = mu; w[j].sg = sg; }
+    __device__ __forceinline__ void set_r(int j, double r) const { e[j].r = r; }
+    __device__ __forceinline__ void set_W(int j, double W) const { e[j].W = W; }
+    template <bool S4> __device__ __forceinline__ void set_state(int j, const double* s, float zero) const {
+        Widen x;
+        x.s0 = s[0]; x.s1 = s[1]; x.s2 = s[2]; x.mu = zero; x.sg = zero;
+        w[j] = x;
+        if constexpr (S4) s3[j] = s[3];
+    }
+    template <bool S4> __device__ __forceinline__ void put(int j, const Cold& c, double W) const {
+        Widen x;
+        x.s0 = c.s[0]; x.s1 = c.s[1]; x.s2 = c.s[2]; x.mu = c.mu; x.sg = c.sg;
+        w[j] = x;
+        if constexpr (S4) s3[j] = c.s[3];
+        EdgeG g;
+        g.W = W; g.r = c.r;
+        e[j] = g;
+        v[j] = c.V;
+    }
+};
+__device__ __forceinline__ ColdG cold_global(const KParams& P, size_t tb) {
+    ColdG c;
+    c.w = P.widen + tb; c.e = P.edge + tb; c.v = P.V + tb; c.s3 = P.s3 + tb;
+    return c;
+}
+struct ColdL {
+    Cold* c; double* eW;
+    template <bool S4, bool WV> __device__ __forceinline__ ColdRegs load(int j) const {
+        ColdRegs o;
+        const Cold x = c[j];
+        o.s[0] = x.s[0]; o.s[1] = x.s[1]; o.s[2] = x.s[2]; o.s[3] = S4 ? x.s[3] : 0.0; o.mu = x.mu; o.sg = x.sg; o.V = WV ? x.V : 0.0f;
+        return o;
+    }
+    template <bool S4> __device__ __forceinline__ void load_state(int j, double* s) const {
+        s[0] = c[j].s[0]; s[1] = c[j].s[1]; s[2] = c[j].s[2];
+        if constexpr (S4) s[3] = c[j].s[3];
+    }
+    __device__ __forceinline__ double state(int j, int k) const { return c[j].s[k]; }
+    __device__ __forceinline__ float mu(int j) const { return c[j].mu; }
+    __device__ __forceinline__ float sg(int j) const { return c[j].sg; }
+    __device__ __forceinline__ float V(int j) const { return c[j].V; }
+    __device__ __forceinline__ double r(int j) const { return c[j].r; }
+    __device__ __forceinline__ double W(int j) const { return eW[j]; }
+    __device__ __forceinline__ void load_rW(int j, double& r, double& W) const { r = c[j].r; W = eW[j]; }
+    __device__ __forceinline__ void set_V(int j, float V) const { c[j].V = V; }
+    __device__ __forceinline__ void set_policy(int j, float mu, float sg) const { c[j].mu = mu; c[j].sg = sg; }
+    __device__ __forceinline__ void set_r(int j, double r) const { c[j].r = r; }
+    __device__ __forceinline__ void set_W(int j, double W) const { eW[j] = W; }
+    template <bool S4> __device__ __forceinline__ void set_state(int j, const double* s, float zero) const {
+        c[j].s[0] = s[0]; c[j].s[1] = s[1]; c[j].s[2] = s[2]; c[j].s[3] = S4 ? s[3] : 0.0; c[j].mu = zero; c[j].sg = zero; c[j].pad = zero;
+    }
+};
+
+template <bool CONT, int TLDS, typename CS, typename F, typename PW = int>
+__device__ __forceinline__ void backup_from(const TreeStore<TLDS>& ts, const CS& cs, int j, float V, int sub,
                                             float gamma_f, double gamma, bool firstlvl, bool at_leaf, double Rv, F&& on_node,
                                             const PW* s_pw = nullptr, int pw_cap = 0) {
     typedef typename TreeStore<TLDS>::Rec Rec;
@@ -173,7 +250,7 @@
         Rec mrec = ts.hot[mine];
         const bool is_edge = (sub < cnt) && (mine != 0);
         double r = 0.0, W = 0.0;
-        if (is_edge) { r = cold[mine].r; W = edge_W[mine]; }
+        if (is_edge) cs.load_rW(mine, r, W);
         double myR = 0.0;
         const int nedge = hit_root ? cnt - 1 : cnt;
 #pragma unroll 1
@@ -195,7 +272,7 @@
                 double Wn = W + myR;
                 mrec.Q = tree_div(Wn, (double)en);
                 mrec.edge_n = (decltype(mrec.edge_n))en;
-                edge_W[mine] = Wn;
+                cs.set_W(mine, Wn);
             }
             if (!(at_leaf && sub == 0)) {
                 mrec.node_n = (decltype(mrec.node_n))(mrec.node_n + 1);
@@ -214,8 +291,8 @@
     }
 }
 
-template <bool CONT, int TLDS, typename F, typename PW = int>
-__device__ __forceinline__ void backup_path(const TreeStore<TLDS>& ts, const Cold* cold, double* edge_W, float V, int sub, float gamma_f,
+template <bool CONT, int TLDS, typename CS, typename F, typename PW = int>
+__device__ __forceinline__ void backup_path(const TreeStore<TLDS>& ts, const CS& cs, float V, int sub, float gamma_f,
                                             double gamma, int D, int my_depth, int pid, double pr, double& pW, F&& on_node,
                                             typename TreeStore<TLDS>::Rec& rec, double& chainR, bool same_chain = false,
                                             double r_uniform = 0.0, double r_first = 0.0, const PW* s_pw = nullptr, int pw_cap = 0) {
@@ -275,7 +352,7 @@
             double Wn = pW + myR;
             rec.Q = tree_div(Wn, (double)en);
             rec.edge_n = (decltype(rec.edge_n))en;
-            edge_W[pid] = Wn;
+            cs.set_W(pid, Wn);
             pW = Wn;
         }
         if (my_depth < D) {
@@ -286,6 +363,6 @@
     }
     if (D >= 16) {
         int j = __shfl(par, (D - 15) & 15, 16);
-        backup_from<CONT, TLDS>(ts, cold, edge_W, j, V, sub, gamma_f, gamma, false, false, Rv, on_node, s_pw, pw_cap);
-    }
-}
+        backup_from<CONT, TLDS>(ts, cs, j, V, sub, gamma_f, gamma, false, false, Rv, on_node, s_pw, pw_cap);
+    }
+}
diff --git a/alphazero_gym_amd/csrc/tree_phases.cuh b/alphazero_gym_amd/csrc/tree_phases.cuh
--- a/alphazero_gym_amd/csrc/tree_phases.cuh
+++ b/alphazero_gym_amd/csrc/tree_phases.cuh
@@ -146,8 +146,8 @@
     return win;
 }
 
-template <int ENV, int TLDS, int TPW = 16, bool OBS8 = false>
-__device__ __forceinline__ void tree_init_root(const KParams& P, TreeState& st, const TreeStore<TLDS>& ts, Cold* cold, double* edge_W,
+template <int ENV, int TLDS, int TPW = 16, bool OBS8 = false, typename CS = ColdG>
+__device__ __forceinline__ void tree_init_root(const KParams& P, TreeState& st, const TreeStore<TLDS>& ts, const CS& cs,
                                                float* action, int tree, bool live, int sub, int tl, unsigned gtree, float* obsT) {
     constexpr bool CONT = EnvFamily<ENV>::CONT;
     constexpr int S = CONT ? 2 : 4;
@@ -169,13 +169,13 @@
             clear_pad(h);
             if (CONT) set_wnext(h, pw_at(P.pw_need, (int)P.carry[tree], P.n_sims + 1) > 0);
             ts.hot[0] = h;
-            Cold c;
-#pragma unroll
-            for (int k = 0; k < 4; ++k) c.s[k] = k < S ? rs[k] : 0.0;
-            if (CONT) c.s[2] = sn;
-            c.r = 0.0; c.V = 0.0f; c.mu = 0.0f; c.sg = 0.0f; c.pad = 0.0f;
-            cold[0] = c;
-            edge_W[0] = 0.0;
+            double s4[4];
+#pragma unroll
+            for (int k = 0; k < 4; ++k) s4[k] = k < S ? rs[k] : 0.0;
+            if (CONT) s4[2] = sn;
+            cs.template set_state<EnvFamily<ENV>::S4>(0, s4, 0.0f);
+            cs.set_r(0, 0.0); cs.set_V(0, 0.0f);
+            cs.set_W(0, 0.0);
             if (CONT) action[0] = 0.0f;
             if constexpr (!CONT && TLDS != TS_GLOBAL) {
                 if (ts.state) {
@@ -193,8 +193,8 @@
         }
 }
 
-template <int ENV, int TLDS, bool GMM, int NCH, int PSTR = 64, bool RESUME = false, int SPEC = 0, typename PW = int>
-__device__ __forceinline__ void tree_phase_a(const KParams& P, TreeState& st, const TreeStore<TLDS>& ts, Cold* cold, double* edge_W,
+template <int ENV, int TLDS, bool GMM, int NCH, int PSTR = 64, bool RESUME = false, int SPEC = 0, typename PW = int, typename CS = ColdG>
+__device__ __forceinline__ void tree_phase_a(const KParams& P, TreeState& st, const TreeStore<TLDS>& ts, const CS& cs,
                                              float* action, size_t tb, int sim, int sub, int tl, unsigned gtree, const f32x4* parts,
                                              const float* bhead, const double* s_sqrt STAMP_PARAM_OPT, const PW* s_pw = nullptr) {
     constexpr bool CONT = EnvFamily<ENV>::CONT;
@@ -222,7 +222,7 @@
                 ls = ls < P.ls_min ? P.ls_min : (ls > P.ls_max ? P.ls_max : ls);
                 sg = azg_expf(ls);
             }
-            if (sub == 0) { cold[st.leaf].V = V; cold[st.leaf].mu = mu; cold[st.leaf].sg = sg; }
+            if (sub == 0) { cs.set_V(st.leaf, V); cs.set_policy(st.leaf, mu, sg); }
             if (sim < 0) {
                 int k = st.nrec++;
                 if constexpr (GMM) gmm_pick(gd, P.ncomp, P.seed, gtree, P.search_idx, (unsigned)k, &mu, &sg);
@@ -232,7 +232,7 @@
                     Rec h = make_edge<Rec>((double)V, 0);
                     clear_pad(h);
                     ts.hot[k] = h;
-                    edge_W[k] = 0.0;
+                    cs.set_W(k, 0.0);
                     action[k] = a;
                 }
                 ts.child_append(0, make_edge<Rec>(0.0, 0), 0, k, st.ptop, sub == 0, P.Kp,
@@ -264,10 +264,10 @@
                 clear_pad(h);
                 ts.hot[k0 + sub] = h;
                 ts.prior[k0 + sub] = prior_a;
-                edge_W[k0 + sub] = 0.0;
+                cs.set_W(k0 + sub, 0.0);
             }
             if (sub == 0) {
-                cold[st.leaf].V = V;
+                cs.set_V(st.leaf, V);
                 ts.hot[st.leaf].n_child = (decltype(ts.hot[st.leaf].n_child))A;
                 ts.hot[st.leaf].first = (decltype(ts.hot[st.leaf].first))k0;
             }
@@ -296,7 +296,8 @@
         if (!TLDS) tree_fence();
         const bool keep = !CONT && Spec<SPEC, ENV>::plain(P);
         Rec myrec;
-        backup_path<CONT, TLDS>(ts, cold, edge_W, V, sub, P.gamma_f, P.gamma, st.path_D, st.my_depth, st.pid, st.pr, st.pW,
+        STAMP_VMWAIT(16);
+        backup_path<CONT, TLDS>(ts, cs, V, sub, P.gamma_f, P.gamma, st.path_D, st.my_depth, st.pid, st.pr, st.pW,
                                 [&](int pn) { if (keep) refresh_best<ENV, TLDS, SPEC>(P, ts, pn, sub, s_sqrt); }, myrec, st.chainR,
                                 RESUME && !CONT && st.repeat,
                                 CONT ? 0.0 : discrete_env_reward(Spec<SPEC, ENV>::env(P)),
@@ -341,15 +342,15 @@
     float cact;
 };
 
-template <int ENV, int TLDS, int SPEC, bool FETCH = false, typename PW = int>
-__device__ __forceinline__ void tree_phase_b2(const KParams& P, TreeState& st, const TreeStore<TLDS>& ts, Cold* cold, double* edge_W, float* action,
+template <int ENV, int TLDS, int SPEC, bool FETCH = false, typename PW = int, typename CS = ColdG>
+__device__ __forceinline__ void tree_phase_b2(const KParams& P, TreeState& st, const TreeStore<TLDS>& ts, const CS& cs, float* action,
                                               const BDeferred& d, int sub, unsigned gtree, const PW* s_pw) {
     typedef typename TreeStore<TLDS>::Rec Rec;
     static_assert(ENV == AZG_ENV_PENDULUM_V1, "deferred expansion: the Pendulum family");
     if (!d.pending) return;
-    const double ps0 = cold[d.p].s[0], ps1 = cold[d.p].s[1];
+    const double ps0 = cs.state(d.p, 0), ps1 = cs.state(d.p, 1);
     if (d.widen) {
-        const float V = cold[d.p].V;
+        const float V = cs.V(d.p);
         const Rec hp = ts.hot[d.p];
         if (sub == 0) {
             Rec h = make_edge<Rec>((double)V, d.p);
@@ -357,7 +358,7 @@
             clear_pad(h);
             set_wnext(h, P.pw0 > 0);
             ts.hot[d.chosen] = h;
-            edge_W[d.chosen] = 0.0;
+            cs.set_W(d.chosen, 0.0);
             action[d.chosen] = d.cact;
         }
         ts.child_append(d.p, hp, (int)hp.n_child, d.chosen, st.ptop, sub == 0, P.Kp,
@@ -374,14 +375,14 @@
     if (sub == 0) {
         float zero = 0.0f;
         asm volatile("" : "+v"(zero));
-        Cold* c = cold + d.chosen;
-        c->s[3] = 0.0; c->r = r; c->V = zero; c->mu = zero; c->sg = zero; c->pad = zero;
+        cs.set_r(d.chosen, r); cs.set_V(d.chosen, zero);
     }
     eps_prepare(P, st, gtree, sub);
 }
 
-template <int ENV, int TLDS, bool GMM, int TPW = 16, typename PW = int, bool FETCH = true, bool RESUME = false, int SPEC = 0, bool OBS8 = false, bool DEFER = false>
-__device__ __forceinline__ void tree_phase_b(const KParams& P, TreeState& st, const TreeStore<TLDS>& ts, Cold* cold, double* edge_W,
+template <int ENV, int TLDS, bool GMM, int TPW = 16, typename PW = int, bool FETCH = true, bool RESUME = false, int SPEC = 0, bool OBS8 = false, bool DEFER = false,
+          typename CS = ColdG>
+__device__ __forceinline__ void tree_phase_b(const KParams& P, TreeState& st, const TreeStore<TLDS>& ts, const CS& cs,
                                              float* action, size_t tb, int sub, int tl, unsigned gtree, const double* s_sqrt,
                                              const PW* s_pw, float* obsT STAMP_PARAM, BDeferred* def = nullptr) {
     static_assert(!DEFER || (ENV == AZG_ENV_PENDULUM_V1 && !GMM), "deferred expansion: Pendulum family, squashed-Normal head");
@@ -407,11 +408,13 @@
     const double r_step = CONT ? 0.0 : discrete_env_reward(Spec<SPEC, ENV>::env(P));
     const bool keep_slot = !CONT && FETCH && resumed && st.my_depth >= 1;
     Rec hp = ts.hot[p];
-    Cold cp;
+    constexpr bool S4 = EnvFamily<ENV>::S4;
+    constexpr bool WV = CONT && !DEFER;
+    ColdRegs cp;
     bool from_cold = true;
     if constexpr (!CONT && TLDS != TS_GLOBAL) from_cold = (ts.state == nullptr);
-    if (from_cold) cp = cold[p];
-    else { cp.s[0] = cp.s[1] = cp.s[2] = cp.s[3] = 0.0; }
+    if (from_cold) cp = cs.template load<S4, WV>(p);
+    else { cp.s[0] = cp.s[1] = cp.s[2] = cp.s[3] = 0.0; cp.mu = cp.sg = cp.V = 0.0f; }
     if (!resumed) { st.path_D = 0; st.my_depth = sub == 0 ? 0 : -1; st.pid = 0; }
     if (!keep_slot) { st.pr = 0.0; st.pW = 0.0; }
     int chosen = 0;
@@ -441,8 +444,12 @@
         STAMP2(tl1, 7, -1);
         STAMP_ADD(7, tl0, tl1);
         STAMP2(tl2, 8, 9);
-        Cold cn;
-        if constexpr (CONT && EARLY_COLD) cn = cold[chosen];
+        ColdRegs cn;
+        [[maybe_unused]] double cn_r = 0.0, cn_W = 0.0;
+        if constexpr (CONT && EARLY_COLD) {
+            cn = cs.template load<S4, WV>(chosen);
+            if constexpr (FETCH) cs.load_rW(chosen, cn_r, cn_W);
+        }
         Rec hc = ts.hot[chosen];
         if (!(hc.flags & FLAG_EXPANDED)) break;
         STAMP2(tl3, 9, 10);
@@ -451,14 +458,17 @@
         hp = hc;
         if (sub == (st.path_D & 15)) {
             st.my_depth = st.path_D; st.pid = chosen;
-            if (CONT && FETCH) { st.pr = EARLY_COLD ? cn.r : cold[chosen].r; st.pW = edge_W[chosen]; }
-            if (!CONT && FETCH) { st.pr = r_step; st.pW = edge_W[chosen]; }
+            if constexpr (CONT && FETCH) {
+                if constexpr (EARLY_COLD) { st.pr = cn_r; st.pW = cn_W; }
+                else cs.load_rW(chosen, st.pr, st.pW);
+            }
+            if (!CONT && FETCH) { st.pr = r_step; st.pW = cs.W(chosen); }
         }
         if constexpr (EnvFamily<ENV>::TERM) {
             if (hc.flags & FLAG_TERMINAL) { hit_terminal = true; break; }
         }
-        if (CONT) { if constexpr (EARLY_COLD) cp = cn; else cp = cold[p]; }
-        else if (from_cold) { cp.s[0] = cold[p].s[0]; cp.s[1] = cold[p].s[1]; cp.s[2] = cold[p].s[2]; cp.s[3] = cold[p].s[3]; }
+        if (CONT) { if constexpr (EARLY_COLD) cp = cn; else cp = cs.template load<S4, WV>(p); }
+        else if (from_cold) cs.template load_state<S4>(p, cp.s);
         STAMP2(tl4, 10, 11);
         STAMP_ADD(8, tl0, tl2);
         STAMP_ADD(9, tl2, tl3);
@@ -470,6 +480,7 @@
     }
     STAMP2(tb1, 13, 14);
     STAMP_ADD(13, tb0, tb1);
+    STAMP_VMWAIT(17);
     if (hit_terminal) {
         st.leaf = p;
     } else {
@@ -492,7 +503,7 @@
                     Rec h = make_edge<Rec>((double)cp.V, p);
                     clear_pad(h);
                     ts.hot[chosen] = h;
-                    edge_W[chosen] = 0.0;
+                    cs.set_W(chosen, 0.0);
                     action[chosen] = cact;
                 }
                 ts.child_append(p, hp, K, chosen, st.ptop, sub == 0, P.Kp, pw_at(s_pw, (int)hp.node_n, P.n_sims + 1) - (K + 1) > 0);
@@ -530,16 +541,21 @@
         STAMP_ADD(15, tw1, tw2);
         if constexpr (DEFER) {
             def->pending = true; def->widen = widen; def->p = p; def->chosen = chosen; def->cact = cact;
-            if (sub == 0) { cold[chosen].s[0] = ns[0]; cold[chosen].s[1] = ns[1]; cold[chosen].s[2] = sn; }
+            if (sub == 0) {
+                float zero = 0.0f;
+                asm volatile("" : "+v"(zero));
+                const double s3w[3] = {ns[0], ns[1], sn};
+                cs.template set_state<false>(chosen, s3w, zero);
+            }
         } else if (sub == 0) {
-            Cold c;
-#pragma unroll
-            for (int k = 0; k < 4; ++k) c.s[k] = k < S ? ns[k] : 0.0;
-            if (CONT) c.s[2] = sn;
+            double s4[4];
+#pragma unroll
+            for (int k = 0; k < 4; ++k) s4[k] = k < S ? ns[k] : 0.0;
+            if (CONT) s4[2] = sn;
             float zero = 0.0f;
             asm volatile("" : "+v"(zero));
-            c.r = r; c.V = zero; c.mu = zero; c.sg = zero; c.pad = zero;
-            cold[chosen] = c;
+            cs.template set_state<S4>(chosen, s4, zero);
+            cs.set_r(chosen, r); cs.set_V(chosen, zero);
             if constexpr (CONT) {
                 Rec hn = ts.hot[chosen];
                 hn.flags = (unsigned char)(FLAG_EXPANDED | (done ? FLAG_TERMINAL : 0));
```
